# Amin-Nadimy/P-A_multigrids

Hardware: NVIDIA B200
Metric: DG DOF-updates/s per smoother sweep (higher is better)
Workload: dtype f64

## Files before the change

### p-a_multigrids_b200/csrc/pamg_api.cu

```cuda
#include <cuda_runtime.h>
#include <dlfcn.h>

#include <algorithm>
#include <cmath>
#include <cstdio>
#include <cstring>
#include <string>
#include <vector>

#include "pamg_internal.h"
#include "pamg_kernels.cuh"
#include "pamg_unstr.cuh"

using namespace pamg;

namespace {
typedef struct ncclComm* ncclComm_t;
typedef struct { char internal[128]; } ncclUniqueId;
enum { ncclUint8 = 1, ncclInt32 = 2, ncclFloat64 = 8, ncclSum = 0, ncclMax = 2, ncclMin = 3, ncclSuccess = 0 };
struct NcclApi {
  void* lib = nullptr;
  int (*GetUniqueId)(ncclUniqueId*) = nullptr;
  int (*CommInitRank)(ncclComm_t*, int, ncclUniqueId, int) = nullptr;
  int (*CommDestroy)(ncclComm_t) = nullptr;
  int (*GroupStart)() = nullptr;
  int (*GroupEnd)() = nullptr;
  int (*Send)(const void*, size_t, int, int, ncclComm_t, cudaStream_t) = nullptr;
  int (*Recv)(void*, size_t, int, int, ncclComm_t, cudaStream_t) = nullptr;
  int (*AllReduce)(const void*, void*, size_t, int, int, ncclComm_t, cudaStream_t) = nullptr;
  bool load() {
    if (lib) return true;
    lib = dlopen("libnccl.so.2", RTLD_NOW | RTLD_GLOBAL);
    if (!lib) return false;
    GetUniqueId = (decltype(GetUniqueId))dlsym(lib, "ncclGetUniqueId");
    CommInitRank = (decltype(CommInitRank))dlsym(lib, "ncclCommInitRank");
    CommDestroy = (decltype(CommDestroy))dlsym(lib, "ncclCommDestroy");
    GroupStart = (decltype(GroupStart))dlsym(lib, "ncclGroupStart");
    GroupEnd = (decltype(GroupEnd))dlsym(lib, "ncclGroupEnd");
    Send = (decltype(Send))dlsym(lib, "ncclSend");
    Recv = (decltype(Recv))dlsym(lib, "ncclRecv");
    AllReduce = (decltype(AllReduce))dlsym(lib, "ncclAllReduce");
    return GetUniqueId && CommInitRank && CommDestroy && GroupStart && GroupEnd && Send && Recv && AllReduce;
  }
};
NcclApi g_nccl;
}

__attribute__((constructor)) static void pamg_request_eager_loading() { setenv("CUDA_MODULE_LOADING", "EAGER", 0); }

struct pamg_handle;
namespace { void p2p_close(pamg_handle* h); }
enum { AGG_COUNTER = 0, AGG_EPOCH = 8, AGG_FLAGS = 40, AGG_EXPECT = 72, AGG_WORDS = 104 };

struct LevelDev {
  int s = 0, S = 0;
  long long C = 0, nelem = 0, ndof = 0;
  double* T[2] = {nullptr, nullptr};
  int cur = 0;
  bool tnew_alias = true;
  double *told = nullptr, *rhs = nullptr, *res = nullptr;
  double* ovlb[2] = {nullptr, nullptr};
  int ovl_cur = 0;
  bool strips_valid = false;
  bool cut_valid = false;
  bool stage_valid = false;
  ulonglong2* xsend = nullptr;
  double* ovl_old = nullptr;
  double* pc = nullptr;
  double* pc_old = nullptr;
  bool rhs_valid = false;
  double* spare = nullptr;
};

struct pamg_handle {
  pamg_params p;
  int device = 0, nsm = 148;
  cudaStream_t stream = nullptr;
  cudaEvent_t ev[16] = {};
  long long launches = 0;
  std::string err;
  HaloPlan plan;
  int U = 0;
  double* xg = nullptr;
  int32_t *strip_of = nullptr, *dst_strip = nullptr, *rev = nullptr, *hmap = nullptr, *nsrc = nullptr, *cut_lf = nullptr;
  std::vector<int32_t> bc_kind_h; std::vector<double> bc_val_h;
  int32_t* bc_kind = nullptr; double* bc_val = nullptr;
  double* strip_arena = nullptr; size_t strip_arena_bytes = 0;
  bool l2_persist = true;
  std::vector<LevelDev> lev;
  double* partial = nullptr; int npartial = 0; int last_partials = 0;
  double* out3 = nullptr;
  double* out3_host = nullptr;
  double* scratch = nullptr; size_t scratch_bytes = 0;
  int kernel_mode = 4;
  int halo_mode = 2;
  long long debug_gap_ns = 0;
  struct KernelCfg { int win2[2] = {0, 0}, win2x = 0, win[2] = {0, 0}, tma[2] = {0, 0}, gs2 = 0, gs2x = 0, gs = 0, halo = 0; bool done = false; } kc;
  bool capturing = false;
  bool use_graph = true;
  struct VcGraph { long long key; std::vector<cudaGraphExec_t> exec; std::vector<long long> launches; };
  std::vector<VcGraph> vc_graphs;
  bool graph_nccl = true;
  bool gs_tma = true;
  bool win_producer = true;
  bool gs_fused = true;
  bool vc_norm_fuse = true;
  bool profiling = false;
  std::vector<cudaEvent_t> pev;
  int pev_used = 0;
  ncclComm_t comm = nullptr; int nranks = 1, rank = 0;
  pamg_handle* agg = nullptr;
  int agg_level = 0;
  int level_offset = 0;
  bool shared_stream = false;
  std::vector<int32_t> part_first;
  int U_global = 0;
  std::vector<pamg_handle*> parts;
  bool is_root = false;
  bool in_group = false;
  unsigned long long* agg_words = nullptr;
  UnstrDev un;
  int un_use_dir = 0;
  long long un_host_syncs = 0;
  cudaStream_t up_stream = nullptr, down_stream = nullptr;
  cudaEvent_t ev_up = nullptr, ev_comp = nullptr, ev_down[2] = {nullptr, nullptr};
  unsigned pipe_calls = 0;
  const double* last_out = nullptr;
  bool p2p_enabled = true, p2p_ready = false, p2p_failed = false;
  unsigned long long* p2p_sync = nullptr;
  unsigned long long* p2p_err_host = nullptr;
  unsigned long long* p2p_err_dev = nullptr;
  uint4* p2p_stage = nullptr;
  long long p2p_strips = 0;
  bool xchg_in_kernel = true;
  struct P2PPeer { int slot_at_peer = -1, strip_begin_at_peer = 0; long long recv_strips_at_peer = 0; uint4* stage = nullptr; };
  std::vector<P2PPeer> p2p_peers;
  std::vector<void*> p2p_opened;
  unsigned long long p2p_timeout_ns = 60000000000ull;
};

namespace {

int fail(pamg_handle* h, int code, const std::string& msg) {
  if (h) h->err = msg;
  return code;
}
 #define CK_(hh, call)                                                                            \
  do {                                                                                           \
    cudaError_t e_ = (call);                                                                     \
    if (e_ != cudaSuccess)                                                                       \
      return fail(hh, PAMG_ERR_CUDA, std::string(#call) + ": " + cudaGetErrorString(e_));        \
  } while (0)
#define CK(call)                                                                                 \
  do {                                                                                           \
    cudaError_t e_ = (call);                                                                     \
    if (e_ != cudaSuccess)                                                                       \
      return fail(h, PAMG_ERR_CUDA, std::string(#call) + ": " + cudaGetErrorString(e_));         \
  } while (0)

inline int grid_for(const pamg_handle* h, long long n) {
  long long need = (n + TPB - 1) / TPB;
  long long cap = (long long)h->nsm * 8;
  return (int)std::max(1ll, std::min(need, cap));
}

bool valid_level(const pamg_handle* h, int level) { return h && level >= 1 && level <= (int)h->lev.size(); }

double* tnew_ptr(LevelDev& L) { return L.tnew_alias ? L.T[L.cur] : L.T[L.cur ^ 1]; }

int materialise_tnew(pamg_handle* h, LevelDev& L) {
  if (!L.tnew_alias) return PAMG_OK;
  CK(cudaMemcpyAsync(L.T[L.cur ^ 1], L.T[L.cur], L.ndof * sizeof(double), cudaMemcpyDeviceToDevice, h->stream));
  L.tnew_alias = false;
  return PAMG_OK;
}

double* field_ptr(pamg_handle* h, int field, int level, bool for_write, int* rc) {
  *rc = PAMG_OK;
  LevelDev& L = h->lev[level - 1];
  switch (field) {
    case PAMG_TNEW:
      if (for_write) { *rc = materialise_tnew(h, L); L.strips_valid = false; L.cut_valid = false; L.stage_valid = false; return L.T[L.cur ^ 1]; }
      return tnew_ptr(L);
    case PAMG_TNONLIN:
      if (for_write) { *rc = materialise_tnew(h, L); L.strips_valid = false; L.cut_valid = false; L.stage_valid = false; }
      return L.T[L.cur];
    case PAMG_TOLD: if (for_write) L.rhs_valid = false; return L.told;
    case PAMG_RHS: if (for_write) L.rhs_valid = true; return L.rhs;
    case PAMG_RES: return L.res;
  }
  *rc = PAMG_ERR_ARG;
  return nullptr;
}

bool parent_coefficients(const pamg_params& p, const double* Xall, const int32_t* neig, const int32_t* bc_kind,
                         int g , int s, double* pc, double th, bool with_mass = true) {
  bool supported = true;
  const double* X = Xall + (size_t)g * 6;
  const double x1 = X[0], y1 = X[1], x2 = X[2], y2 = X[3], x3 = X[4], y3 = X[5];
  const double A = x1 - x3, B = y1 - y3, Cc = x2 - x3, D = y2 - y3;
  const double detj = A * D - B * Cc;
  const double area = 0.5 * std::fabs(detj);
  const double g1[2] = {D / detj, -Cc / detj}, g2[2] = {-B / detj, A / detj};
  const double g3[2] = {-(g1[0] + g2[0]), -(g1[1] + g2[1])};
  const double* G[3] = {g1, g2, g3};
  const double two_s = std::ldexp(1.0, s), four_s = std::ldexp(1.0, 2 * s);
  pc[PC_CM] = with_mass ? area / (12.0 * four_s * p.dt) : 0.0;
  auto dot = [](const double* a, const double* b) { return a[0] * b[0] + a[1] * b[1]; };
  const double kth = th * p.k;
  pc[PC_K11] = kth * area * dot(g1, g1); pc[PC_K12] = kth * area * dot(g1, g2); pc[PC_K13] = kth * area * dot(g1, g3);
  pc[PC_K22] = kth * area * dot(g2, g2); pc[PC_K23] = kth * area * dot(g2, g3); pc[PC_K33] = kth * area * dot(g3, g3);
  const double uu[2] = {th * p.u_x, th * p.u_y};
  for (int i = 0; i < 3; ++i) pc[PC_ADV + i] = area * dot(G[i], uu) / (3.0 * two_s);
  const double cx = (x1 + x2 + x3) / 3.0, cy = (y1 + y2 + y3) / 3.0;
  const int fa[3] = {0, 2, 1}, fb[3] = {2, 1, 0}, mface[3] = {0, 2, 1};
  const double V1[2] = {A, B}, V2[2] = {Cc, D};
  const double ci[3][2] = {{1.0 / 3, -2.0 / 3}, {-2.0 / 3, 1.0 / 3}, {1.0 / 3, 1.0 / 3}};
  for (int f = 0; f < 3; ++f) {
    const double ax = X[2 * fa[f]], ay = X[2 * fa[f] + 1], bx = X[2 * fb[f]], by = X[2 * fb[f] + 1];
    const double ex = bx - ax, ey = by - ay, L = std::sqrt(ex * ex + ey * ey);
    double nx = ey / L, ny = -ex / L;
    const double mx = 0.5 * (ax + bx), my = 0.5 * (ay + by);
    if (nx * (mx - cx) + ny * (my - cy) < 0) { nx = -nx; ny = -ny; }
    const double lhalf = 0.5 * L;
    pc[PC_FL + f] = (uu[0] * nx + uu[1] * ny) * lhalf / (3.0 * two_s);
    const double dix = ci[f][0] * V1[0] + ci[f][1] * V2[0], diy = ci[f][0] * V1[1] + ci[f][1] * V2[1];
    const double dcI = std::sqrt(dix * dix + diy * diy);
    pc[PC_PENI + f] = kth * lhalf / (3.0 * dcI);
    const int q = neig[(size_t)g * 3 + mface[f]];
    double dcX;
    if (q != 0) {
      const double* Y = Xall + (size_t)(q - 1) * 6;
      const double qx = (Y[0] + Y[2] + Y[4]) / 3.0, qy = (Y[1] + Y[3] + Y[5]) / 3.0;
      dcX = std::sqrt((cx - qx) * (cx - qx) + (cy - qy) * (cy - qy));
    } else {
      dcX = std::sqrt((cx - mx) * (cx - mx) + (cy - my) * (cy - my));
    }
    pc[PC_PENX + f] = kth * lhalf / (3.0 * dcX);
    if (q == 0 && bc_kind && bc_kind[(size_t)g * 3 + mface[f]] == 2) {
      pc[PC_PENX + f] = 0.0;
      if (p.face_terms && pc[PC_FL + f] < 0.0) supported = false;
    }
  }
  const double f2 = p.face_terms ? 2.0 : 0.0;
  pc[PC_W + 0] = p.omega / (4.0 * pc[PC_CM] + pc[PC_K11] + f2 * (pc[PC_PENI + 0] + pc[PC_PENI + 2]));
  pc[PC_W + 1] = p.omega / (4.0 * pc[PC_CM] + pc[PC_K22] + f2 * (pc[PC_PENI + 1] + pc[PC_PENI + 2]));
  pc[PC_W + 2] = p.omega / (4.0 * pc[PC_CM] + pc[PC_K33] + f2 * (pc[PC_PENI + 0] + pc[PC_PENI + 1]));
  pc[22] = 0.0; pc[23] = 0.0;
  for (int o = 0; o < 2; ++o) {
    const double sg = o == 0 ? 1.0 : -1.0;
    double* F = pc + PC_FOLD + 16 * o;
    double A[3][3];
    const double K[3][3] = {{pc[PC_K11], pc[PC_K12], pc[PC_K13]}, {pc[PC_K12], pc[PC_K22], pc[PC_K23]},
                            {pc[PC_K13], pc[PC_K23], pc[PC_K33]}};
    for (int i = 0; i < 3; ++i)
      for (int j = 0; j < 3; ++j)
        A[i][j] = pc[PC_CM] * ((i == j ? 1.0 : 0.0) + 1.0) - sg * pc[PC_ADV + i] + K[i][j];
    const int fa2[3] = {0, 2, 1}, fb2[3] = {2, 1, 0};
    double c[3];
    for (int f = 0; f < 3; ++f) {
      const double pen = p.face_terms ? pc[PC_PENI + f] : 0.0;
      const double fl = p.face_terms ? sg * pc[PC_FL + f] : 0.0;
      const bool in = fl < 0.0;
      const double own = pen + (in ? 0.0 : fl);
      c[f] = -pen + (in ? fl : 0.0);
      const int ia = fa2[f], ib = fb2[f];
      A[ia][ia] += 2.0 * own; A[ia][ib] += own; A[ib][ia] += own; A[ib][ib] += 2.0 * own;
    }
    F[0] = A[0][0]; F[1] = A[0][1]; F[2] = A[0][2]; F[3] = A[1][0]; F[4] = A[1][1]; F[5] = A[1][2];
    F[6] = A[2][0]; F[7] = A[2][1]; F[8] = A[2][2]; F[9] = c[0]; F[10] = c[1]; F[11] = c[2];
    F[12] = pc[PC_W + 0]; F[13] = pc[PC_W + 1]; F[14] = pc[PC_W + 2]; F[15] = 0.0;
  }
  for (int f = 0; f < 3; ++f) pc[PC_DPEN + f] = p.face_terms ? pc[PC_PENX + f] - pc[PC_PENI + f] : 0.0;
  pc[PC_DPEN + 3] = 0.0;
  for (int mask = 0; mask < 8; ++mask) {
    double pen[3];
    for (int f = 0; f < 3; ++f) pen[f] = p.face_terms ? ((mask >> f) & 1 ? pc[PC_PENX + f] : pc[PC_PENI + f]) : 0.0;
    pc[PC_WB + mask * 3 + 0] = p.omega / (4.0 * pc[PC_CM] + pc[PC_K11] + 2.0 * (pen[0] + pen[2]));
    pc[PC_WB + mask * 3 + 1] = p.omega / (4.0 * pc[PC_CM] + pc[PC_K22] + 2.0 * (pen[1] + pen[2]));
    pc[PC_WB + mask * 3 + 2] = p.omega / (4.0 * pc[PC_CM] + pc[PC_K33] + 2.0 * (pen[0] + pen[1]));
  }
  for (int i = PC_WB + 24; i < NPC; ++i) pc[i] = 0.0;
  if (!with_mass) {
    for (int i = 0; i < 3; ++i) { pc[PC_W + i] = 0.0; pc[PC_FOLD + 12 + i] = 0.0; pc[PC_FOLD + 16 + 12 + i] = 0.0; }
    for (int i = 0; i < 24; ++i) pc[PC_WB + i] = 0.0;
  }
  return supported;
}

int launch_halo(pamg_handle* h, int level, int what = 0);
int p2p_upload_args(pamg_handle* h);

void p2p_close(pamg_handle* h) {
  for (void* p : h->p2p_opened) cudaIpcCloseMemHandle(p);
  h->p2p_opened.clear();
  if (h->p2p_sync) { cudaFree(h->p2p_sync); h->p2p_sync = nullptr; }
  if (h->p2p_stage) { cudaFree(h->p2p_stage); h->p2p_stage = nullptr; }
  if (h->p2p_err_host) { cudaFreeHost(h->p2p_err_host); h->p2p_err_host = nullptr; h->p2p_err_dev = nullptr; }
  h->p2p_ready = false; h->p2p_failed = false;
  for (auto& pp : h->p2p_peers) pp.stage = nullptr;
}

int p2p_check(pamg_handle* h) {
  if (h->p2p_err_host && *(volatile unsigned long long*)h->p2p_err_host)
    return fail(h, PAMG_ERR_CUDA, "halo exchange timed out waiting for a peer GPU");
  return PAMG_OK;
}

long long stage_offset(long long strips, const std::vector<LevelDev>& lev, int il) {
  long long off = 0;
  for (int l = 0; l < il; ++l) off += (long long)P2P_SLOTS * strips * 3 * lev[l].S;
  return off;
}

int p2p_alloc_local(pamg_handle* h) {
  long long strips = 0;
  for (const auto& pr : h->plan.peers) strips = std::max(strips, (long long)pr.strip_begin + pr.nfaces);
  h->p2p_strips = strips;
  const size_t nlev = h->lev.size();
  const size_t stage_bytes = (size_t)std::max(1ll, stage_offset(h->p2p_strips, h->lev, (int)nlev)) * sizeof(uint4);
  CK(cudaMalloc(&h->p2p_sync, nlev * P2P_WORDS * sizeof(unsigned long long)));
  CK(cudaMemset(h->p2p_sync, 0, nlev * P2P_WORDS * sizeof(unsigned long long)));
  CK(cudaMalloc(&h->p2p_stage, stage_bytes));
  CK(cudaMemset(h->p2p_stage, 0, stage_bytes));
  CK(cudaHostAlloc(&h->p2p_err_host, sizeof(unsigned long long), cudaHostAllocMapped | cudaHostAllocPortable));
  *h->p2p_err_host = 0;
  CK(cudaHostGetDevicePointer((void**)&h->p2p_err_dev, h->p2p_err_host, 0));
  return PAMG_OK;
}

int p2p_setup(pamg_handle* h) {
  const int R = h->nranks;
  int ok = 1;
  if ((int)h->plan.peers.size() > P2P_MAXP) ok = 0;
  for (const auto& pp : h->p2p_peers) if (pp.slot_at_peer < 0) ok = 0;
  if (p2p_alloc_local(h) != PAMG_OK) { ok = 0; (void)cudaGetLastError(); }
  struct Card { cudaIpcMemHandle_t handle; };
  Card mine;
  std::memset(&mine, 0, sizeof(mine));
  if (ok && cudaIpcGetMemHandle(&mine.handle, h->p2p_stage) != cudaSuccess) { ok = 0; (void)cudaGetLastError(); }
  const size_t hb = sizeof(Card);
  std::vector<Card> all(R);
  unsigned char* d_buf = nullptr;
  const bool have_buf = cudaMalloc(&d_buf, hb * (R + 1) + sizeof(int)) == cudaSuccess;
  int rc = PAMG_OK;
  if (!have_buf) {
    return fail(h, PAMG_ERR_CUDA, "cudaMalloc failed in the halo-exchange set-up");
  }
  unsigned char* d_mine = d_buf; unsigned char* d_all = d_buf + hb; int* d_ok = (int*)(d_buf + hb * (R + 1));
  if (cudaMemcpy(d_mine, &mine, hb, cudaMemcpyHostToDevice) != cudaSuccess) ok = 0;
  g_nccl.GroupStart();
  for (int r = 0; r < R; ++r) {
    g_nccl.Send(d_mine, hb, ncclUint8, r, h->comm, h->stream);
    g_nccl.Recv(d_all + hb * r, hb, ncclUint8, r, h->comm, h->stream);
  }
  if (g_nccl.GroupEnd() != ncclSuccess) rc = fail(h, PAMG_ERR_CUDA, "handle exchange failed");
  if (!rc && cudaStreamSynchronize(h->stream) != cudaSuccess) ok = 0;
  if (!rc && cudaMemcpy(all.data(), d_all, hb * R, cudaMemcpyDeviceToHost) != cudaSuccess) ok = 0;
  if (!rc && ok) {
    for (size_t i = 0; i < h->plan.peers.size(); ++i) {
      void* ptr = nullptr;
      if (cudaIpcOpenMemHandle(&ptr, all[h->plan.peers[i].part].handle, cudaIpcMemLazyEnablePeerAccess) != cudaSuccess) { ok = 0; (void)cudaGetLastError(); break; }
      h->p2p_opened.push_back(ptr);
      h->p2p_peers[i].stage = (uint4*)ptr;
    }
  }
  if (!rc) {
    if (cudaMemcpy(d_ok, &ok, sizeof(int), cudaMemcpyHostToDevice) != cudaSuccess) ok = 0;
    if (g_nccl.AllReduce(d_ok, d_ok, 1, ncclInt32, ncclMin, h->comm, h->stream) != ncclSuccess) rc = fail(h, PAMG_ERR_CUDA, "ncclAllReduce failed");
    else if (cudaStreamSynchronize(h->stream) != cudaSuccess || cudaMemcpy(&ok, d_ok, sizeof(int), cudaMemcpyDeviceToHost) != cudaSuccess)
      rc = fail(h, PAMG_ERR_CUDA, "halo-exchange set-up: reading the agreement failed");
  }
  cudaFree(d_buf);
  if (rc) return rc;
  if (ok) {
    if ((rc = p2p_upload_args(h))) return rc;
    h->p2p_ready = true;
  } else h->p2p_failed = true;
  return PAMG_OK;
}

int p2p_args(pamg_handle* h, LevelDev& L, double* ovl, P2PArgs& a) {
  const long long S3 = 3ll * L.S;
  const int il = (int)(&L - h->lev.data());
  const int base = h->plan.peers[0].send_begin;
  a.send = ovl + ((size_t)h->plan.nstrips + base) * S3;
  a.strips = ovl; a.stage = h->p2p_stage + stage_offset(h->p2p_strips, h->lev, il); a.stage_words = h->p2p_strips * S3;
  a.sync = h->p2p_sync + (size_t)il * P2P_WORDS; a.err = h->p2p_err_dev; a.npeers = (int)h->plan.peers.size();
  a.timeout_ns = h->p2p_timeout_ns;
  long long so = 0, ro = 0;
  for (int i = 0; i < a.npeers; ++i) {
    const auto& pr = h->plan.peers[i];
    if ((long long)(pr.send_begin - base) * S3 != so) return fail(h, PAMG_ERR_STATE, "send slots are not contiguous per peer");
    a.remote[i] = h->p2p_peers[i].stage + stage_offset(h->p2p_peers[i].recv_strips_at_peer, h->lev, il) +
                  (long long)h->p2p_peers[i].strip_begin_at_peer * S3;
    a.rstride[i] = h->p2p_peers[i].recv_strips_at_peer * S3;
    a.soff[i] = so; a.roff[i] = ro; a.rbeg[i] = (long long)pr.strip_begin * S3;
    so += pr.nfaces * S3; ro += pr.nfaces * S3;
  }
  a.soff[a.npeers] = so; a.roff[a.npeers] = ro;
  a.send_base = base;
  return PAMG_OK;
}

int p2p_upload_args(pamg_handle* h) {
  if (h->plan.peers.empty()) return PAMG_OK;
  std::vector<ulonglong2> t((size_t)h->U * 3);
  for (size_t l = 0; l < h->lev.size(); ++l) {
    P2PArgs v;
    std::memset(&v, 0, sizeof(v));
    int rc = p2p_args(h, h->lev[l], h->lev[l].ovlb[0], v);
    if (rc) return rc;
    const long long S3 = 3ll * h->lev[l].S;
    for (int lf = 0; lf < h->U * 3; ++lf) {
      const int d = h->plan.dst_strip[lf];
      t[lf] = make_ulonglong2(0ull, 0ull);
      if (d < h->plan.nstrips) continue;
      const long long q0 = (long long)(d - h->plan.nstrips - v.send_base) * S3;
      int p = 0;
      while (q0 >= v.soff[p + 1]) ++p;
      t[lf] = make_ulonglong2((unsigned long long)(v.remote[p] + (q0 - v.soff[p])), (unsigned long long)v.rstride[p]);
    }
    if (!h->lev[l].xsend) CK(cudaMalloc(&h->lev[l].xsend, t.size() * sizeof(ulonglong2)));
    CK(cudaMemcpy(h->lev[l].xsend, t.data(), t.size() * sizeof(ulonglong2), cudaMemcpyHostToDevice));
  }
  return PAMG_OK;
}

int exchange_halo_nccl(pamg_handle* h, LevelDev& L, double* ovl) {
  if (!h->comm) return fail(h, PAMG_ERR_STATE, "partitioned mesh but pamg_comm_init was not called");
  const size_t S3 = (size_t)3 * L.S;
  g_nccl.GroupStart();
  for (const auto& pr : h->plan.peers) {
    const size_t n = (size_t)pr.nfaces * S3;
    g_nccl.Send(ovl + ((size_t)h->plan.nstrips + pr.send_begin) * S3, n, ncclFloat64, pr.part, h->comm, h->stream);
    g_nccl.Recv(ovl + (size_t)pr.strip_begin * S3, n, ncclFloat64, pr.part, h->comm, h->stream);
  }
  if (g_nccl.GroupEnd() != ncclSuccess) return fail(h, PAMG_ERR_CUDA, "ncclGroupEnd failed in halo exchange");
  return PAMG_OK;
}

int launch_halo(pamg_handle* h, int level, int what) {
  LevelDev& L = h->lev[level - 1];
  HaloArgs a;
  a.tnew = tnew_ptr(L); a.told = L.told; a.ovl = L.ovlb[L.ovl_cur]; a.ovl_old = L.ovl_old; a.xg = h->xg;
  a.dst_strip = h->dst_strip; a.rev = h->rev; a.strip_of = h->strip_of;
  a.bc_scale = (h->p.coarse_bc_zero && level + h->level_offset > 1) ? 0.0 : 1.0;
  a.U = h->U; a.s = L.s; a.with_old = (what == 0) ? 1 : 0; a.what = what; a.nstrips = h->plan.nstrips;
  a.cut_lf = h->cut_lf; a.ncut = (int)h->plan.cut_lf.size();
  a.bc_kind = h->bc_kind; a.bc_val = h->bc_val;
  const bool cut = what != 1 && !h->plan.peers.empty();
  if ((what == 2 || what == 4) && !cut) { L.cut_valid = true; return PAMG_OK; }
  if (what == 4 && !(h->p2p_ready && L.stage_valid)) return fail(h, PAMG_ERR_STATE, "nothing staged to unpack");
  const long long n = (what == 2 ? (long long)a.ncut : what == 4 ? (long long)a.ncut * 3 : (long long)h->U * 3) * L.S;
  a.x.npeers = 0;
  if (cut && h->comm && h->p2p_enabled && !h->p2p_ready && !h->p2p_failed && !h->capturing && h->level_offset == 0) {
    int rc = p2p_setup(h);
    if (rc) return rc;
  }
  const bool fused_x = cut && h->p2p_ready;
  if (what == 0 && cut) {
    HaloArgs b = a;
    b.tnew = L.told; b.ovl = L.ovl_old; b.with_old = 0; b.what = 2;
    if (fused_x) { int rc = p2p_args(h, L, L.ovl_old, b.x); if (rc) return rc; }
    const long long n2 = (long long)b.ncut * L.S;
    int g2 = grid_for(h, n2);
    if (fused_x) g2 = std::min(g2, h->nsm * std::min(std::max(h->kc.halo, 1), 4));
    k_halo<<<g2, TPB, 0, h->stream>>>(b);
    h->launches++;
    CK(cudaGetLastError());
    if (!fused_x) { int rc = exchange_halo_nccl(h, L, L.ovl_old); if (rc) return rc; }
  }
  if (fused_x) { int rc = p2p_args(h, L, L.ovlb[L.ovl_cur], a.x); if (rc) return rc; }
  int hgrid = grid_for(h, n);
  if (fused_x) hgrid = std::min(hgrid, h->nsm * std::min(std::max(h->kc.halo, 1), 4));
  k_halo<<<hgrid, TPB, 0, h->stream>>>(a);
  h->launches++;
  CK(cudaGetLastError());
  if (what == 1) return PAMG_OK;
  if (what == 4) { L.cut_valid = true; return PAMG_OK; }
  if (cut && !fused_x) { int rc = exchange_halo_nccl(h, L, L.ovlb[L.ovl_cur]); if (rc) return rc; }
  L.cut_valid = true;
  if (fused_x) L.stage_valid = true;
  if (what != 2) L.strips_valid = true;
  return PAMG_OK;
}

int ensure_strips(pamg_handle* h, int level, bool all = true) {
  LevelDev& L = h->lev[level - 1];
  if (!h->p.face_terms) return PAMG_OK;
  if ((all || h->halo_mode == 0) && !L.strips_valid) return launch_halo(h, level, 3);
  if (L.cut_valid) return PAMG_OK;
  return launch_halo(h, level, (L.stage_valid && h->p2p_ready) ? 4 : 2);
}

bool xchg_kernel(const pamg_handle* h, const LevelDev& L) {
  return h->xchg_in_kernel && h->p2p_ready && L.xsend && !h->plan.peers.empty() && h->p.face_terms &&
         h->kernel_mode == 4 && h->win_producer && L.s >= 6 && L.s <= 8;
}

int add_old_time_terms(pamg_handle* h);

int launch_build_rhs(pamg_handle* h) {
  LevelDev& L = h->lev[0];
  RhsArgs a;
  a.told = L.told; a.rhs = L.rhs; a.pc = L.pc; a.xg = h->xg; a.dt = h->p.dt; a.source_coef = h->p.source_coef;
  a.nelem = L.nelem; a.s = L.s; a.literal_source = h->p.literal_source;
  k_build_rhs<<<grid_for(h, L.nelem), TPB, 0, h->stream>>>(a);
  h->launches++;
  CK(cudaGetLastError());
  if (L.pc_old) { int rc = add_old_time_terms(h); if (rc) return rc; }
  L.rhs_valid = true;
  return PAMG_OK;
}

template <typename K>
int configure_one(pamg_handle* h, K kern, int threads, size_t smem, int& resident) {
  CK(cudaFuncSetAttribute(kern, cudaFuncAttributeMaxDynamicSharedMemorySize, (int)smem));
  CK(cudaOccupancyMaxActiveBlocksPerMultiprocessor(&resident, kern, threads, smem));
  if (resident < 1) resident = 1;
  return PAMG_OK;
}
template <bool FACE>
int configure_face(pamg_handle* h) {
  int rc, dummy = 0;
  const int f = FACE ? 1 : 0;
  if ((rc = configure_one(h, k_element_win2<MODE_JACOBI, FACE>, WIN2_THREADS, WIN_SMEM_BYTES, h->kc.win2[f]))) return rc;
  if ((rc = configure_one(h, k_element_win2<MODE_RESID, FACE>, WIN2_THREADS, WIN_SMEM_BYTES, dummy))) return rc;
  if ((rc = configure_one(h, k_element_win2<MODE_RICH, FACE>, WIN2_THREADS, WIN_SMEM_BYTES, dummy))) return rc;
  if (FACE) {
    if ((rc = configure_one(h, k_element_win2<MODE_JACOBI, FACE, true>, WIN2_THREADS, WIN_SMEM_BYTES, h->kc.win2x))) return rc;
    if ((rc = configure_one(h, k_element_win2<MODE_JACOBI, FACE, false, true>, WIN2_THREADS, WIN_SMEM_BYTES, dummy))) return rc;
    if ((rc = configure_one(h, k_element_win2<MODE_JACOBI, FACE, true, true>, WIN2_THREADS, WIN_SMEM_BYTES, dummy))) return rc;
    if ((rc = configure_one(h, k_element_win2<MODE_RICH, FACE, true>, WIN2_THREADS, WIN_SMEM_BYTES, dummy))) return rc;
  }
  if ((rc = configure_one(h, k_element_win<MODE_JACOBI, FACE>, TPB, WIN_SMEM_BYTES, h->kc.win[f]))) return rc;
  if ((rc = configure_one(h, k_element_win<MODE_RESID, FACE>, TPB, WIN_SMEM_BYTES, dummy))) return rc;
  if ((rc = configure_one(h, k_element_win<MODE_RICH, FACE>, TPB, WIN_SMEM_BYTES, dummy))) return rc;
  if ((rc = configure_one(h, k_element_win<MODE_GS, FACE>, TPB, WIN_SMEM_BYTES, dummy))) return rc;
  if ((rc = configure_one(h, k_element_tma<MODE_JACOBI, FACE>, TPB, TMA_SMEM_BYTES, h->kc.tma[f]))) return rc;
  if ((rc = configure_one(h, k_element_tma<MODE_RESID, FACE>, TPB, TMA_SMEM_BYTES, dummy))) return rc;
  if ((rc = configure_one(h, k_element_tma<MODE_RICH, FACE>, TPB, TMA_SMEM_BYTES, dummy))) return rc;
  if ((rc = configure_one(h, k_element_tma<MODE_GS, FACE>, TPB, TMA_SMEM_BYTES, dummy))) return rc;
  return PAMG_OK;
}
int configure_kernels(pamg_handle* h) {
  if (h->kc.done) return PAMG_OK;
  int rc;
  if ((rc = configure_face<true>(h))) return rc;
  if ((rc = configure_face<false>(h))) return rc;
  if ((rc = configure_one(h, k_gs_win2<false>, WIN2_THREADS, GSW_SMEM_BYTES, h->kc.gs2))) return rc;
  if ((rc = configure_one(h, k_gs_win2<true>, WIN2_THREADS, GSW_SMEM_BYTES, h->kc.gs2x))) return rc;
  if ((rc = configure_one(h, k_gs_win, TPB, GSW_SMEM_BYTES, h->kc.gs))) return rc;
  CK(cudaOccupancyMaxActiveBlocksPerMultiprocessor(&h->kc.halo, k_halo, TPB, 0));
  if (h->kc.halo < 1) h->kc.halo = 1;
  cudaFuncAttributes fa;
  CK(cudaFuncGetAttributes(&fa, k_halo));
  CK(cudaFuncGetAttributes(&fa, k_gs_small));
  CK(cudaFuncGetAttributes(&fa, k_build_rhs));
  CK(cudaFuncGetAttributes(&fa, k_restrict));
  CK(cudaFuncGetAttributes(&fa, k_prolong_literal));
  CK(cudaFuncGetAttributes(&fa, k_prolong_p1));
  CK(cudaFuncGetAttributes(&fa, k_reduce_partials));
  CK(cudaFuncGetAttributes(&fa, k_fill));
  CK(cudaFuncGetAttributes(&fa, k_push));
  CK(cudaFuncGetAttributes(&fa, k_wait_flags));
  CK(cudaFuncGetAttributes(&fa, k_spin));
  CK(cudaFuncGetAttributes(&fa, k_output_fields));
  CK(cudaFuncGetAttributes(&fa, k_element_direct2<MODE_JACOBI, true>));
  CK(cudaFuncGetAttributes(&fa, k_element_direct2<MODE_JACOBI, false>));
  CK(cudaFuncGetAttributes(&fa, k_element_direct2<MODE_RESID, true>));
  CK(cudaFuncGetAttributes(&fa, k_element_direct2<MODE_RESID, false>));
  CK(cudaFuncGetAttributes(&fa, k_element_direct2<MODE_RICH, true>));
  CK(cudaFuncGetAttributes(&fa, k_element_direct2<MODE_RICH, false>));
  CK(cudaFuncGetAttributes(&fa, k_element_direct2<MODE_GS, true>));
  CK(cudaFuncGetAttributes(&fa, k_element_direct2<MODE_GS, false>));
  h->kc.done = true;
  return PAMG_OK;
}

bool producer_kernel(const pamg_handle* h, const LevelDev& L, bool gs) {
  if (!(h->kernel_mode == 4 && h->win_producer && L.s >= 6 && L.s <= 8)) return false;
  return !gs || (h->gs_fused && h->p.face_terms);
}

struct ElemOverride { const double* ovl; const double* pc; double rsign; };

template <int MODE>
int launch_element(pamg_handle* h, LevelDev& L, const double* Tin, double* Tout, int colour, int grid, bool use_strips,
                   bool write_next = false, bool xchg = false, bool norm = false, const ElemOverride* ov = nullptr) {
  ElemArgs a;
  a.xsend = L.xsend; a.xsync = h->p2p_sync ? h->p2p_sync + (size_t)(&L - h->lev.data()) * P2P_WORDS : nullptr;
  if (MODE == MODE_RESID) xchg = false;
  a.Tin = Tin; a.Tout = Tout; a.rhs = L.rhs; a.ovl = L.ovlb[L.ovl_cur]; a.pc = L.pc; a.strip_of = h->strip_of; a.hmap = h->hmap;
  a.nsrc = (use_strips || Tin == Tout) ? nullptr : h->nsrc;
  a.ovl_next = write_next ? L.ovlb[L.ovl_cur ^ 1] : nullptr; a.dst_strip = h->dst_strip; a.rev = h->rev; a.nstrips = h->plan.nstrips;
  a.partial = h->partial; a.omega = h->p.omega; a.rsign = (double)h->p.residual_sign; a.nelem = L.nelem; a.s = L.s;
  a.colour = colour; a.partial_off = 0;
  if (ov) { a.ovl = ov->ovl; a.pc = ov->pc; a.rsign = ov->rsign; }
  const int f = h->p.face_terms ? 1 : 0;
  const bool prof = !ov && h->profiling && h->pev_used + 2 <= (int)h->pev.size();
  if (prof) CK(cudaEventRecord(h->pev[h->pev_used], h->stream));
  if (MODE != MODE_GS && h->kernel_mode == 4 && h->win_producer && L.s >= 6 && L.s <= 8) {
    auto kern = xchg ? k_element_win2<MODE == MODE_RESID ? MODE_JACOBI : MODE, true, true>
                     : h->p.face_terms ? k_element_win2<MODE, true> : k_element_win2<MODE, false>;
    if (norm) kern = xchg ? k_element_win2<MODE == MODE_JACOBI ? MODE_JACOBI : MODE, true, true, MODE == MODE_JACOBI>
                          : k_element_win2<MODE == MODE_JACOBI ? MODE_JACOBI : MODE, true, false, MODE == MODE_JACOBI>;
    const int tgrid = (int)std::max(1ll, std::min(L.nelem / TPB, (long long)h->nsm * (xchg ? h->kc.win2x : h->kc.win2[f])));
    kern<<<tgrid, WIN2_THREADS, WIN_SMEM_BYTES, h->stream>>>(a);
    if (MODE == MODE_RESID || norm) h->last_partials = tgrid;
  } else if ((MODE != MODE_GS || h->gs_tma) && h->kernel_mode == 4 && L.C >= TPB && L.s <= 8) {
    auto kern = h->p.face_terms ? k_element_win<MODE, true> : k_element_win<MODE, false>;
    const int tgrid = (int)std::max(1ll, std::min(L.nelem / TPB, (long long)h->nsm * h->kc.win[f]));
    kern<<<tgrid, TPB, WIN_SMEM_BYTES, h->stream>>>(a);
    if (MODE == MODE_RESID) h->last_partials = tgrid;
  } else if ((MODE != MODE_GS || h->gs_tma) && (h->kernel_mode == 1 || h->kernel_mode == 4) && L.C >= TPB) {
    auto kern = h->p.face_terms ? k_element_tma<MODE, true> : k_element_tma<MODE, false>;
    const int tgrid = (int)std::max(1ll, std::min((L.nelem + TPB - 1) / TPB, (long long)h->nsm * h->kc.tma[f]));
    kern<<<tgrid, TPB, TMA_SMEM_BYTES, h->stream>>>(a);
    if (MODE == MODE_RESID) h->last_partials = tgrid;
  } else {
    if (MODE == MODE_RESID) h->last_partials = grid;
    if (h->p.face_terms) k_element_direct2<MODE, true><<<grid, TPB, 0, h->stream>>>(a);
    else k_element_direct2<MODE, false><<<grid, TPB, 0, h->stream>>>(a);
  }
  if (prof) { CK(cudaEventRecord(h->pev[h->pev_used + 1], h->stream)); h->pev_used += 2; }
  h->launches++;
  CK(cudaGetLastError());
  return PAMG_OK;
}

int exchange_told_cut(pamg_handle* h) {
  LevelDev& L = h->lev[0];
  if (h->plan.peers.empty()) return PAMG_OK;
  HaloArgs b;
  b.tnew = L.told; b.told = L.told; b.ovl = L.ovl_old; b.ovl_old = L.ovl_old; b.xg = h->xg;
  b.dst_strip = h->dst_strip; b.rev = h->rev; b.strip_of = h->strip_of;
  b.bc_scale = 1.0; b.U = h->U; b.s = L.s; b.with_old = 0; b.what = 2; b.nstrips = h->plan.nstrips;
  b.cut_lf = h->cut_lf; b.ncut = (int)h->plan.cut_lf.size();
  b.bc_kind = h->bc_kind; b.bc_val = h->bc_val;
  b.x.npeers = 0;
  if (h->comm && h->p2p_enabled && !h->p2p_ready && !h->p2p_failed && !h->capturing && h->level_offset == 0) {
    int rc = p2p_setup(h);
    if (rc) return rc;
  }
  const bool fused_x = h->p2p_ready;
  if (fused_x) { int rc = p2p_args(h, L, L.ovl_old, b.x); if (rc) return rc; }
  int g2 = grid_for(h, (long long)b.ncut * L.S);
  if (fused_x) g2 = std::min(g2, h->nsm * std::min(std::max(h->kc.halo, 1), 4));
  k_halo<<<g2, TPB, 0, h->stream>>>(b);
  h->launches++;
  CK(cudaGetLastError());
  if (!fused_x) { int rc = exchange_halo_nccl(h, L, L.ovl_old); if (rc) return rc; }
  if (fused_x) L.stage_valid = false;
  return PAMG_OK;
}

int add_old_time_terms(pamg_handle* h) {
  LevelDev& L = h->lev[0];
  int rc;
  if (h->p.face_terms && (rc = exchange_told_cut(h))) return rc;
  const int grid = grid_for(h, L.nelem);
  if (2 * grid > h->npartial) return fail(h, PAMG_ERR_STATE, "partial buffer too small");
  const ElemOverride ov = {L.ovl_old, L.pc_old, -1.0};
  if ((rc = launch_element<MODE_RESID>(h, L, L.told, L.res, 0, grid, false, false, false, false, &ov))) return rc;
  CK(cudaMemcpyAsync(L.rhs, L.res, (size_t)L.ndof * sizeof(double), cudaMemcpyDeviceToDevice, h->stream));
  return PAMG_OK;
}

bool gs_small_ok(const pamg_handle* h, const LevelDev& L) {
  return h->gs_fused && h->kernel_mode == 4 && h->p.face_terms && L.C <= TPB;
}
bool gs_fused_ok(const pamg_handle* h, const LevelDev& L) {
  if (gs_small_ok(h, L)) return true;
  return h->gs_fused && h->kernel_mode == 4 && h->p.face_terms && L.C >= TPB && L.s <= 8;
}

int launch_gs_fused(pamg_handle* h, LevelDev& L, const double* Tin, double* Tout, bool use_strips, bool write_next, bool xchg) {
  ElemArgs a;
  a.xsend = L.xsend; a.xsync = h->p2p_sync ? h->p2p_sync + (size_t)(&L - h->lev.data()) * P2P_WORDS : nullptr;
  a.Tin = Tin; a.Tout = Tout; a.rhs = L.rhs; a.ovl = L.ovlb[L.ovl_cur]; a.pc = L.pc; a.strip_of = h->strip_of; a.hmap = h->hmap;
  a.nsrc = use_strips ? nullptr : h->nsrc;
  a.ovl_next = write_next ? L.ovlb[L.ovl_cur ^ 1] : nullptr; a.dst_strip = h->dst_strip; a.rev = h->rev; a.nstrips = h->plan.nstrips;
  a.partial = h->partial; a.omega = h->p.omega; a.rsign = (double)h->p.residual_sign; a.nelem = L.nelem; a.s = L.s;
  a.colour = 1; a.partial_off = 0;
  if (gs_small_ok(h, L)) {
    const long long ppc = TPB / L.C, nparents = L.nelem / L.C;
    const int sgrid = (int)std::max(1ll, std::min((nparents + ppc - 1) / ppc, (long long)h->nsm * 8));
    k_gs_small<<<sgrid, TPB, 0, h->stream>>>(a);
    h->launches++;
    CK(cudaGetLastError());
    return PAMG_OK;
  }
  const bool producer = h->win_producer && L.s >= 6;
  const int resident = producer ? (xchg ? h->kc.gs2x : h->kc.gs2) : h->kc.gs;
  const bool prof = h->profiling && h->pev_used + 2 <= (int)h->pev.size();
  if (prof) CK(cudaEventRecord(h->pev[h->pev_used], h->stream));
  const int tgrid = (int)std::max(1ll, std::min(L.nelem / TPB, (long long)h->nsm * resident));
  if (producer && xchg) k_gs_win2<true><<<tgrid, WIN2_THREADS, GSW_SMEM_BYTES, h->stream>>>(a);
  else if (producer) k_gs_win2<false><<<tgrid, WIN2_THREADS, GSW_SMEM_BYTES, h->stream>>>(a);
  else k_gs_win<<<tgrid, TPB, GSW_SMEM_BYTES, h->stream>>>(a);
  if (prof) { CK(cudaEventRecord(h->pev[h->pev_used + 1], h->stream)); h->pev_used += 2; }
  h->launches++;
  CK(cudaGetLastError());
  return PAMG_OK;
}

bool norm_fusable(const pamg_handle* h, const LevelDev& L) {
  return h->p.face_terms && h->kernel_mode == 4 && h->win_producer && L.s >= 6 && L.s <= 8;
}

int do_smooth(pamg_handle* h, int level, int solver, int nsweeps, bool norm_first = false) {
  LevelDev& L = h->lev[level - 1];
  if (level == 1 && !L.rhs_valid) { int rc = launch_build_rhs(h); if (rc) return rc; }
  const int grid = grid_for(h, L.nelem);
  if (solver < 1 || solver > 4) return fail(h, PAMG_ERR_ARG, "solver must be 1 (Jacobi), 2 (Richardson) or 3 (Gauss-Seidel)");
  for (int sw = 0; sw < nsweeps; ++sw) {
    L.tnew_alias = true;
    if (h->debug_gap_ns > 0) { k_spin<<<1, 32, 0, h->stream>>>(h->debug_gap_ns); }
    const bool gs = solver == 3 || solver == 4;
    const bool in_place = gs && !gs_fused_ok(h, L);
    const bool fusedk = h->halo_mode == 2 && h->p.face_terms && !in_place && producer_kernel(h, L, gs);
    const bool use_strips = in_place || fusedk || h->halo_mode == 0;
    const bool xs = fusedk && xchg_kernel(h, L) && (!gs || (h->win_producer && L.s >= 6));
    int rc = ensure_strips(h, level, use_strips);
    if (rc) return rc;
    if (solver == 1 || solver == 2) {
      rc = (solver == 1) ? launch_element<MODE_JACOBI>(h, L, L.T[L.cur], L.T[L.cur ^ 1], 0, grid, use_strips, fusedk, xs,
                                                       norm_first && sw == 0)
                         : launch_element<MODE_RICH>(h, L, L.T[L.cur], L.T[L.cur ^ 1], 0, grid, use_strips, fusedk, xs);
      if (rc) return rc;
      L.cur ^= 1;
      L.tnew_alias = false;
    } else if (!in_place) {
      rc = launch_gs_fused(h, L, L.T[L.cur], L.T[L.cur ^ 1], use_strips, fusedk, xs);
      if (rc) return rc;
      L.cur ^= 1;
      L.tnew_alias = false;
    } else {
      if (sw == nsweeps - 1 && h->p.keep_tnew_gs) { rc = materialise_tnew(h, L); if (rc) return rc; }
      rc = launch_element<MODE_GS>(h, L, L.T[L.cur], L.T[L.cur], 0, grid, true);
      if (rc) return rc;
      rc = launch_element<MODE_GS>(h, L, L.T[L.cur], L.T[L.cur], 1, grid, true);
      if (rc) return rc;
    }
    if (fusedk) {
      L.ovl_cur ^= 1;
      L.strips_valid = true; L.cut_valid = h->plan.peers.empty();
      L.stage_valid = xs;
    } else {
      L.strips_valid = false; L.cut_valid = false; L.stage_valid = false;
    }
  }
  return PAMG_OK;
}

int queue_norms(pamg_handle* h) {
  k_reduce_partials<<<1, 1024, 0, h->stream>>>(h->partial, h->last_partials, h->out3);
  h->launches++;
  CK(cudaGetLastError());
  if (h->comm && h->nranks > 1) {
    g_nccl.GroupStart();
    g_nccl.AllReduce(h->out3, h->out3, 1, ncclFloat64, ncclSum, h->comm, h->stream);
    g_nccl.AllReduce(h->out3 + 1, h->out3 + 1, 2, ncclFloat64, ncclMax, h->comm, h->stream);
    if (g_nccl.GroupEnd() != ncclSuccess) return fail(h, PAMG_ERR_CUDA, "ncclAllReduce failed");
  }
  CK(cudaMemcpyAsync(h->out3_host, h->out3, 3 * sizeof(double), cudaMemcpyDeviceToHost, h->stream));
  return PAMG_OK;
}

int do_residual(pamg_handle* h, int level, double* l2, double* linf, double* smax, bool queue_only = false) {
  LevelDev& L = h->lev[level - 1];
  if (level == 1 && !L.rhs_valid) { int rc = launch_build_rhs(h); if (rc) return rc; }
  const int grid = grid_for(h, L.nelem);
  if (2 * grid > h->npartial) return fail(h, PAMG_ERR_STATE, "partial buffer too small");
  const bool use_strips = L.strips_valid || h->halo_mode == 0;
  int rc = ensure_strips(h, level, use_strips);
  if (rc) return rc;
  rc = launch_element<MODE_RESID>(h, L, tnew_ptr(L), L.res, 0, grid, use_strips);
  if (rc) return rc;
  if (l2 || linf || smax) {
    if ((rc = queue_norms(h))) return rc;
    if (queue_only || h->capturing) return PAMG_OK;
    CK(cudaStreamSynchronize(h->stream));
    if ((rc = p2p_check(h))) return rc;
    if (l2) *l2 = std::sqrt(h->out3_host[0]);
    if (linf) *linf = h->out3_host[1];
    if (smax) *smax = h->out3_host[2];
  }
  return PAMG_OK;
}

int do_restrict(pamg_handle* h, int fine_level) {
  if (fine_level >= (int)h->lev.size()) return PAMG_OK;
  LevelDev& F = h->lev[fine_level - 1];
  LevelDev& Cc = h->lev[fine_level];
  XferArgs a;
  a.src = F.res; a.dst = Cc.rhs; a.ncoarse = Cc.nelem; a.sc = Cc.s; a.mode = h->p.transfer;
  k_restrict<<<grid_for(h, Cc.nelem), TPB, 0, h->stream>>>(a);
  h->launches++;
  CK(cudaGetLastError());
  Cc.rhs_valid = true;
  return PAMG_OK;
}

int do_prolong(pamg_handle* h, int fine_level, bool keep_tnew = true) {
  if (fine_level >= (int)h->lev.size()) return fail(h, PAMG_ERR_ARG, "no coarser level to prolong from");
  LevelDev& F = h->lev[fine_level - 1];
  LevelDev& Cc = h->lev[fine_level];
  XferArgs a;
  a.ncoarse = Cc.nelem; a.sc = Cc.s; a.mode = h->p.transfer;
  if (h->p.transfer == 0) {
    int rc = materialise_tnew(h, F);
    if (rc) return rc;
    a.src = tnew_ptr(Cc); a.dst = F.T[F.cur ^ 1];
    k_prolong_literal<<<grid_for(h, Cc.nelem), TPB, 0, h->stream>>>(a);
  } else {
    if (keep_tnew) {
      int rc = materialise_tnew(h, F);
      if (rc) return rc;
    } else {
      F.tnew_alias = true;
    }
    a.src = Cc.T[Cc.cur]; a.dst = F.T[F.cur];
    F.strips_valid = false; F.cut_valid = false; F.stage_valid = false;
    k_prolong_p1<<<grid_for(h, F.nelem), TPB, 0, h->stream>>>(a);
  }
  h->launches++;
  CK(cudaGetLastError());
  return PAMG_OK;
}

int do_fill(pamg_handle* h, double* p, long long n, double v) {
  if (v == 0.0) { CK(cudaMemsetAsync(p, 0, n * sizeof(double), h->stream)); return PAMG_OK; }
  k_fill<<<grid_for(h, n), TPB, 0, h->stream>>>(p, n, v);
  h->launches++;
  CK(cudaGetLastError());
  return PAMG_OK;
}

typedef std::vector<pamg_handle*> Group;
Group group_of(pamg_handle* h) { return h->parts.empty() ? Group{h} : h->parts; }
int gfail(pamg_handle* owner, pamg_handle* q, int rc) { if (owner != q) owner->err = q->err; return rc; }
#define GALL(G, owner, q, expr)                                            \
  do {                                                                     \
    for (pamg_handle* q : G) {                                             \
      if (q->in_group) cudaSetDevice(q->device);                           \
      int rc_ = (expr);                                                    \
      if (rc_) return gfail(owner, q, rc_);                                \
    }                                                                      \
  } while (0)

int vcycle_rec(const Group& G, pamg_handle* owner, int level, int solver, int nu1, int nu2, int ncoarse, int skip_pre = 0);

int launch_push(pamg_handle* q, const double* src, double* dst, long long n, int channel, unsigned long long* peer_flag) {
  PushArgs a;
  a.src = src; a.dst = dst; a.n = n; a.counter = q->agg_words + AGG_COUNTER; a.epoch = q->agg_words + AGG_EPOCH + channel;
  a.flag = peer_flag;
  const int grid = (int)std::max(1ll, std::min((n + TPB - 1) / TPB, (long long)q->nsm * 2));
  k_push<<<grid, TPB, 0, q->stream>>>(a);
  q->launches++;
  CK_(q, cudaGetLastError());
  return PAMG_OK;
}

int launch_wait(pamg_handle* q, unsigned senders) {
  WaitArgs a;
  a.flags = q->agg_words + AGG_FLAGS; a.expect = q->agg_words + AGG_EXPECT; a.err = q->p2p_err_dev;
  a.timeout_ns = q->p2p_timeout_ns; a.senders = senders;
  k_wait_flags<<<1, 32, 0, q->stream>>>(a);
  q->launches++;
  CK_(q, cudaGetLastError());
  return PAMG_OK;
}

int agg_coarse_solve(const Group& G, pamg_handle* owner, int solver, int nu1, int nu2, int ncoarse) {
  pamg_handle* h0 = G[0];
  const int lvl = h0->agg_level;
  const size_t per_parent = (size_t)3 * h0->lev[lvl - 1].C;
  if (G.size() == 1) {
    pamg_handle* h = h0;
    LevelDev& Lc = h->lev[lvl - 1];
    if (!h->comm) return fail(h, PAMG_ERR_STATE, "agglomeration needs pamg_comm_init");
    g_nccl.GroupStart();
    if (h->rank == 0) {
      LevelDev& A = h->agg->lev[0];
      for (int p = 1; p < h->nranks; ++p)
        g_nccl.Recv(A.rhs + per_parent * h->part_first[p], per_parent * (h->part_first[p + 1] - h->part_first[p]), ncclFloat64, p,
                    h->comm, h->stream);
    } else {
      g_nccl.Send(Lc.rhs, per_parent * h->U, ncclFloat64, 0, h->comm, h->stream);
    }
    if (g_nccl.GroupEnd() != ncclSuccess) return fail(h, PAMG_ERR_CUDA, "ncclGroupEnd failed in coarse gather");
    if (h->rank == 0) {
      pamg_handle* g = h->agg;
      LevelDev& A = g->lev[0];
      CK(cudaMemcpyAsync(A.rhs, Lc.rhs, per_parent * h->U * sizeof(double), cudaMemcpyDeviceToDevice, h->stream));
      CK(cudaMemsetAsync(A.T[A.cur], 0, A.ndof * sizeof(double), h->stream));
      A.tnew_alias = true; A.strips_valid = false; A.cut_valid = false; A.stage_valid = false; A.rhs_valid = true;
      const long long l0 = g->launches;
      int rc = vcycle_rec(Group{g}, g, 1, solver, nu1, nu2, ncoarse);
      h->launches += g->launches - l0;
      if (rc) return fail(h, rc, g->err);
      CK(cudaMemcpyAsync(Lc.T[Lc.cur], A.T[A.cur], per_parent * h->U * sizeof(double), cudaMemcpyDeviceToDevice, h->stream));
    }
    g_nccl.GroupStart();
    if (h->rank == 0) {
      LevelDev& A = h->agg->lev[0];
      for (int p = 1; p < h->nranks; ++p)
        g_nccl.Send(A.T[A.cur] + per_parent * h->part_first[p], per_parent * (h->part_first[p + 1] - h->part_first[p]), ncclFloat64,
                    p, h->comm, h->stream);
    } else {
      g_nccl.Recv(Lc.T[Lc.cur], per_parent * h->U, ncclFloat64, 0, h->comm, h->stream);
    }
    if (g_nccl.GroupEnd() != ncclSuccess) return fail(h, PAMG_ERR_CUDA, "ncclGroupEnd failed in coarse scatter");
    Lc.tnew_alias = true; Lc.strips_valid = false; Lc.cut_valid = false; Lc.stage_valid = false;
    return PAMG_OK;
  }
  pamg_handle* g = h0->agg;
  LevelDev& A = g->lev[0];
  unsigned all = 0;
  for (size_t p = 1; p < G.size(); ++p) {
    pamg_handle* q = G[p];
    cudaSetDevice(q->device);
    LevelDev& Lc = q->lev[lvl - 1];
    int rc = launch_push(q, Lc.rhs, A.rhs + per_parent * q->part_first[p], (long long)(per_parent * q->U), 0,
                         h0->agg_words + AGG_FLAGS + p);
    if (rc) return gfail(owner, q, rc);
    all |= 1u << p;
  }
  {
    pamg_handle* h = h0;
    cudaSetDevice(h->device);
    LevelDev& Lc = h->lev[lvl - 1];
    CK(cudaMemcpyAsync(A.rhs, Lc.rhs, per_parent * h->U * sizeof(double), cudaMemcpyDeviceToDevice, h->stream));
    CK(cudaMemsetAsync(A.T[A.cur], 0, A.ndof * sizeof(double), h->stream));
    int rc = launch_wait(h, all);
    if (rc) return gfail(owner, h, rc);
    A.tnew_alias = true; A.strips_valid = false; A.cut_valid = false; A.stage_valid = false; A.rhs_valid = true;
    const long long l0 = g->launches;
    rc = vcycle_rec(Group{g}, g, 1, solver, nu1, nu2, ncoarse);
    h->launches += g->launches - l0;
    if (rc) { h->err = g->err; return gfail(owner, h, rc); }
    CK(cudaMemcpyAsync(Lc.T[Lc.cur], A.T[A.cur], per_parent * h->U * sizeof(double), cudaMemcpyDeviceToDevice, h->stream));
    Lc.tnew_alias = true; Lc.strips_valid = false; Lc.cut_valid = false; Lc.stage_valid = false;
    for (size_t p = 1; p < G.size(); ++p) {
      pamg_handle* q = G[p];
      LevelDev& Lq = q->lev[lvl - 1];
      rc = launch_push(h, A.T[A.cur] + per_parent * q->part_first[p], Lq.T[Lq.cur], (long long)(per_parent * q->U), (int)p,
                       q->agg_words + AGG_FLAGS + 0);
      if (rc) return gfail(owner, h, rc);
    }
  }
  for (size_t p = 1; p < G.size(); ++p) {
    pamg_handle* q = G[p];
    cudaSetDevice(q->device);
    int rc = launch_wait(q, 1u);
    if (rc) return gfail(owner, q, rc);
    LevelDev& Lq = q->lev[lvl - 1];
    Lq.tnew_alias = true; Lq.strips_valid = false; Lq.cut_valid = false; Lq.stage_valid = false;
  }
  return PAMG_OK;
}

int normalise_parity(pamg_handle* h, LevelDev& L, int cur0) {
  if (L.cur == cur0) return PAMG_OK;
  CK(cudaMemcpyAsync(L.T[L.cur ^ 1], L.T[L.cur], L.ndof * sizeof(double), cudaMemcpyDeviceToDevice, h->stream));
  L.cur ^= 1;
  L.tnew_alias = true;
  return PAMG_OK;
}

int vcycle_rec(const Group& G, pamg_handle* owner, int level, int solver, int nu1, int nu2, int ncoarse, int skip_pre) {
  const int Lmax = (int)G[0]->lev.size();
  std::vector<int> cur0(G.size());
  for (size_t i = 0; i < G.size(); ++i) cur0[i] = G[i]->lev[level - 1].cur;
  auto restore = [&]() -> int {
    for (size_t i = 0; i < G.size(); ++i) {
      if (G[i]->in_group) cudaSetDevice(G[i]->device);
      int rc = normalise_parity(G[i], G[i]->lev[level - 1], cur0[i]);
      if (rc) return gfail(owner, G[i], rc);
    }
    return PAMG_OK;
  };
  if (level == Lmax) {
    GALL(G, owner, q, do_smooth(q, level, solver, ncoarse));
    return restore();
  }
  GALL(G, owner, q, do_smooth(q, level, solver, nu1 - skip_pre));
  for (pamg_handle* q : G) q->lev[level - 1].tnew_alias = true;
  GALL(G, owner, q, do_residual(q, level, nullptr, nullptr, nullptr));
  GALL(G, owner, q, do_restrict(q, level));
  for (pamg_handle* q : G) {
    if (q->in_group) cudaSetDevice(q->device);
    LevelDev& Cc = q->lev[level];
    int rc = do_fill(q, Cc.T[Cc.cur], Cc.ndof, 0.0);
    if (rc) return gfail(owner, q, rc);
    Cc.tnew_alias = true;
    Cc.strips_valid = false; Cc.cut_valid = false; Cc.stage_valid = false;
  }
  int rc;
  if (G[0]->agg_level && level + 1 == G[0]->agg_level) {
    if ((rc = agg_coarse_solve(G, owner, solver, nu1, nu2, ncoarse))) return rc;
  } else {
    if ((rc = vcycle_rec(G, owner, level + 1, solver, nu1, nu2, ncoarse))) return rc;
  }
  GALL(G, owner, q, do_prolong(q, level, false));
  GALL(G, owner, q, do_smooth(q, level, solver, nu2));
  return skip_pre ? PAMG_OK : restore();
}

int vcycle_body(const Group& G, pamg_handle* owner, int solver, int nu1, int nu2, int ncoarse, bool fuse = false, bool first = true) {
  int rc;
  if ((rc = vcycle_rec(G, owner, 1, solver, nu1, nu2, ncoarse, (fuse && !first) ? 1 : 0))) return rc;
  for (pamg_handle* q : G) q->lev[0].tnew_alias = true;
  if (fuse) {
    GALL(G, owner, q, do_smooth(q, 1, solver, 1, true));
    GALL(G, owner, q, queue_norms(q));
    return PAMG_OK;
  }
  double dummy;
  GALL(G, owner, q, do_residual(q, 1, &dummy, nullptr, nullptr, true));
  return PAMG_OK;
}

int undo_norm_sweep(pamg_handle* h) {
  LevelDev& L = h->lev[0];
  const bool fusedk = h->halo_mode == 2 && h->p.face_terms && producer_kernel(h, L, false);
  L.cur ^= 1;
  L.tnew_alias = true;
  if (fusedk) { L.ovl_cur ^= 1; L.strips_valid = true; L.cut_valid = true; }
  else { L.strips_valid = false; L.cut_valid = false; }
  L.stage_valid = false;
  return PAMG_OK;
}

int group_norms(const Group& G, pamg_handle* owner, double* l2, double* linf, double* smax) {
  double s0 = 0.0, s1 = 0.0, s2 = 0.0;
  for (pamg_handle* q : G) {
    if (q->in_group) cudaSetDevice(q->device);
    CK_(q, cudaStreamSynchronize(q->stream));
    int rc = p2p_check(q);
    if (rc) return gfail(owner, q, rc);
    s0 += q->out3_host[0]; s1 = std::max(s1, q->out3_host[1]); s2 = std::max(s2, q->out3_host[2]);
  }
  for (pamg_handle* q : G) if (q != owner && !q->err.empty()) { owner->err = q->err; }
  if (l2) *l2 = std::sqrt(s0);
  if (linf) *linf = s1;
  if (smax) *smax = s2;
  return PAMG_OK;
}

void free_levels(pamg_handle* h) {
  for (auto& g : h->vc_graphs) for (auto e : g.exec) cudaGraphExecDestroy(e);
  h->vc_graphs.clear();
  for (auto& L : h->lev) {
    cudaFree(L.T[0]); cudaFree(L.T[1]); cudaFree(L.spare); cudaFree(L.told); cudaFree(L.rhs); cudaFree(L.res);
    cudaFree(L.ovl_old); cudaFree(L.pc); cudaFree(L.pc_old); cudaFree(L.xsend);
  }
  h->lev.clear();
  cudaFree(h->strip_arena); h->strip_arena = nullptr; h->strip_arena_bytes = 0;
  cudaFree(h->xg); cudaFree(h->strip_of); cudaFree(h->dst_strip); cudaFree(h->rev); cudaFree(h->hmap);
  cudaFree(h->nsrc); cudaFree(h->cut_lf); cudaFree(h->bc_kind); cudaFree(h->bc_val);
  cudaFree(h->partial);
  h->xg = nullptr; h->strip_of = h->dst_strip = h->rev = h->hmap = h->nsrc = h->cut_lf = h->bc_kind = nullptr;
  h->bc_val = nullptr; h->partial = nullptr;
}

}

#define FANOUT(h, q, expr)                                                              \
  if ((h) && !(h)->parts.empty()) {                                                     \
    for (pamg_handle* q : (h)->parts) { int rc_ = (expr); if (rc_) return gfail((h), q, rc_); } \
    return PAMG_OK;                                                                     \
  }
#define ON_PART0(h) if ((h) && !(h)->parts.empty()) (h) = (h)->parts[0]

extern "C" {

const char* pamg_version(void) { return "pamg-b200 0.1 (sm_100a)"; }

int pamg_device_count(int* n) {
  if (!n) return PAMG_ERR_ARG;
  int c = 0;
  cudaError_t e = cudaGetDeviceCount(&c);
  if (e != cudaSuccess || c < 1) { *n = 0; return PAMG_ERR_CUDA; }
  *n = c;
  return PAMG_OK;
}

void pamg_default_params(pamg_params* p, int literal_head) {
  if (!p) return;
  std::memset(p, 0, sizeof(*p));
  p->n_split = 1; p->multi_levels = 1; p->n_smooth = 4; p->n_multigrid = 2; p->n_coarse_smooth = 15; p->solver = 3;
  p->theta = 1.0; p->k = 1.0; p->omega = 0.8; p->u_x = 0.0; p->u_y = 0.0;
  if (literal_head) {
    p->dt = 1.25e-5; p->face_terms = 0; p->literal_source = 1; p->transfer = 0; p->residual_sign = 1;
    p->halo_rule = 0; p->coarse_bc_zero = 0; p->source_coef = -2.0; p->keep_tnew_gs = 1;
  } else {
    p->dt = 1e-3; p->face_terms = 1; p->literal_source = 0; p->transfer = 1; p->residual_sign = -1;
    p->halo_rule = 1; p->coarse_bc_zero = 1; p->source_coef = 2.0; p->keep_tnew_gs = 0;
  }
}

int pamg_create(const pamg_params* p, int device, pamg_handle** out) {
  if (!p || !out) return PAMG_ERR_ARG;
  *out = nullptr;
  if (p->n_split < 1 || p->n_split > 13 || p->multi_levels < 1 || p->multi_levels > p->n_split) return PAMG_ERR_ARG;
  if (!(p->theta >= 0.0 && p->theta <= 1.0)) return PAMG_ERR_ARG;
  if (!(p->dt > 0.0)) return PAMG_ERR_ARG;
  int ndev = 0;
  if (cudaGetDeviceCount(&ndev) != cudaSuccess || ndev < 1) return PAMG_ERR_CUDA;
  if (device < 0 || device >= ndev) return PAMG_ERR_ARG;
  pamg_handle* h = new pamg_handle();
  h->p = *p; h->device = device;
  {
    const char* e = getenv("PAMG_KERNEL");
    if (e && !strcmp(e, "tma1d")) h->kernel_mode = 1;
    else if (e && !strcmp(e, "direct2")) h->kernel_mode = 3;
    else if (e && !strcmp(e, "win")) h->kernel_mode = 4;
    const char* wp = getenv("PAMG_WIN");
    if (wp && !strcmp(wp, "producer")) h->win_producer = true;
    if (wp && !strcmp(wp, "barrier")) h->win_producer = false;
    const char* pp = getenv("PAMG_P2P");
    if (pp && pp[0] == '0') h->p2p_enabled = false;
    const char* pt = getenv("PAMG_P2P_TIMEOUT_S");
    if (pt && atof(pt) > 0.0) h->p2p_timeout_ns = (unsigned long long)(atof(pt) * 1e9);
    const char* dg = getenv("PAMG_DEBUG_GAP_NS");
    if (dg) h->debug_gap_ns = atoll(dg);
    const char* lp = getenv("PAMG_L2_PERSIST");
    if (lp && lp[0] == '0') h->l2_persist = false;
    const char* vn = getenv("PAMG_VC_NORM");
    if (vn && vn[0] == '0') h->vc_norm_fuse = false;
    const char* xk = getenv("PAMG_XCHG");
    if (xk && !strcmp(xk, "halo")) h->xchg_in_kernel = false;
    const char* hl = getenv("PAMG_HALO");
    if (hl && !strcmp(hl, "strips")) h->halo_mode = 0;
    if (hl && !strcmp(hl, "direct")) h->halo_mode = 1;
    if (hl && !strcmp(hl, "fused")) h->halo_mode = 2;
    const char* gr = getenv("PAMG_GRAPH");
    if (gr && gr[0] == '0') h->use_graph = false;
    const char* gn = getenv("PAMG_GRAPH_NCCL");
    if (gn && gn[0] == '0') h->graph_nccl = false;
    const char* g = getenv("PAMG_GS");
    if (g && !strcmp(g, "direct")) { h->gs_tma = false; h->gs_fused = false; }
    if (g && !strcmp(g, "twopass")) h->gs_fused = false;
  }
  if (cudaSetDevice(device) != cudaSuccess) { delete h; return PAMG_ERR_CUDA; }
  cudaDeviceProp prop;
  if (cudaGetDeviceProperties(&prop, device) == cudaSuccess) h->nsm = prop.multiProcessorCount;
  if (cudaStreamCreateWithFlags(&h->stream, cudaStreamNonBlocking) != cudaSuccess) { delete h; return PAMG_ERR_CUDA; }
  bool ok = true;
  for (auto& e : h->ev) ok = ok && cudaEventCreate(&e) == cudaSuccess;
  ok = ok && cudaMalloc(&h->out3, 3 * sizeof(double)) == cudaSuccess;
  ok = ok && cudaMallocHost(&h->out3_host, 3 * sizeof(double)) == cudaSuccess;
  ok = ok && configure_kernels(h) == PAMG_OK;
  if (!ok) { pamg_destroy(h); return PAMG_ERR_CUDA; }
  *out = h;
  return PAMG_OK;
}

namespace {
int group_p2p_setup(pamg_handle* root) {
  const Group& G = root->parts;
  for (pamg_handle* a : G)
    for (pamg_handle* b : G) {
      if (a->device == b->device) continue;
      int can = 0;
      CK_(root, cudaDeviceCanAccessPeer(&can, a->device, b->device));
      if (!can) return fail(root, PAMG_ERR_UNSUPPORTED, "the GPUs of the group cannot access each other's memory (no NVLink / PCIe peer access)");
      CK_(root, cudaSetDevice(a->device));
      cudaError_t e = cudaDeviceEnablePeerAccess(b->device, 0);
      if (e != cudaSuccess && e != cudaErrorPeerAccessAlreadyEnabled) return fail(root, PAMG_ERR_CUDA, std::string("cudaDeviceEnablePeerAccess: ") + cudaGetErrorString(e));
      (void)cudaGetLastError();
    }
  for (pamg_handle* q : G) {
    CK_(root, cudaSetDevice(q->device));
    if ((int)q->plan.peers.size() > P2P_MAXP) return fail(root, PAMG_ERR_UNSUPPORTED, "too many neighbour parts");
    int rc = p2p_alloc_local(q);
    if (rc) return gfail(root, q, rc);
    CK_(root, cudaMalloc(&q->agg_words, AGG_WORDS * sizeof(unsigned long long)));
    CK_(root, cudaMemset(q->agg_words, 0, AGG_WORDS * sizeof(unsigned long long)));
  }
  for (pamg_handle* q : G) {
    for (size_t i = 0; i < q->plan.peers.size(); ++i) {
      if (q->p2p_peers[i].slot_at_peer < 0) return fail(root, PAMG_ERR_STATE, "inconsistent halo plans between parts");
      q->p2p_peers[i].stage = G[q->plan.peers[i].part]->p2p_stage;
    }
  }
  for (pamg_handle* q : G) {
    CK_(root, cudaSetDevice(q->device));
    int rc = p2p_upload_args(q);
    if (rc) return gfail(root, q, rc);
    q->p2p_ready = true;
  }
  return PAMG_OK;
}
}

int pamg_create_multi(const pamg_params* p, int ngpus, const int* devices, pamg_handle** out) {
  if (!p || !out || ngpus < 1 || ngpus > 16) return PAMG_ERR_ARG;
  *out = nullptr;
  pamg_handle* root = new pamg_handle();
  root->p = *p; root->is_root = true;
  for (int i = 0; i < ngpus; ++i) {
    pamg_handle* q = nullptr;
    int rc = pamg_create(p, devices ? devices[i] : i, &q);
    if (rc) { pamg_destroy(root); return rc; }
    q->in_group = true; q->nranks = ngpus; q->rank = i;
    root->parts.push_back(q);
  }
  root->device = root->parts[0]->device; root->nsm = root->parts[0]->nsm; root->use_graph = root->parts[0]->use_graph;
  *out = root;
  return PAMG_OK;
}

void pamg_destroy(pamg_handle* h) {
  if (!h) return;
  if (h->is_root) {
    for (pamg_handle* q : h->parts) { cudaSetDevice(q->device); if (q->stream) cudaStreamSynchronize(q->stream); }
    for (auto& g : h->vc_graphs) for (auto e : g.exec) cudaGraphExecDestroy(e);
    h->vc_graphs.clear();
    for (pamg_handle* q : h->parts) pamg_destroy(q);
    delete h;
    return;
  }
  cudaSetDevice(h->device);
  if (h->stream) cudaStreamSynchronize(h->stream);
  for (auto& g : h->vc_graphs) for (auto e : g.exec) cudaGraphExecDestroy(e);
  h->vc_graphs.clear();
  if (h->stream) cudaStreamSynchronize(h->stream);
  if (h->agg) { pamg_destroy(h->agg); h->agg = nullptr; }
  if (h->comm) g_nccl.CommDestroy(h->comm);
  p2p_close(h);
  if (h->agg_words) { cudaFree(h->agg_words); h->agg_words = nullptr; }
  free_levels(h);
  unstr_free(h->un);
  cudaFree(h->out3); cudaFreeHost(h->out3_host); cudaFree(h->scratch);
  for (auto& e : h->ev) if (e) cudaEventDestroy(e);
  for (auto& e : h->pev) if (e) cudaEventDestroy(e);
  if (h->up_stream) { cudaStreamSynchronize(h->up_stream); cudaStreamSynchronize(h->down_stream); cudaStreamDestroy(h->up_stream); cudaStreamDestroy(h->down_stream); cudaEventDestroy(h->ev_up); cudaEventDestroy(h->ev_comp); cudaEventDestroy(h->ev_down[0]); cudaEventDestroy(h->ev_down[1]); }
  if (h->stream && !h->shared_stream) cudaStreamDestroy(h->stream);
  delete h;
}

const char* pamg_last_error(const pamg_handle* h) { return h ? h->err.c_str() : "null handle"; }

int pamg_set_parents_partition(pamg_handle* h, int U_global, const double* X, const int32_t* neig,
                               const int32_t* fneig, const int32_t* dir, int nparts, const int32_t* part_first,
                               int my_part) {
  if (!h) return PAMG_ERR_ARG;
  if (h->is_root) return fail(h, PAMG_ERR_ARG, "a multi-GPU handle partitions the mesh itself: call pamg_set_parents");
  CK(cudaSetDevice(h->device));
  int rc = build_halo_plan(U_global, X, neig, fneig, dir, h->p.halo_rule, nparts, part_first, my_part, h->plan);
  if (rc) return fail(h, rc, "inconsistent parent arrays (X / Neig / fNeig)");
  free_levels(h);
  if (h->agg) { pamg_destroy(h->agg); h->agg = nullptr; }
  h->agg_level = 0;
  p2p_close(h);
  h->p2p_peers.assign(h->plan.peers.size(), pamg_handle::P2PPeer());
  for (size_t i = 0; i < h->plan.peers.size(); ++i) {
    HaloPlan theirs;
    if (build_halo_plan(U_global, X, neig, fneig, dir, h->p.halo_rule, nparts, part_first, h->plan.peers[i].part, theirs)) continue;
    for (size_t j = 0; j < theirs.peers.size(); ++j)
      h->p2p_peers[i].recv_strips_at_peer = std::max(h->p2p_peers[i].recv_strips_at_peer, (long long)theirs.peers[j].strip_begin + theirs.peers[j].nfaces);
    for (size_t j = 0; j < theirs.peers.size(); ++j)
      if (theirs.peers[j].part == my_part && theirs.peers[j].nfaces == h->plan.peers[i].nfaces) {
        h->p2p_peers[i].slot_at_peer = (int)j;
        h->p2p_peers[i].strip_begin_at_peer = theirs.peers[j].strip_begin;
      }
  }
  const int U = h->plan.U_local, first = h->plan.first;
  if (U < 1) return fail(h, PAMG_ERR_ARG, "empty partition");
  h->U = U; h->U_global = U_global;
  h->part_first.assign(nparts + 1, 0);
  if (part_first) for (int i = 0; i <= nparts; ++i) h->part_first[i] = part_first[i]; else h->part_first[1] = U_global;
  std::vector<double> xg((size_t)U * 6);
  for (int u = 0; u < U; ++u) {
    const double* P = X + (size_t)(first + u) * 6;
    double* o = &xg[(size_t)u * 6];
    o[0] = P[4]; o[1] = P[5]; o[2] = P[0] - P[4]; o[3] = P[1] - P[5]; o[4] = P[2] - P[4]; o[5] = P[3] - P[5];
  }
  CK(cudaMalloc(&h->xg, xg.size() * sizeof(double)));
  CK(cudaMemcpy(h->xg, xg.data(), xg.size() * sizeof(double), cudaMemcpyHostToDevice));
  const size_t n3 = (size_t)U * 3 * sizeof(int32_t);
  CK(cudaMalloc(&h->strip_of, n3)); CK(cudaMalloc(&h->dst_strip, n3)); CK(cudaMalloc(&h->rev, n3)); CK(cudaMalloc(&h->hmap, n3));
  CK(cudaMemcpy(h->strip_of, h->plan.strip_of.data(), n3, cudaMemcpyHostToDevice));
  CK(cudaMemcpy(h->dst_strip, h->plan.dst_strip.data(), n3, cudaMemcpyHostToDevice));
  CK(cudaMemcpy(h->rev, h->plan.rev.data(), n3, cudaMemcpyHostToDevice));
  CK(cudaMemcpy(h->hmap, h->plan.hmap.data(), n3, cudaMemcpyHostToDevice));
  CK(cudaMalloc(&h->nsrc, n3));
  CK(cudaMemcpy(h->nsrc, h->plan.nsrc.data(), n3, cudaMemcpyHostToDevice));
  if (!h->plan.cut_lf.empty()) {
    CK(cudaMalloc(&h->cut_lf, h->plan.cut_lf.size() * sizeof(int32_t)));
    CK(cudaMemcpy(h->cut_lf, h->plan.cut_lf.data(), h->plan.cut_lf.size() * sizeof(int32_t), cudaMemcpyHostToDevice));
  }
  const int32_t* bc_glob = nullptr;
  if (!h->bc_kind_h.empty()) {
    if ((int)h->bc_kind_h.size() != U_global * 3) return fail(h, PAMG_ERR_ARG, "pamg_set_boundary_data was given a different number of parents");
    bc_glob = h->bc_kind_h.data();
    CK(cudaMalloc(&h->bc_kind, n3)); CK(cudaMalloc(&h->bc_val, (size_t)U * 3 * sizeof(double)));
    CK(cudaMemcpy(h->bc_kind, h->bc_kind_h.data() + (size_t)first * 3, n3, cudaMemcpyHostToDevice));
    CK(cudaMemcpy(h->bc_val, h->bc_val_h.data() + (size_t)first * 3, (size_t)U * 3 * sizeof(double), cudaMemcpyHostToDevice));
  }
  h->lev.resize(h->p.multi_levels);
  {
    size_t tot = 0;
    for (int il = 0; il < h->p.multi_levels; ++il) {
      const size_t S = (size_t)1 << (h->p.n_split - il);
      tot += 2 * (((size_t)(h->plan.nstrips + h->plan.nsend) * 3 * S * sizeof(double) + 255) / 256 * 256);
    }
    CK(cudaMalloc(&h->strip_arena, tot));
    CK(cudaMemsetAsync(h->strip_arena, 0, tot, h->stream));
    h->strip_arena_bytes = tot;
    if (h->l2_persist && !h->shared_stream) {
      cudaDeviceProp prop;
      if (cudaGetDeviceProperties(&prop, h->device) == cudaSuccess && prop.persistingL2CacheMaxSize > 0) {
        const size_t want = std::min((size_t)prop.persistingL2CacheMaxSize, std::max(tot, (size_t)1 << 20));
        cudaDeviceSetLimit(cudaLimitPersistingL2CacheSize, want);
        cudaStreamAttrValue av;
        std::memset(&av, 0, sizeof(av));
        av.accessPolicyWindow.base_ptr = h->strip_arena;
        av.accessPolicyWindow.num_bytes = std::min(tot, (size_t)prop.accessPolicyMaxWindowSize);
        av.accessPolicyWindow.hitRatio = (float)std::min(1.0, (double)want / (double)std::max(tot, (size_t)1));
        av.accessPolicyWindow.hitProp = cudaAccessPropertyPersisting;
        av.accessPolicyWindow.missProp = cudaAccessPropertyStreaming;
        cudaStreamSetAttribute(h->stream, cudaStreamAttributeAccessPolicyWindow, &av);
        (void)cudaGetLastError();
      }
    }
  }
  size_t arena_off = 0;
  std::vector<double> pc((size_t)U * NPC);
  for (int il = 0; il < h->p.multi_levels; ++il) {
    LevelDev& L = h->lev[il];
    L.s = h->p.n_split - il; L.S = 1 << L.s; L.C = 1ll << (2 * L.s);
    L.nelem = L.C * U; L.ndof = 3 * L.nelem;
    const size_t fb = (size_t)L.ndof * sizeof(double);
    CK(cudaMalloc(&L.T[0], fb)); CK(cudaMalloc(&L.T[1], fb)); CK(cudaMalloc(&L.told, fb));
    CK(cudaMalloc(&L.rhs, fb)); CK(cudaMalloc(&L.res, fb));
    CK(cudaMemsetAsync(L.T[0], 0, fb, h->stream)); CK(cudaMemsetAsync(L.T[1], 0, fb, h->stream));
    CK(cudaMemsetAsync(L.told, 0, fb, h->stream)); CK(cudaMemsetAsync(L.rhs, 0, fb, h->stream));
    CK(cudaMemsetAsync(L.res, 0, fb, h->stream));
    const size_t ob = (size_t)(h->plan.nstrips + h->plan.nsend) * 3 * L.S * sizeof(double);
    const size_t obp = (ob + 255) / 256 * 256;
    L.ovlb[0] = reinterpret_cast<double*>(reinterpret_cast<char*>(h->strip_arena) + arena_off);
    L.ovlb[1] = reinterpret_cast<double*>(reinterpret_cast<char*>(h->strip_arena) + arena_off + obp);
    arena_off += 2 * obp;
    CK(cudaMalloc(&L.ovl_old, ob));
    CK(cudaMemsetAsync(L.ovl_old, 0, ob, h->stream));
    L.ovl_cur = 0; L.strips_valid = false; L.cut_valid = false; L.stage_valid = false;
    for (int u = 0; u < U; ++u)
      if (!parent_coefficients(h->p, X, neig, bc_glob, first + u, L.s, &pc[(size_t)u * NPC], h->p.theta))
        return fail(h, PAMG_ERR_UNSUPPORTED, "open boundary face (kind 2) with inflow: give it Dirichlet data instead");
    CK(cudaMalloc(&L.pc, pc.size() * sizeof(double)));
    CK(cudaMemcpy(L.pc, pc.data(), pc.size() * sizeof(double), cudaMemcpyHostToDevice));
    if (il == 0 && h->p.theta != 1.0 && h->level_offset == 0) {
      for (int u = 0; u < U; ++u)
        if (!parent_coefficients(h->p, X, neig, bc_glob, first + u, L.s, &pc[(size_t)u * NPC], 1.0 - h->p.theta, false))
          return fail(h, PAMG_ERR_UNSUPPORTED, "open boundary face (kind 2) with inflow: give it Dirichlet data instead");
      CK(cudaMalloc(&L.pc_old, pc.size() * sizeof(double)));
      CK(cudaMemcpy(L.pc_old, pc.data(), pc.size() * sizeof(double), cudaMemcpyHostToDevice));
    }
    L.cur = 0; L.tnew_alias = true; L.rhs_valid = (il != 0);
  }
  for (int il = 1; il <= h->p.multi_levels; ++il)
    for (int bsel = 0; bsel < 2; ++bsel) {
      h->lev[il - 1].ovl_cur = bsel;
      int rc2 = launch_halo(h, il, 1);
      if (rc2) return rc2;
    }
  for (auto& Lv : h->lev) Lv.ovl_cur = 0;
  if (h->lev[0].pc_old) {
    LevelDev& L1 = h->lev[0];
    double* keep = L1.ovlb[0];
    L1.ovlb[0] = L1.ovl_old;
    int rc2 = launch_halo(h, 1, 1);
    L1.ovlb[0] = keep;
    if (rc2) return rc2;
  }
  if (nparts > 1 && h->level_offset == 0) {
    const char* e = getenv("PAMG_AGG_ELEMS");
    const long long limit = e ? atoll(e) : (1ll << 17);
    int lvl = 0;
    for (int il = 2; il <= h->p.multi_levels; ++il)
      if (limit > 0 && (long long)U_global * h->lev[il - 1].C <= limit) { lvl = il; break; }
    if (lvl) {
      h->agg_level = lvl;
      if (my_part == 0) {
        pamg_params ap = h->p;
        ap.n_split = h->lev[lvl - 1].s;
        ap.multi_levels = h->p.multi_levels - lvl + 1;
        pamg_handle* g = new pamg_handle();
        g->p = ap; g->device = h->device; g->nsm = h->nsm; g->kernel_mode = h->kernel_mode; g->gs_tma = h->gs_tma; g->gs_fused = h->gs_fused; g->win_producer = h->win_producer;
        g->stream = h->stream; g->shared_stream = true; g->level_offset = lvl - 1; g->halo_mode = h->halo_mode;
        g->bc_kind_h = h->bc_kind_h; g->bc_val_h = h->bc_val_h;
        h->agg = g;
        for (auto& ev : g->ev) CK(cudaEventCreate(&ev));
        CK(cudaMalloc(&g->out3, 3 * sizeof(double)));
        CK(cudaMallocHost(&g->out3_host, 3 * sizeof(double)));
        if (configure_kernels(g)) return fail(h, PAMG_ERR_CUDA, g->err);
        int rc3 = pamg_set_parents_partition(g, U_global, X, neig, fneig, dir, 1, nullptr, 0);
        if (rc3) return fail(h, rc3, std::string("agglomerated coarse problem: ") + g->err);
      }
    }
  }
  h->npartial = h->nsm * 16;
  CK(cudaMalloc(&h->partial, (size_t)h->npartial * 3 * sizeof(double)));
  CK(cudaStreamSynchronize(h->stream));
  return PAMG_OK;
}

int pamg_halo_sources(int U_global, const double* X, const int32_t* neig, const int32_t* fneig, const int32_t* dir,
                      int halo_rule, int nparts, const int32_t* part_first, int my_part, int s, int64_t* src) {
  if (!src || s < 1 || s > 13) return PAMG_ERR_ARG;
  HaloPlan plan;
  int rc = build_halo_plan(U_global, X, neig, fneig, dir, halo_rule, nparts, part_first, my_part, plan);
  if (rc != PAMG_OK) return rc;
  const int S = 1 << s;
  for (int lf = 0; lf < plan.U_local * 3; ++lf) {
    const int d = plan.nsrc[lf];
    for (int p = 0; p < S; ++p) {
      int64_t* o = src + ((size_t)lf * S + p) * 2;
      if (d < 0) { o[0] = o[1] = -1; continue; }
      const size_t base = nbr_child_offset(d, p, s);
      o[0] = (int64_t)(base + (d & 3)); o[1] = (int64_t)(base + ((d >> 2) & 3));
    }
  }
  return PAMG_OK;
}

int pamg_numbering(int what, int s, int64_t first, int64_t count, int32_t* out) {
  if (!out || s < 1 || s > 13 || what < 0 || what > 3 || first < 0 || count < 0) return PAMG_ERR_ARG;
  const int64_t C = (int64_t)1 << (2 * s);
  if (first + count > C) return PAMG_ERR_ARG;
  const int b = 2 << s;
  for (int64_t i = 0; i < count; ++i) {
    const int k = (int)(first + i);
    int32_t* o = out + 4 * i;
    int r = 0, ipos = 0, ele = 0, len = 0;
    if (what == 0) { child_from_ele0(k, s, r, ipos, len); o[0] = r; o[1] = ipos; o[2] = len; o[3] = 0; }
    else if (what == 1) { child_from_flat(k, s, r, ipos, ele, len); o[0] = r; o[1] = ipos; o[2] = ele; o[3] = len; }
    else if (what == 2) { int fin[4]; child_from_ele0(k, s, r, ipos, len); fine_children(s, r, ipos, fin); for (int q = 0; q < 4; ++q) o[q] = fin[q]; }
    else {
      if (k + TPB >= C) { o[0] = o[1] = o[2] = o[3] = 0; continue; }
      child_from_ele0(k, s, r, ipos, len);
      child_advance(s, b, k + TPB, r, ipos);
      o[0] = r; o[1] = ipos; o[2] = b + 1 - 2 * r; o[3] = 0;
    }
  }
  return PAMG_OK;
}

int pamg_parent_table(const pamg_params* p, int U, const double* X, const int32_t* neig, const int32_t* bc_kind, int parent,
                      int s, double theta_weight, int with_mass, double* table) {
  if (!p || !X || !neig || !table || U < 1 || parent < 0 || parent >= U || s < 0 || s > 13 || !(p->dt > 0.0)) return PAMG_ERR_ARG;
  for (int f = 0; f < 3; ++f) { const int q = neig[(size_t)parent * 3 + f]; if (q < 0 || q > U) return PAMG_ERR_ARG; }
  return parent_coefficients(*p, X, neig, bc_kind, parent, s, table, theta_weight, with_mass != 0) ? PAMG_OK : PAMG_ERR_UNSUPPORTED;
}

int pamg_set_boundary_data(pamg_handle* h, int U_global, const int32_t* kind, const double* value) {
  if (!h || U_global < 1 || !kind) return PAMG_ERR_ARG;
  for (size_t i = 0; i < (size_t)U_global * 3; ++i)
    if (kind[i] < 0 || kind[i] > 2) return fail(h, PAMG_ERR_ARG, "boundary kind must be 0 (sin(x+y)), 1 (constant) or 2 (open)");
  h->bc_kind_h.assign(kind, kind + (size_t)U_global * 3);
  if (value) h->bc_val_h.assign(value, value + (size_t)U_global * 3);
  else h->bc_val_h.assign((size_t)U_global * 3, 0.0);
  FANOUT(h, q, pamg_set_boundary_data(q, U_global, kind, value));
  if (!h->lev.empty()) return fail(h, PAMG_ERR_STATE, "pamg_set_boundary_data must precede pamg_set_parents (the coefficient tables depend on it)");
  return PAMG_OK;
}

int pamg_set_parents(pamg_handle* h, int U, const double* X, const int32_t* neig, const int32_t* fneig,
                     const int32_t* dir) {
  if (h && h->is_root) {
    const int n = (int)h->parts.size();
    if (U < n) return fail(h, PAMG_ERR_ARG, "fewer parents than GPUs");
    std::vector<int32_t> pf(n + 1);
    for (int i = 0; i <= n; ++i) pf[i] = (int32_t)((long long)U * i / n);
    for (auto& g : h->vc_graphs) for (auto e : g.exec) cudaGraphExecDestroy(e);
    h->vc_graphs.clear();
    for (int i = 0; i < n; ++i) {
      pamg_handle* q = h->parts[i];
      if (q->agg_words) { cudaSetDevice(q->device); cudaFree(q->agg_words); q->agg_words = nullptr; }
      int rc = pamg_set_parents_partition(q, U, X, neig, fneig, dir, n, pf.data(), i);
      if (rc) return gfail(h, q, rc);
    }
    h->U = U; h->U_global = U;
    return n > 1 ? group_p2p_setup(h) : PAMG_OK;
  }
  return pamg_set_parents_partition(h, U, X, neig, fneig, dir, 1, nullptr, 0);
}

int pamg_ndof(const pamg_handle* h, int level, int64_t* ndof) {
  if (h && h->is_root && ndof) {
    *ndof = 0;
    for (const pamg_handle* q : h->parts) { if (!valid_level(q, level)) return PAMG_ERR_ARG; *ndof += q->lev[level - 1].ndof; }
    return PAMG_OK;
  }
  if (!valid_level(h, level) || !ndof) return PAMG_ERR_ARG;
  *ndof = h->lev[level - 1].ndof;
  return PAMG_OK;
}

int pamg_upload_field(pamg_handle* h, int field, int level, const double* host) {
  if (h && h->is_root && host) {
    size_t off = 0;
    for (pamg_handle* q : h->parts) {
      int rc = pamg_upload_field(q, field, level, host + off);
      if (rc) return gfail(h, q, rc);
      off += (size_t)q->lev[level - 1].ndof;
    }
    return PAMG_OK;
  }
  if (!valid_level(h, level) || !host) return PAMG_ERR_ARG;
  CK(cudaSetDevice(h->device));
  int rc;
  double* d = field_ptr(h, field, level, true, &rc);
  if (rc) return rc;
  CK(cudaMemcpyAsync(d, host, h->lev[level - 1].ndof * sizeof(double), cudaMemcpyHostToDevice, h->stream));
  CK(cudaStreamSynchronize(h->stream));
  return PAMG_OK;
}

int pamg_download_field(pamg_handle* h, int field, int level, double* host) {
  if (h && h->is_root && host) {
    size_t off = 0;
    for (pamg_handle* q : h->parts) {
      int rc = pamg_download_field(q, field, level, host + off);
      if (rc) return gfail(h, q, rc);
      off += (size_t)q->lev[level - 1].ndof;
    }
    return PAMG_OK;
  }
  if (!valid_level(h, level) || !host) return PAMG_ERR_ARG;
  CK(cudaSetDevice(h->device));
  int rc;
  double* d = field_ptr(h, field, level, false, &rc);
  if (rc) return rc;
  CK(cudaMemcpyAsync(host, d, h->lev[level - 1].ndof * sizeof(double), cudaMemcpyDeviceToHost, h->stream));
  CK(cudaStreamSynchronize(h->stream));
  return p2p_check(h);
}

int pamg_fill_field(pamg_handle* h, int field, int level, double value) {
  FANOUT(h, q, pamg_fill_field(q, field, level, value));
  if (!valid_level(h, level)) return PAMG_ERR_ARG;
  CK(cudaSetDevice(h->device));
  int rc;
  double* d = field_ptr(h, field, level, true, &rc);
  if (rc) return rc;
  return do_fill(h, d, h->lev[level - 1].ndof, value);
}

int pamg_copy_field(pamg_handle* h, int level, int dst_field, int src_field) {
  FANOUT(h, q, pamg_copy_field(q, level, dst_field, src_field));
  if (!valid_level(h, level)) return PAMG_ERR_ARG;
  CK(cudaSetDevice(h->device));
  LevelDev& L = h->lev[level - 1];
  if (dst_field == src_field) return PAMG_OK;
  if (dst_field == PAMG_TNEW && src_field == PAMG_TNONLIN) { L.tnew_alias = true; return PAMG_OK; }
  if (dst_field == PAMG_TNONLIN && src_field == PAMG_TNEW) {
    if (!L.tnew_alias) { L.cur ^= 1; L.tnew_alias = true; L.strips_valid = false; L.cut_valid = false; L.stage_valid = false; }
    return PAMG_OK;
  }
  int rc;
  const double* s = field_ptr(h, src_field, level, false, &rc);
  if (rc) return rc;
  double* d = field_ptr(h, dst_field, level, true, &rc);
  if (rc) return rc;
  CK(cudaMemcpyAsync(d, s, L.ndof * sizeof(double), cudaMemcpyDeviceToDevice, h->stream));
  return PAMG_OK;
}

int pamg_download_overlap(pamg_handle* h, int level, int old, double* host) {
  if (h && h->is_root && host) {
    size_t off = 0;
    for (pamg_handle* q : h->parts) {
      int rc = pamg_download_overlap(q, level, old, host + off);
      if (rc) return gfail(h, q, rc);
      off += (size_t)q->U * 9 * q->lev[level - 1].S;
    }
    return PAMG_OK;
  }
  if (!valid_level(h, level) || !host) return PAMG_ERR_ARG;
  CK(cudaSetDevice(h->device));
  LevelDev& L = h->lev[level - 1];
  const size_t S3 = (size_t)3 * L.S;
  std::vector<double> tmp((size_t)h->plan.nstrips * S3);
  CK(cudaMemcpyAsync(tmp.data(), old ? L.ovl_old : L.ovlb[L.ovl_cur], tmp.size() * sizeof(double), cudaMemcpyDeviceToHost, h->stream));
  CK(cudaStreamSynchronize(h->stream));
  for (int lf = 0; lf < h->U * 3; ++lf)
    std::memcpy(host + (size_t)lf * S3, &tmp[(size_t)h->plan.strip_of[lf] * S3], S3 * sizeof(double));
  return PAMG_OK;
}

int pamg_device_ptr(pamg_handle* h, int field, int level, void** dptr) {
  if (h && h->is_root) return fail(h, PAMG_ERR_UNSUPPORTED, "a multi-GPU handle has no single device pointer per field");
  if (!valid_level(h, level) || !dptr) return PAMG_ERR_ARG;
  int rc;
  *dptr = field_ptr(h, field, level, false, &rc);
  return rc;
}

int pamg_update_overlaps(pamg_handle* h, int level) {
  FANOUT(h, q, pamg_update_overlaps(q, level));
  if (!valid_level(h, level)) return PAMG_ERR_ARG;
  CK(cudaSetDevice(h->device));
  return launch_halo(h, level);
}

int pamg_build_rhs(pamg_handle* h) {
  FANOUT(h, q, pamg_build_rhs(q));
  if (!valid_level(h, 1)) return PAMG_ERR_STATE;
  CK(cudaSetDevice(h->device));
  return launch_build_rhs(h);
}

int pamg_smooth(pamg_handle* h, int level, int solver, int nsweeps) {
  if (h && h->is_root) {
    for (int done = 0; done < nsweeps; done += 4)
      for (pamg_handle* q : h->parts) { int rc = pamg_smooth(q, level, solver, std::min(4, nsweeps - done)); if (rc) return gfail(h, q, rc); }
    return PAMG_OK;
  }
  if (!valid_level(h, level) || nsweeps < 0) return PAMG_ERR_ARG;
  CK(cudaSetDevice(h->device));
  return do_smooth(h, level, solver, nsweeps);
}

int pamg_residual(pamg_handle* h, int level, double* l2, double* linf) {
  if (h && h->is_root) {
    const Group& G = h->parts;
    if (!valid_level(G[0], level)) return PAMG_ERR_ARG;
    double dummy;
    GALL(G, h, q, do_residual(q, level, &dummy, nullptr, nullptr, true));
    return group_norms(G, h, l2, linf, nullptr);
  }
  if (!valid_level(h, level)) return PAMG_ERR_ARG;
  CK(cudaSetDevice(h->device));
  return do_residual(h, level, l2, linf, nullptr);
}

int pamg_convergence(pamg_handle* h, int level, double* conv) {
  if (h && h->is_root && conv) {
    const Group& G = h->parts;
    if (!valid_level(G[0], level)) return PAMG_ERR_ARG;
    double dummy;
    GALL(G, h, q, do_residual(q, level, &dummy, nullptr, nullptr, true));
    return group_norms(G, h, nullptr, nullptr, conv);
  }
  if (!valid_level(h, level) || !conv) return PAMG_ERR_ARG;
  CK(cudaSetDevice(h->device));
  double l2, li;
  return do_residual(h, level, &l2, &li, conv);
}

int pamg_restrict(pamg_handle* h, int fine_level) {
  FANOUT(h, q, pamg_restrict(q, fine_level));
  if (!valid_level(h, fine_level)) return PAMG_ERR_ARG;
  CK(cudaSetDevice(h->device));
  return do_restrict(h, fine_level);
}

int pamg_prolong(pamg_handle* h, int fine_level) {
  FANOUT(h, q, pamg_prolong(q, fine_level));
  if (!valid_level(h, fine_level)) return PAMG_ERR_ARG;
  CK(cudaSetDevice(h->device));
  return do_prolong(h, fine_level);
}

int pamg_vcycle_solve(pamg_handle* h, int solver, int nu1, int nu2, int ncoarse, int max_cycles, double tol,
                      int* cycles, double* hist) {
  if (!h || max_cycles < 0) return PAMG_ERR_ARG;
  const Group G = group_of(h);
  if (!valid_level(G[0], 1)) return PAMG_ERR_ARG;
  CK(cudaSetDevice(G[0]->device));
  int rc;
  for (pamg_handle* q : G) { LevelDev& L = q->lev[0]; L.tnew_alias = true; L.strips_valid = false; L.cut_valid = false; L.stage_valid = false; }
  double r0 = 0, r = 0, dummy;
  GALL(G, h, q, do_residual(q, 1, &dummy, nullptr, nullptr, true));
  if ((rc = group_norms(G, h, &r0, nullptr, nullptr))) return rc;
  if (hist) hist[0] = r0;
  if (cycles) *cycles = 0;
  if (r0 == 0.0) return PAMG_OK;
  bool fuse = solver == 1 && nu1 >= 1 && G[0]->vc_norm_fuse;
  for (pamg_handle* q : G) fuse = fuse && norm_fusable(q, q->lev[0]) && q->halo_mode == 2;
  bool swept = false;
  auto finish = [&]() -> int {
    if (!fuse || !swept) return PAMG_OK;
    for (pamg_handle* q : G) { if (q->in_group) cudaSetDevice(q->device); int rc2 = undo_norm_sweep(q); if (rc2) return gfail(h, q, rc2); }
    GALL(G, h, q, do_residual(q, 1, nullptr, nullptr, nullptr));
    return PAMG_OK;
  };
  const long long key0 = (((((long long)solver * 64 + nu1) * 64 + nu2) * 64 + ncoarse) * 2 + (fuse ? 1 : 0));
  bool graph_ok = h->use_graph;
  for (pamg_handle* q : G) graph_ok = graph_ok && !q->profiling && (!q->comm || q->graph_nccl);
  for (int c = 1; c <= max_cycles; ++c) {
    if (c >= 2 && graph_ok) {
      unsigned long long hk = (unsigned long long)key0;
      for (pamg_handle* q : G) for (auto& Lv : q->lev) hk = hk * 1000003ull + (unsigned long long)(Lv.cur * 2 + Lv.ovl_cur + 1);
      const long long key = (long long)hk;
      pamg_handle::VcGraph* vg = nullptr;
      for (auto& g : h->vc_graphs) if (g.key == key) vg = &g;
      if (!vg) {
        if (h->vc_graphs.size() >= 8) { for (auto e : h->vc_graphs.front().exec) cudaGraphExecDestroy(e); h->vc_graphs.erase(h->vc_graphs.begin()); }
        std::vector<long long> l0(G.size());
        size_t begun = 0;
        cudaError_t ce = cudaSuccess;
        for (; begun < G.size(); ++begun) {
          pamg_handle* q = G[begun];
          if (q->in_group) cudaSetDevice(q->device);
          l0[begun] = q->launches;
          ce = cudaStreamBeginCapture(q->stream, G.size() > 1 ? cudaStreamCaptureModeRelaxed : cudaStreamCaptureModeThreadLocal);
          if (ce != cudaSuccess) break;
          q->capturing = true;
// ... 291 lines not shown
  if (val) {
    k_from_planes<double><<<grid, TPB, 0, h->stream>>>(h->un.bsr_val, h->un.xfer, 36, h->un.E, h->un.ld);
    h->launches++;
    CK(cudaGetLastError());
    CK(cudaMemcpyAsync(val, h->un.xfer, E * 36 * sizeof(double), cudaMemcpyDeviceToHost, h->stream));
  }
  if (col) {
    int32_t* tmp = reinterpret_cast<int32_t*>(h->un.xfer);
    CK(cudaStreamSynchronize(h->stream));
    k_from_planes<int32_t><<<grid, TPB, 0, h->stream>>>(h->un.bsr_col, tmp, 4, h->un.E, h->un.ld);
    h->launches++;
    CK(cudaGetLastError());
    CK(cudaMemcpyAsync(col, tmp, E * 4 * sizeof(int32_t), cudaMemcpyDeviceToHost, h->stream));
  }
  CK(cudaStreamSynchronize(h->stream));
  return PAMG_OK;
}

int pamg_implicit_apply(pamg_handle* h, const double* x, double* y) {
  ON_PART0(h);
  if (!h || h->un.E < 1 || !x || !y) return PAMG_ERR_ARG;
  if (!h->un.assembled) return fail(h, PAMG_ERR_STATE, "pamg_implicit_assemble has not been called");
  CK(cudaSetDevice(h->device));
  const size_t nb = (size_t)h->un.E * 3 * sizeof(double);
  double* W = h->un.work;
  CK(cudaMemcpyAsync(W, x, nb, cudaMemcpyHostToDevice, h->stream));
  const int grid = stream_grid(k_bsr_spmv, h->un.occ_spmv, h->un.E, h->nsm);
  k_bsr_spmv<<<grid, TPB, 0, h->stream>>>(h->un.bsr_val, h->un.bsr_col, W, nullptr, W + (size_t)h->un.E * 3, h->un.E, h->un.ld, 0);
  h->launches++;
  CK(cudaGetLastError());
  CK(cudaMemcpyAsync(y, W + (size_t)h->un.E * 3, nb, cudaMemcpyDeviceToHost, h->stream));
  CK(cudaStreamSynchronize(h->stream));
  return PAMG_OK;
}

int pamg_implicit_set_stab(pamg_handle* h, int with_stab) {
  ON_PART0(h);
  if (!h || h->un.E < 1) return PAMG_ERR_ARG;
  if (!h->un.assembled) return fail(h, PAMG_ERR_STATE, "pamg_implicit_assemble has not been called");
  CK(cudaSetDevice(h->device));
  if (h->un.with_stab && !with_stab)
    return pamg_implicit_assemble_diffusion(h, h->un.dt, h->un.ux, h->un.uy, h->un.kdiff, -1);
  if (with_stab && !h->un.with_stab) {
    const size_t bytes = h->un.ld * 9 * sizeof(double);
    if (!h->un.diag0) CK(cudaMalloc(&h->un.diag0, bytes));
    CK(cudaMemcpyAsync(h->un.diag0, h->un.bsr_val, bytes, cudaMemcpyDeviceToDevice, h->stream));
  }
  h->un.with_stab = with_stab != 0;
  return PAMG_OK;
}

int pamg_unstr_stab(pamg_handle* h, const double* told, double dt, double u_x, double u_y, double* diff_coe, double* stab) {
  ON_PART0(h);
  if (!h || h->un.E < 1 || !told || !(dt > 0.0) || (!diff_coe && !stab)) return PAMG_ERR_ARG;
  CK(cudaSetDevice(h->device));
  const size_t E = (size_t)h->un.E;
  double *d_old = nullptr, *d_out = nullptr;
  CK(cudaMalloc(&d_old, E * 3 * sizeof(double)));
  if (cudaMalloc(&d_out, E * 12 * sizeof(double)) != cudaSuccess) { cudaFree(d_old); return fail(h, PAMG_ERR_CUDA, "cudaMalloc"); }
  cudaMemcpyAsync(d_old, told, E * 3 * sizeof(double), cudaMemcpyHostToDevice, h->stream);
  StabArgs sa;
  sa.X = h->un.X; sa.tnew = h->un.T[h->un.cur]; sa.told = d_old; sa.diff_coe = d_out + E * 9; sa.stab = d_out; sa.diag0 = nullptr;
  sa.val = nullptr; sa.dinv = nullptr; sa.dt = dt; sa.ux = u_x; sa.uy = u_y; sa.ld = h->un.ld; sa.E = h->un.E; sa.mode = 0;
  const int grid = std::max(1, std::min((h->un.E + TPB - 1) / TPB, h->nsm * 8));
  k_unstr_stab<<<grid, TPB, 0, h->stream>>>(sa);
  h->launches++;
  cudaError_t e1 = cudaGetLastError();
  if (stab) cudaMemcpyAsync(stab, d_out, E * 9 * sizeof(double), cudaMemcpyDeviceToHost, h->stream);
  if (diff_coe) cudaMemcpyAsync(diff_coe, d_out + E * 9, E * 3 * sizeof(double), cudaMemcpyDeviceToHost, h->stream);
  cudaError_t e2 = cudaStreamSynchronize(h->stream);
  cudaFree(d_old); cudaFree(d_out);
  if (e1 != cudaSuccess || e2 != cudaSuccess) return fail(h, PAMG_ERR_CUDA, cudaGetErrorString(e1 != cudaSuccess ? e1 : e2));
  return PAMG_OK;
}

int pamg_implicit_step(pamg_handle* h, int ntime, int nits, double tol, int max_iters, int* iters_total, double* relres) {
  ON_PART0(h);
  if (!h || h->un.E < 1 || ntime < 0 || nits < 1 || !(tol > 0.0) || max_iters < 1) return PAMG_ERR_ARG;
  if (!h->un.assembled) return fail(h, PAMG_ERR_STATE, "pamg_implicit_assemble has not been called");
  CK(cudaSetDevice(h->device));
  std::string e;
  long long nl = 0;
  int rc = implicit_step(h->un, ntime, nits, tol, max_iters, iters_total, relres, h->nsm, h->stream, nl, e, &h->un_host_syncs);
  h->launches += nl;
  if (rc) return fail(h, rc, e);
  return PAMG_OK;
}

int pamg_implicit_spmv_time(pamg_handle* h, int reps, float* ms) {
  ON_PART0(h);
  if (!h || h->un.E < 1 || reps < 1 || !ms) return PAMG_ERR_ARG;
  if (!h->un.assembled) return fail(h, PAMG_ERR_STATE, "pamg_implicit_assemble has not been called");
  CK(cudaSetDevice(h->device));
  double* W = h->un.work;
  const size_t n = (size_t)h->un.E * 3;
  const int grid = stream_grid(k_bsr_spmv, h->un.occ_spmv, h->un.E, h->nsm);
  CK(cudaMemcpyAsync(W, h->un.T[h->un.cur], n * sizeof(double), cudaMemcpyDeviceToDevice, h->stream));
  k_bsr_spmv<<<grid, TPB, 0, h->stream>>>(h->un.bsr_val, h->un.bsr_col, W, nullptr, W + n, h->un.E, h->un.ld, 0);
  CK(cudaEventRecord(h->ev[14], h->stream));
  for (int i = 0; i < reps; ++i) k_bsr_spmv<<<grid, TPB, 0, h->stream>>>(h->un.bsr_val, h->un.bsr_col, W, nullptr, W + n, h->un.E, h->un.ld, 0);
  CK(cudaEventRecord(h->ev[15], h->stream));
  h->launches += reps + 1;
  CK(cudaGetLastError());
  CK(cudaEventSynchronize(h->ev[15]));
  CK(cudaEventElapsedTime(ms, h->ev[14], h->ev[15]));
  *ms /= (float)reps;
  return PAMG_OK;
}

int pamg_implicit_host_syncs(pamg_handle* h, int64_t* n) {
  ON_PART0(h);
  if (!h || !n) return PAMG_ERR_ARG;
  *n = h->un_host_syncs;
  return PAMG_OK;
}

int pamg_trans_rec(pamg_handle* h, double CFL, int no_ele_row, int no_ele_col, double x_length, double y_length, double u_x,
                   double u_y, double time, int nits, int njac_its, int direct_solver, int volume_term, double* x_all,
                   double* tnew, int* ntime) {
  ON_PART0(h);
  if (!h || !tnew || no_ele_row < 1 || no_ele_col < 1 || !(CFL > 0.0) || !(x_length > 0.0) || !(y_length > 0.0) || time < 0.0 ||
      nits < 1 || njac_its < 0)
    return PAMG_ERR_ARG;
  CK(cudaSetDevice(h->device));
  std::string e;
  long long nl = 0;
  int rc = rect_run(CFL, no_ele_row, no_ele_col, x_length, y_length, u_x, u_y, time, nits, njac_its, direct_solver, volume_term,
                    x_all, tnew, ntime, h->nsm, h->stream, nl, e);
  h->launches += nl;
  if (rc) return fail(h, rc, e);
  return PAMG_OK;
}

int pamg_apply_local_minv(pamg_handle* h, int n, int batch, const double* M, const double* rhs, double* x,
                          double* Minv, int32_t* status) {
  ON_PART0(h);
  if (!h || batch < 1 || !M || !(n == 3 || n == 4 || n == 6)) return PAMG_ERR_ARG;
  if (!rhs != !x) return PAMG_ERR_ARG;
  CK(cudaSetDevice(h->device));
  std::string e;
  long long nl = 0;
  int rc = local_minv(n, batch, M, rhs, x, Minv, status, h->nsm, h->stream, nl, e);
  h->launches += nl;
  if (rc) return fail(h, rc, e);
  return PAMG_OK;
}

namespace {
int output_fields(pamg_handle* h, double* x_all, double* analytical, double* error) {
  LevelDev& L = h->lev[0];
  const size_t n = (size_t)L.nelem;
  double* d = nullptr;
  CK(cudaMalloc(&d, n * 12 * sizeof(double)));
  OutArgs a;
  a.xg = h->xg; a.T = tnew_ptr(L); a.x_all = x_all ? d : nullptr; a.analytical = analytical ? d + n * 6 : nullptr;
  a.error = error ? d + n * 9 : nullptr; a.nelem = L.nelem; a.s = L.s;
  k_output_fields<<<grid_for(h, L.nelem), TPB, 0, h->stream>>>(a);
  h->launches++;
  cudaError_t e = cudaGetLastError();
  if (x_all) cudaMemcpyAsync(x_all, d, n * 6 * sizeof(double), cudaMemcpyDeviceToHost, h->stream);
  if (analytical) cudaMemcpyAsync(analytical, d + n * 6, n * 3 * sizeof(double), cudaMemcpyDeviceToHost, h->stream);
  if (error) cudaMemcpyAsync(error, d + n * 9, n * 3 * sizeof(double), cudaMemcpyDeviceToHost, h->stream);
  cudaError_t e2 = cudaStreamSynchronize(h->stream);
  cudaFree(d);
  if (e != cudaSuccess || e2 != cudaSuccess) return fail(h, PAMG_ERR_CUDA, cudaGetErrorString(e != cudaSuccess ? e : e2));
  return PAMG_OK;
}
}

int pamg_output_fields(pamg_handle* h, double* x_all, double* analytical, double* error) {
  if (h && h->is_root) {
    size_t off = 0;
    for (pamg_handle* q : h->parts) {
      int rc = pamg_output_fields(q, x_all ? x_all + off * 6 : nullptr, analytical ? analytical + off * 3 : nullptr,
                                  error ? error + off * 3 : nullptr);
      if (rc) return gfail(h, q, rc);
      off += (size_t)q->lev[0].nelem;
    }
    return PAMG_OK;
  }
  if (!h || h->lev.empty() || (!x_all && !analytical && !error)) return PAMG_ERR_ARG;
  CK(cudaSetDevice(h->device));
  return output_fields(h, x_all, analytical, error);
}

int pamg_write_vtu(pamg_handle* h, const char* path, const char* solve_for, int binary) {
  if (!h || !path || !solve_for) return PAMG_ERR_ARG;
  int64_t nd = 0;
  int rc = pamg_ndof(h, 1, &nd);
  if (rc) return rc;
  const size_t n = (size_t)nd / 3;
  std::vector<double> X(n * 6), T(n * 3), An(n * 3), Er(n * 3);
  if ((rc = pamg_output_fields(h, X.data(), An.data(), Er.data()))) return rc;
  if ((rc = pamg_download_field(h, PAMG_TNEW, 1, T.data()))) return rc;
  FILE* f = fopen(path, binary ? "wb" : "w");
  if (!f) return fail(h, PAMG_ERR_IO, std::string("cannot open ") + path);
  const unsigned long long npts = 3ull * n;
  fprintf(f, "<VTKFile type=\"UnstructuredGrid\" version=\"0.1\" byte_order=\"LittleEndian\"%s>\n", binary ? " header_type=\"UInt64\"" : "");
  fprintf(f, "  <UnstructuredGrid>\n    <Piece NumberOfPoints=\"%llu\" NumberOfCells=\"%llu\">\n", npts, (unsigned long long)n);
  fprintf(f, "      <PointData Scalars=\"scalars\">\n");
  if (!binary) {
    const double* arr[3] = {T.data(), Er.data(), An.data()};
    const char* names[3] = {solve_for, "error", "analytical"};
    for (int k = 0; k < 3; ++k) {
      fprintf(f, "        <DataArray type=\"Float32\" Name=\"%s\" Format=\"ascii\">\n", names[k]);
      for (size_t i = 0; i < n * 3; ++i) fprintf(f, k == 0 ? "          %12.10f  \n" : "          %10.7f  \n", arr[k][i]);
      fprintf(f, "        </DataArray>\n");
    }
    fprintf(f, "      </PointData>\n      <Points>\n        <DataArray type=\"Float32\" NumberOfComponents=\"3\" Format=\"ascii\">\n");
    for (size_t i = 0; i < n * 3; ++i) fprintf(f, "          %.3f %.3f %.3f   \n", X[2 * i], X[2 * i + 1], 0.0);
    fprintf(f, "        </DataArray>\n      </Points>\n      <Cells>\n        <DataArray type=\"Int32\" Name=\"connectivity\" Format=\"ascii\">\n");
    for (size_t e = 0; e < n; ++e) fprintf(f, "          %zu %zu %zu\n", 3 * e, 3 * e + 1, 3 * e + 2);
    fprintf(f, "        </DataArray>\n        <DataArray type=\"Int32\" Name=\"offsets\" Format=\"ascii\">\n          ");
    for (size_t e = 1; e <= n; ++e) fprintf(f, e == 1 ? "%zu" : "  %zu", 3 * e);
    fprintf(f, "\n        </DataArray>\n        <DataArray type=\"Int32\" Name=\"types\" Format=\"ascii\">\n          ");
    for (size_t e = 0; e < n; ++e) fprintf(f, e == 0 ? "5" : " 5");
    fprintf(f, "\n        </DataArray>\n      </Cells>\n    </Piece>\n  </UnstructuredGrid>\n</VTKFile>\n");
  } else {
    unsigned long long off = 0;
    const char* names[3] = {solve_for, "error", "analytical"};
    for (int k = 0; k < 3; ++k) {
      fprintf(f, "        <DataArray type=\"Float64\" Name=\"%s\" format=\"appended\" offset=\"%llu\"/>\n", names[k], off);
      off += 8 + npts * 8;
    }
    fprintf(f, "      </PointData>\n      <Points>\n        <DataArray type=\"Float64\" NumberOfComponents=\"3\" format=\"appended\" offset=\"%llu\"/>\n      </Points>\n", off);
    off += 8 + npts * 24;
    fprintf(f, "      <Cells>\n        <DataArray type=\"Int64\" Name=\"connectivity\" format=\"appended\" offset=\"%llu\"/>\n", off);
    off += 8 + npts * 8;
    fprintf(f, "        <DataArray type=\"Int64\" Name=\"offsets\" format=\"appended\" offset=\"%llu\"/>\n", off);
    off += 8 + n * 8;
    fprintf(f, "        <DataArray type=\"UInt8\" Name=\"types\" format=\"appended\" offset=\"%llu\"/>\n", off);
    fprintf(f, "      </Cells>\n    </Piece>\n  </UnstructuredGrid>\n  <AppendedData encoding=\"raw\">\n   _");
    auto block = [&](const void* p, unsigned long long bytes) { fwrite(&bytes, 8, 1, f); fwrite(p, 1, bytes, f); };
    block(T.data(), npts * 8); block(Er.data(), npts * 8); block(An.data(), npts * 8);
    std::vector<double> P3(npts * 3);
    for (size_t i = 0; i < npts; ++i) { P3[3 * i] = X[2 * i]; P3[3 * i + 1] = X[2 * i + 1]; P3[3 * i + 2] = 0.0; }
    block(P3.data(), npts * 24);
    std::vector<long long> conn(npts), offs(n);
    for (size_t i = 0; i < npts; ++i) conn[i] = (long long)i;
    for (size_t e = 0; e < n; ++e) offs[e] = 3ll * (long long)(e + 1);
    block(conn.data(), npts * 8); block(offs.data(), n * 8);
    std::vector<unsigned char> types(n, 5);
    block(types.data(), n);
    fprintf(f, "\n  </AppendedData>\n</VTKFile>\n");
  }
  if (fclose(f) != 0) return fail(h, PAMG_ERR_IO, std::string("write failed: ") + path);
  return PAMG_OK;
}

int pamg_sync(pamg_handle* h) {
  if (!h) return PAMG_ERR_ARG;
  FANOUT(h, q, pamg_sync(q));
  CK(cudaSetDevice(h->device));
  CK(cudaStreamSynchronize(h->stream));
  if (h->up_stream) { CK(cudaStreamSynchronize(h->up_stream)); CK(cudaStreamSynchronize(h->down_stream)); h->pipe_calls = 0; h->last_out = nullptr; }
  return p2p_check(h);
}

int pamg_event_record(pamg_handle* h, int slot) {
  if (!h || slot < 0 || slot >= 16) return PAMG_ERR_ARG;
  FANOUT(h, q, pamg_event_record(q, slot));
  CK(cudaSetDevice(h->device));
  CK(cudaEventRecord(h->ev[slot], h->stream));
  return PAMG_OK;
}

int pamg_event_elapsed_ms(pamg_handle* h, int a, int b, float* ms) {
  if (!h || !ms || a < 0 || a >= 16 || b < 0 || b >= 16) return PAMG_ERR_ARG;
  if (h->is_root) {
    *ms = 0.f;
    for (pamg_handle* q : h->parts) { float m = 0.f; int rc = pamg_event_elapsed_ms(q, a, b, &m); if (rc) return gfail(h, q, rc); *ms = std::max(*ms, m); }
    return PAMG_OK;
  }
  CK(cudaSetDevice(h->device));
  CK(cudaEventSynchronize(h->ev[b]));
  CK(cudaEventElapsedTime(ms, h->ev[a], h->ev[b]));
  return PAMG_OK;
}

int pamg_launch_count(const pamg_handle* h, int64_t* n) {
  if (!h || !n) return PAMG_ERR_ARG;
  *n = h->launches;
  for (const pamg_handle* q : h->parts) *n += q->launches;
  return PAMG_OK;
}

int pamg_profile(pamg_handle* h, int on) {
  if (!h) return PAMG_ERR_ARG;
  FANOUT(h, q, pamg_profile(q, on));
  CK(cudaSetDevice(h->device));
  if (on && h->pev.empty()) {
    h->pev.resize(2048);
    for (auto& e : h->pev) CK(cudaEventCreate(&e));
  }
  h->profiling = on != 0;
  h->pev_used = 0;
  return PAMG_OK;
}

int pamg_profile_read(pamg_handle* h, double* total_ms, int* launches) {
  if (!h || !total_ms || !launches) return PAMG_ERR_ARG;
  if (h->is_root) {
    *total_ms = 0.0; *launches = 0;
    for (pamg_handle* q : h->parts) { double t = 0; int l = 0; int rc = pamg_profile_read(q, &t, &l); if (rc) return gfail(h, q, rc); *total_ms += t; *launches += l; }
    return PAMG_OK;
  }
// ... 35 lines not shown
```

### p-a_multigrids_b200/csrc/pamg_kernels.cuh

```cuda
#pragma once
#include <cstdint>

namespace pamg {

constexpr int NPC = 88;
constexpr int PC_FOLD = 24;
constexpr int PC_DPEN = 56;
constexpr int PC_WB = 60;
enum { PC_CM = 0, PC_K11 = 1, PC_K12, PC_K13, PC_K22, PC_K23, PC_K33, PC_ADV = 7, PC_FL = 10, PC_PENI = 13, PC_W = 16, PC_PENX = 19 };

constexpr int TPB = 256;

enum { MODE_JACOBI = 0, MODE_RESID = 1, MODE_GS = 2, MODE_RICH = 3 };

constexpr int P2P_SLOTS = 4;
constexpr int P2P_MAXP = 16;
enum { P2P_EPOCH = 0, P2P_COUNT = 1, P2P_WORDS = 8 };
struct P2PArgs {
  const double* send;
  int send_base;
  double* strips;
  uint4* remote[P2P_MAXP];
  long long rstride[P2P_MAXP];
  long long soff[P2P_MAXP + 1];
  long long rbeg[P2P_MAXP];
  long long roff[P2P_MAXP + 1];
  uint4* stage;
  long long stage_words;
  unsigned long long* sync;
  unsigned long long* err;
  int npeers;
  unsigned long long timeout_ns;
};

__device__ __forceinline__ unsigned long long p2p_now() {
  unsigned long long t;
  asm volatile("mov.u64 %0, %%globaltimer;" : "=l"(t));
  return t;
}

__device__ __forceinline__ void p2p_put(const P2PArgs& a, unsigned e, int p, long long idx, double val) {
  const unsigned long long v = (unsigned long long)__double_as_longlong(val);
  asm volatile("st.volatile.global.v4.u32 [%0], {%1, %2, %3, %4};" ::"l"(a.remote[p] + (long long)(e & (P2P_SLOTS - 1)) * a.rstride[p] + idx), "r"((unsigned)v), "r"(e),
               "r"((unsigned)(v >> 32)), "r"(e) : "memory");
}


struct ElemArgs {
  const double* Tin;
  double* Tout;
  const double* rhs;
  const double* ovl;
  const double* pc;
  const int32_t* strip_of;
  const int32_t* hmap;
  const int32_t* nsrc;
  double* ovl_next;
  const int32_t* dst_strip;
  const int32_t* rev;
  int nstrips;
  const ulonglong2* xsend;
  unsigned long long* xsync;
  double* partial;
  double omega;
  double rsign;
  long long nelem;
  int s;
  int colour;
  int partial_off;
};

__host__ __device__ __forceinline__ void child_from_flat(int t, int s, int& r, int& ipos, int& ele, int& len) {
  const int b = 2 << s;
  const int S = 1 << s;
  const int p = t >> (s + 1);
  const int q = t & (b - 1);
  const int lenA = b - 1 - 2 * p;
  if (q < lenA) { r = p + 1; ipos = q + 1; len = lenA; }
  else { r = S - p; ipos = q - lenA + 1; len = 2 * p + 1; }
  ele = 1 + (r - 1) * (b + 1 - r) + ipos - 1;
}

struct FaceIn { double n1a, n1b, n2a, n2b, n3a, n3b, pen1, pen2, pen3; };

template <int MODE, bool FACE>
__device__ __forceinline__ void elem_apply(const double* __restrict__ pc, bool up, double T1, double T2, double T3,
                                           const FaceIn& fi, double b1, double b2, double b3, double omega,
                                           double rsign, double& o1, double& o2, double& o3) {
  const double sg = up ? 1.0 : -1.0;
  const double cm = __ldg(pc + PC_CM);
  const double sumT = T1 + T2 + T3;
  const double k11 = __ldg(pc + PC_K11), k12 = __ldg(pc + PC_K12), k13 = __ldg(pc + PC_K13);
  const double k22 = __ldg(pc + PC_K22), k23 = __ldg(pc + PC_K23), k33 = __ldg(pc + PC_K33);
  const double adv = sg * sumT;
  const double mass1 = cm * (T1 + sumT), mass2 = cm * (T2 + sumT), mass3 = cm * (T3 + sumT);
  const double st1 = __ldg(pc + PC_ADV + 0) * adv, st2 = __ldg(pc + PC_ADV + 1) * adv, st3 = __ldg(pc + PC_ADV + 2) * adv;
  double ax1 = mass1 - st1 + (k11 * T1 + k12 * T2 + k13 * T3);
  double ax2 = mass2 - st2 + (k12 * T1 + k22 * T2 + k23 * T3);
  double ax3 = mass3 - st3 + (k13 * T1 + k23 * T2 + k33 * T3);
  double d1 = 4.0 * cm + k11, d2 = 4.0 * cm + k22, d3 = 4.0 * cm + k33;
  double fx1 = 0.0, fx2 = 0.0, fx3 = 0.0;
  if (FACE) {
    {
      const double da = T1 - fi.n1a, db = T3 - fi.n1b;
      ax1 += fi.pen1 * (2.0 * da + db); ax3 += fi.pen1 * (da + 2.0 * db);
      d1 += 2.0 * fi.pen1; d3 += 2.0 * fi.pen1;
    }
    {
      const double da = T3 - fi.n2a, db = T2 - fi.n2b;
      ax3 += fi.pen2 * (2.0 * da + db); ax2 += fi.pen2 * (da + 2.0 * db);
      d3 += 2.0 * fi.pen2; d2 += 2.0 * fi.pen2;
    }
    {
      const double da = T2 - fi.n3a, db = T1 - fi.n3b;
      ax2 += fi.pen3 * (2.0 * da + db); ax1 += fi.pen3 * (da + 2.0 * db);
      d2 += 2.0 * fi.pen3; d1 += 2.0 * fi.pen3;
    }
    {
      const double fl = sg * __ldg(pc + PC_FL + 0);
      const bool in = fl < 0.0;
      const double wa = in ? fi.n1a : T1, wb = in ? fi.n1b : T3;
      fx1 += fl * (2.0 * wa + wb); fx3 += fl * (wa + 2.0 * wb);
    }
    {
      const double fl = sg * __ldg(pc + PC_FL + 1);
      const bool in = fl < 0.0;
      const double wa = in ? fi.n2a : T3, wb = in ? fi.n2b : T2;
      fx3 += fl * (2.0 * wa + wb); fx2 += fl * (wa + 2.0 * wb);
    }
    {
      const double fl = sg * __ldg(pc + PC_FL + 2);
      const bool in = fl < 0.0;
      const double wa = in ? fi.n3a : T2, wb = in ? fi.n3b : T1;
      fx2 += fl * (2.0 * wa + wb); fx1 += fl * (wa + 2.0 * wb);
    }
    ax1 += fx1; ax2 += fx2; ax3 += fx3;
  }
  if (MODE == MODE_RESID) {
    o1 = rsign * (ax1 - b1); o2 = rsign * (ax2 - b2); o3 = rsign * (ax3 - b3);
  } else if (MODE == MODE_RICH) {
    o1 = T1 + omega * (b1 - (mass1 - st1 + fx1));
    o2 = T2 + omega * (b2 - (mass2 - st2 + fx2));
    o3 = T3 + omega * (b3 - (mass3 - st3 + fx3));
  } else {
    o1 = T1 + omega / d1 * (b1 - ax1);
    o2 = T2 + omega / d2 * (b2 - ax2);
    o3 = T3 + omega / d3 * (b3 - ax3);
  }
}

__host__ __device__ __forceinline__ size_t nbr_child_offset(int d, int p, int s) {
  const int S = 1 << s, b = 2 << s;
  const int m = (d & 16) ? (S - 1 - p) : p;
  const int ns = (d >> 5) & 3;
  const int e0 = (ns == 0) ? 2 * m : (m * (b - m) + (ns == 1 ? b - 2 - 2 * m : 0));
  return ((((size_t)(d >> 7)) << (2 * s)) + (size_t)e0) * 3;
}
__device__ __forceinline__ void nbr_pair(const double* __restrict__ T, int d, int p, int s, double& va, double& vb) {
  const size_t o = nbr_child_offset(d, p, s);
  va = __ldg(T + o + (d & 3)); vb = __ldg(T + o + ((d >> 2) & 3));
}

__device__ __forceinline__ void ext_pair(const ElemArgs& a, int d, int strip, int hm, int p, int S, double& va, double& vb) {
  if (d >= 0) { nbr_pair(a.Tin, d, p, a.s, va, vb); return; }
  const double* e = a.ovl + ((size_t)strip * S + p) * 3;
  va = __ldg(e + (hm & 3)); vb = __ldg(e + (hm >> 2));
}

__device__ __forceinline__ void halo_pair(const ElemArgs& a, int u, int mf, int slot0, int S, double& va, double& vb) {
  const int d = a.nsrc ? __ldg(a.nsrc + u * 3 + mf) : -1;
  ext_pair(a, d, __ldg(a.strip_of + u * 3 + mf), __ldg(a.hmap + u * 3 + mf), slot0, S, va, vb);
}

__device__ __forceinline__ void p2p_advance(unsigned long long* sync, unsigned long long e64) {
  if (atomicAdd(sync + P2P_COUNT, 1ull) == (unsigned long long)gridDim.x - 1) {
    sync[P2P_COUNT] = 0;
    *(volatile unsigned long long*)(sync + P2P_EPOCH) = e64 + 1;
  }
}

__device__ __forceinline__ void block_partial(double acc_sum, double acc_abs, double acc_max, double* partial) {
  for (int o = 16; o > 0; o >>= 1) {
    acc_sum += __shfl_xor_sync(0xffffffffu, acc_sum, o);
    acc_abs = fmax(acc_abs, __shfl_xor_sync(0xffffffffu, acc_abs, o));
    acc_max = fmax(acc_max, __shfl_xor_sync(0xffffffffu, acc_max, o));
  }
  __shared__ double sh[3][TPB / 32];
  const int w = threadIdx.x >> 5, l = threadIdx.x & 31;
  if (l == 0) { sh[0][w] = acc_sum; sh[1][w] = acc_abs; sh[2][w] = acc_max; }
  __syncthreads();
  if (threadIdx.x == 0) {
    double s0 = 0, s1 = 0, s2 = 0;
    for (int i = 0; i < TPB / 32; ++i) { s0 += sh[0][i]; s1 = fmax(s1, sh[1][i]); s2 = fmax(s2, sh[2][i]); }
    partial[(size_t)blockIdx.x * 3 + 0] = s0;
    partial[(size_t)blockIdx.x * 3 + 1] = s1;
    partial[(size_t)blockIdx.x * 3 + 2] = s2;
  }
}

__device__ __forceinline__ uint32_t smem_u32(const void* p) { return (uint32_t)__cvta_generic_to_shared(p); }
__device__ __forceinline__ void mbar_init(uint64_t* bar, int count) {
  asm volatile("mbarrier.init.shared::cta.b64 [%0], %1;" ::"r"(smem_u32(bar)), "r"(count) : "memory");
}
__device__ __forceinline__ void mbar_expect_tx(uint64_t* bar, uint32_t bytes) {
  asm volatile("mbarrier.arrive.expect_tx.shared::cta.b64 _, [%0], %1;" ::"r"(smem_u32(bar)), "r"(bytes) : "memory");
}
__device__ __forceinline__ void mbar_wait(uint64_t* bar, uint32_t parity) {
  asm volatile(
      "{\n"
      ".reg .pred p;\n"
      "LAB_WAIT_%=:\n"
      "mbarrier.try_wait.parity.shared::cta.b64 p, [%0], %1;\n"
      "@p bra LAB_DONE_%=;\n"
      "bra LAB_WAIT_%=;\n"
      "LAB_DONE_%=:\n"
      "}\n" ::"r"(smem_u32(bar)), "r"(parity) : "memory");
}
__device__ __forceinline__ void tma_load_1d(void* smem_dst, const void* gsrc, uint32_t bytes, uint64_t* bar) {
  asm volatile("cp.async.bulk.shared::cluster.global.mbarrier::complete_tx::bytes [%0], [%1], %2, [%3];" ::"r"(
                   smem_u32(smem_dst)), "l"(gsrc), "r"(bytes), "r"(smem_u32(bar)) : "memory");
}
__device__ __forceinline__ void tma_store_1d(void* gdst, const void* smem_src, uint32_t bytes) {
  asm volatile("cp.async.bulk.global.shared::cta.bulk_group [%0], [%1], %2;" ::"l"(gdst), "r"(smem_u32(smem_src)),
               "r"(bytes) : "memory");
}
__device__ __forceinline__ void tma_store_commit() { asm volatile("cp.async.bulk.commit_group;" ::: "memory"); }
__device__ __forceinline__ void tma_store_wait_read() { asm volatile("cp.async.bulk.wait_group.read 0;" ::: "memory"); }
__device__ __forceinline__ void tma_store_wait_all() { asm volatile("cp.async.bulk.wait_group 0;" ::: "memory"); }
__device__ __forceinline__ void fence_async_smem() { asm volatile("fence.proxy.async.shared::cta;" ::: "memory"); }

__host__ __device__ __forceinline__ void child_from_ele0(int k, int s, int& r, int& ipos, int& len) {
  const int b = 2 << s, S = 1 << s;
  int m = (int)(((float)b - sqrtf((float)(b * b - 4 * k))) * 0.5f);
  m = max(0, min(m, S - 1));
  m -= (m * (b - m) > k);
  m += (m + 1 < S) && ((m + 1) * (b - m - 1) <= k);
  m -= (m * (b - m) > k);
  r = m + 1;
  ipos = k - m * (b - m) + 1;
  len = b + 1 - 2 * r;
}

__host__ __device__ __forceinline__ void child_advance(int s, int b, int k_next, int& r, int& ipos) {
  if (k_next < TPB) { int len; child_from_ele0(k_next, s, r, ipos, len); return; }
  ipos += TPB;
  int len = b + 1 - 2 * r;
  while (ipos > len) { ipos -= len; len -= 2; ++r; }
}

constexpr int TMA_T_DOUBLES = 3 * TPB + 8;
constexpr int NSTAGE = 3;
constexpr size_t TMA_SMEM_BYTES = sizeof(double) * (NSTAGE * (TMA_T_DOUBLES + 3 * TPB) + 2 * 3 * TPB) + 16 * NSTAGE + 64;

struct ParentRegs {
  double cm, k11, k12, k13, k22, k23, k33, adv1, adv2, adv3, fl1, fl2, fl3, pi1, pi2, pi3;
  double w1, w2, w3;
  double px1, px2, px3;
};
static_assert(sizeof(ParentRegs) == 22 * sizeof(double), "ParentRegs must mirror the pc table");
__device__ __forceinline__ void load_parent(const double* __restrict__ pc, ParentRegs& P) {
  double* d = reinterpret_cast<double*>(&P);
#pragma unroll
  for (int i = 0; i < 22; ++i) d[i] = __ldg(pc + i);
}

struct Folded { double a11, a12, a13, a21, a22, a23, a31, a32, a33, c1, c2, c3, w1, w2, w3, pad; };
static_assert(sizeof(Folded) == 16 * sizeof(double), "Folded layout");

template <int MODE, bool WITH_R = false>
__device__ __forceinline__ void elem_apply_folded(const Folded& F, const double* ext, int mask, double T1, double T2,
                                                  double T3, const FaceIn& fi, double b1, double b2, double b3,
                                                  double rsign, double& o1, double& o2, double& o3, double* rr = nullptr) {
  double ax1 = F.a11 * T1 + F.a12 * T2 + F.a13 * T3;
  double ax2 = F.a21 * T1 + F.a22 * T2 + F.a23 * T3;
  double ax3 = F.a31 * T1 + F.a32 * T2 + F.a33 * T3;
  ax1 += F.c1 * (2.0 * fi.n1a + fi.n1b); ax3 += F.c1 * (fi.n1a + 2.0 * fi.n1b);
  ax3 += F.c2 * (2.0 * fi.n2a + fi.n2b); ax2 += F.c2 * (fi.n2a + 2.0 * fi.n2b);
  ax2 += F.c3 * (2.0 * fi.n3a + fi.n3b); ax1 += F.c3 * (fi.n3a + 2.0 * fi.n3b);
  double w1 = F.w1, w2 = F.w2, w3 = F.w3;
  if (mask) {
    if (mask & 1) { const double dp = ext[0], da = T1 - fi.n1a, db = T3 - fi.n1b; ax1 += dp * (2.0 * da + db); ax3 += dp * (da + 2.0 * db); }
    if (mask & 2) { const double dp = ext[1], da = T3 - fi.n2a, db = T2 - fi.n2b; ax3 += dp * (2.0 * da + db); ax2 += dp * (da + 2.0 * db); }
    if (mask & 4) { const double dp = ext[2], da = T2 - fi.n3a, db = T1 - fi.n3b; ax2 += dp * (2.0 * da + db); ax1 += dp * (da + 2.0 * db); }
    const double* wb = ext + 4 + mask * 3;
    w1 = wb[0]; w2 = wb[1]; w3 = wb[2];
  }
  if (WITH_R) { rr[0] = rsign * (ax1 - b1); rr[1] = rsign * (ax2 - b2); rr[2] = rsign * (ax3 - b3); }
  if (MODE == MODE_RESID) {
    o1 = rsign * (ax1 - b1); o2 = rsign * (ax2 - b2); o3 = rsign * (ax3 - b3);
  } else {
    o1 = T1 + w1 * (b1 - ax1); o2 = T2 + w2 * (b2 - ax2); o3 = T3 + w3 * (b3 - ax3);
  }
}

template <int MODE, bool FACE>
__device__ __forceinline__ void elem_apply_regs(const ParentRegs& P, bool up, bool interior, double T1, double T2,
                                                double T3, const FaceIn& fi, double b1, double b2, double b3,
                                                double omega, double rsign, double& o1, double& o2, double& o3) {
  const double sg = up ? 1.0 : -1.0;
  const double sumT = T1 + T2 + T3;
  const double adv = sg * sumT;
  const double mass1 = P.cm * (T1 + sumT), mass2 = P.cm * (T2 + sumT), mass3 = P.cm * (T3 + sumT);
  const double st1 = P.adv1 * adv, st2 = P.adv2 * adv, st3 = P.adv3 * adv;
  double ax1 = mass1 - st1 + (P.k11 * T1 + P.k12 * T2 + P.k13 * T3);
  double ax2 = mass2 - st2 + (P.k12 * T1 + P.k22 * T2 + P.k23 * T3);
  double ax3 = mass3 - st3 + (P.k13 * T1 + P.k23 * T2 + P.k33 * T3);
  double fx1 = 0.0, fx2 = 0.0, fx3 = 0.0;
  if (FACE) {
    {
      const double da = T1 - fi.n1a, db = T3 - fi.n1b;
      ax1 += fi.pen1 * (2.0 * da + db); ax3 += fi.pen1 * (da + 2.0 * db);
    }
    {
      const double da = T3 - fi.n2a, db = T2 - fi.n2b;
      ax3 += fi.pen2 * (2.0 * da + db); ax2 += fi.pen2 * (da + 2.0 * db);
    }
    {
      const double da = T2 - fi.n3a, db = T1 - fi.n3b;
      ax2 += fi.pen3 * (2.0 * da + db); ax1 += fi.pen3 * (da + 2.0 * db);
// ... 239 lines not shown
        const int mf = (p.ipos == 1) ? 2 : 1;
        const int strip = same ? sIdx[mf] : __ldg(a.strip_of + u * 3 + mf), hm = same ? sIdx[4 + mf] : __ldg(a.hmap + u * 3 + mf);
        const int d = same ? sIdx[8 + mf] : (a.nsrc ? __ldg(a.nsrc + u * 3 + mf) : -1);
        ext_pair(a, d, strip, hm, p.r - 1, S, p.h2a, p.h2b);
      }
    }
  };
  Prep cur, nxt;
  prepare(tbeg, cur);
  for (long long tile = tbeg; tile < tend; ++tile) {
    const int it = (int)(tile - tbeg);
    const long long g0 = tile * TPB;
    if (tid == 0) {
      if (tile + 5 < thi) issueT(tile + 5);
      if (tile + 2 < tend) { tma_store_wait_read1(); issueB(tile + 2); }
    }
    {
      const int u_tile = (int)(g0 >> twos);
      if (u_tile != u_loaded) {
        __syncthreads();
        if (tid < NPC) sPC[tid] = __ldg(a.pc + (size_t)u_tile * NPC + tid);
        else if (tid < NPC + 3) sIdx[tid - NPC] = __ldg(a.strip_of + u_tile * 3 + (tid - NPC));
        else if (tid < NPC + 6) sIdx[4 + tid - NPC - 3] = __ldg(a.hmap + u_tile * 3 + (tid - NPC - 3));
        else if (tid < NPC + 9) sIdx[8 + tid - NPC - 6] = a.nsrc ? __ldg(a.nsrc + u_tile * 3 + (tid - NPC - 6)) : -1;
        __syncthreads();
        u_loaded = u_tile;
      }
    }
    prepare(tile + 1, nxt);
    if (it == 0) {
      for (long long tw = tlo; tw <= min(tile + 2, thi - 1); ++tw) mbar_wait(&barT[tw & (WIN_NT - 1)], (uint32_t)(((tw - tlo) >> 3) & 1));
    } else if (tile + 2 < thi) {
      mbar_wait(&barT[(tile + 2) & (WIN_NT - 1)], (uint32_t)(((tile + 2 - tlo) >> 3) & 1));
    }
    mbar_wait(&barB[it & (WIN_NB - 1)], (uint32_t)((it / WIN_NB) & 1));
    double* bb = sB + (it & (WIN_NB - 1)) * 3 * TPB + tid * 3;
    {
      const int cw = (int)(g0 & (WIN_CH - 1)) + tid;
      const double* t = sT + cw * 3;
      const double T1 = t[0], T2 = t[1], T3 = t[2];
      const bool up = cur.ipos & 1;
      double o1, o2, o3;
      if (MODE == MODE_GS && (int)up != a.colour) {
        o1 = T1; o2 = T2; o3 = T3;
      } else {
        FaceIn fi;
        int bmask = 0;
        bool interior = true;
        const ParentRegs& P = *reinterpret_cast<const ParentRegs*>(sPC);
        if (FACE) {
          fi.pen1 = P.pi1; fi.pen2 = P.pi2; fi.pen3 = P.pi3;
          const int dv = up ? (2 * cur.r - b - 2) : (b - 2 * cur.r);
          const double* tv = sT + ((cw + dv) & (WIN_CH - 1)) * 3;
          fi.n1a = tv[2]; fi.n1b = tv[0];
          const double* tl = sT + ((cw - 1) & (WIN_CH - 1)) * 3;
          const double* tr = sT + ((cw + 1) & (WIN_CH - 1)) * 3;
          const double* t2 = up ? tl : tr;
          const double* t3 = up ? tr : tl;
          fi.n2a = t2[1]; fi.n2b = t2[2];
          fi.n3a = t3[0]; fi.n3b = t3[1];
          if (up && (cur.r == 1 || cur.ipos == 1 || cur.ipos == cur.len)) {
            interior = false;
            if (cur.r == 1) { fi.n1a = cur.h1a; fi.n1b = cur.h1b; fi.pen1 = P.px1; bmask |= 1; }
            if (cur.ipos == 1) { fi.n2a = cur.h2a; fi.n2b = cur.h2b; fi.pen2 = P.px2; bmask |= 2; }
            if (cur.ipos == cur.len) {
              if (cur.len == 1) halo_pair(a, (int)(g0 >> twos), 1, cur.r - 1, S, fi.n3a, fi.n3b);
              else { fi.n3a = cur.h2a; fi.n3b = cur.h2b; }
              fi.pen3 = P.px3; bmask |= 4;
            }
          }
        }
        if (FACE && MODE != MODE_RICH) {
          const Folded& F = *reinterpret_cast<const Folded*>(sPC + PC_FOLD + (up ? 0 : 16));
          elem_apply_folded<MODE>(F, sPC + PC_DPEN, bmask, T1, T2, T3, fi, bb[0], bb[1], bb[2], a.rsign, o1, o2, o3);
        } else {
          elem_apply_regs<MODE, FACE>(P, up, interior, T1, T2, T3, fi, bb[0], bb[1], bb[2], a.omega, a.rsign, o1, o2, o3);
        }
      }
      bb[0] = o1; bb[1] = o2; bb[2] = o3;
      if (MODE == MODE_RESID) {
        acc_sum += o1 * o1 + o2 * o2 + o3 * o3;
        acc_abs = fmax(acc_abs, fmax(fabs(o1), fmax(fabs(o2), fabs(o3))));
        acc_max = fmax(acc_max, fmax(o1, fmax(o2, o3)));
      }
    }
    fence_async_smem();
    __syncthreads();
    if (tid == 0) {
      tma_store_1d(a.Tout + g0 * 3, sB + (it & (WIN_NB - 1)) * 3 * TPB, TILE_BYTES);
      tma_store_commit();
    }
    cur = nxt;
  }
  if (tid == 0) tma_store_wait_all();
  if (MODE == MODE_RESID) block_partial(acc_sum, acc_abs, acc_max, a.partial + (size_t)3 * a.partial_off);
}

struct StripDst { int d0, d1, d2, rv; uint4 *r0, *r1, *r2; };
__device__ __forceinline__ StripDst strip_dst_load(const ElemArgs& a, int u, int lane, unsigned long long xe = 0) {
  int d = 0, rv = 0;
  unsigned long long r = 0;
  if (lane < 3) {
    d = __ldg(a.dst_strip + u * 3 + lane); rv = __ldg(a.rev + u * 3 + lane) << lane;
    if (xe != 0) {
      const ulonglong2 t = __ldg(a.xsend + u * 3 + lane);
      if (t.x) r = t.x + (xe & (P2P_SLOTS - 1)) * t.y * sizeof(uint4);
    }
  }
  StripDst o;
  o.d0 = __shfl_sync(0xffffffffu, d, 0); o.d1 = __shfl_sync(0xffffffffu, d, 1); o.d2 = __shfl_sync(0xffffffffu, d, 2);
  o.rv = __shfl_sync(0xffffffffu, rv, 0) | __shfl_sync(0xffffffffu, rv, 1) | __shfl_sync(0xffffffffu, rv, 2);
  o.r0 = (uint4*)__shfl_sync(0xffffffffu, r, 0); o.r1 = (uint4*)__shfl_sync(0xffffffffu, r, 1); o.r2 = (uint4*)__shfl_sync(0xffffffffu, r, 2);
  return o;
}

__device__ __forceinline__ void strips_from_tile(const ElemArgs& a, const double* __restrict__ tile, const StripDst& sd, int k0,
                                                 int s, int& m0, int lane, unsigned long long xe = 0) {
  const int S = 1 << s, b = 2 << s;
  const int kend = k0 + TPB;
  auto put = [&](int dst, uint4* rbase, int rvf, int pos, int k) {
    const int slot = rvf ? (S - 1 - pos) : pos;
    const double* t = tile + (k - k0) * 3;
    if (rbase != nullptr) {
      const unsigned e = (unsigned)xe;
#pragma unroll
      for (int i = 0; i < 3; ++i) {
        const unsigned long long v = (unsigned long long)__double_as_longlong(t[i]);
        asm volatile("st.volatile.global.v4.u32 [%0], {%1, %2, %3, %4};" ::"l"(rbase + slot * 3 + i), "r"((unsigned)v), "r"(e), "r"((unsigned)(v >> 32)), "r"(e) : "memory");
      }
      return;
    }
    double* e = a.ovl_next + ((size_t)dst * S + slot) * 3;
    e[0] = t[0]; e[1] = t[1]; e[2] = t[2];
  };
  if (sd.d0 >= 0 && k0 < b - 1) {
    const int e1 = min(kend, b - 1);
    for (int k = k0 + 2 * lane; k < e1; k += 64) put(sd.d0, sd.r0, sd.rv & 1, k >> 1, k);
  }
  while ((m0 + 1) * (b - m0 - 1) <= k0) ++m0;
  if (sd.d1 >= 0 || sd.d2 >= 0) {
    for (int m = m0 + lane; m < S; m += 32) {
      const int first = m * (b - m);
      if (first >= kend) break;
      const int last = (m + 1) * (b - m - 1) - 1;
      if (sd.d2 >= 0 && first >= k0) put(sd.d2, sd.r2, sd.rv & 4, m, first);
      if (sd.d1 >= 0 && last < kend) put(sd.d1, sd.r1, sd.rv & 2, m, last);
    }
  }
}

constexpr int WIN2_THREADS = TPB + 32;
__device__ __forceinline__ void named_arrive(int id, int count) { asm volatile("bar.arrive %0, %1;" ::"r"(id), "r"(count) : "memory"); }
__device__ __forceinline__ void named_sync(int id, int count) { asm volatile("bar.sync %0, %1;" ::"r"(id), "r"(count) : "memory"); }

template <int MODE, bool FACE, bool XCHG = false, bool NORM = false>
__global__ void __launch_bounds__(WIN2_THREADS, 3) k_element_win2(ElemArgs a) {
  extern __shared__ __align__(128) unsigned char dsm[];
  double* sT = reinterpret_cast<double*>(dsm);
  double* sB = sT + 3 * WIN_CH;
  uint64_t* barT = reinterpret_cast<uint64_t*>(sB + 3 * TPB * WIN_NB);
  uint64_t* barB = barT + WIN_NT;
  __shared__ __align__(16) double sPC2[2][NPC];
  __shared__ int sIdx2[2][12];
  __shared__ double shp[3][TPB / 32];
  const int s = a.s, twos = 2 * s, b = 2 << s, S = 1 << s;
  const long long Cmask = (1ll << twos) - 1;
  const int tid = threadIdx.x;
  constexpr uint32_t TILE_BYTES = 3 * TPB * sizeof(double);
  double acc_sum = 0.0, acc_abs = 0.0, acc_max = 0.0;
  if (tid == 0) {
    for (int i = 0; i < WIN_NT + WIN_NB; ++i) mbar_init(&barT[i], 1);
    asm volatile("fence.mbarrier_init.release.cluster;" ::: "memory");
  }
  __syncthreads();
  const long long ntiles = a.nelem / TPB;
  const long long per = (ntiles + gridDim.x - 1) / gridDim.x;
  const long long tbeg = (long long)blockIdx.x * per, tend = min(ntiles, tbeg + per);
  const long long tlo = max(0ll, tbeg - 2), thi = min(ntiles, tend + 2);

  if (tid >= TPB) {
    const int lane = tid - TPB;
    int u_loaded = -1;
    unsigned long long e64 = 0;
    if (XCHG) e64 = *(volatile unsigned long long*)(a.xsync + P2P_EPOCH);
    auto issueT = [&](long long tile) {
      const int sl = (int)(tile & (WIN_NT - 1));
      mbar_expect_tx(&barT[sl], TILE_BYTES);
      tma_load_1d(sT + sl * 3 * TPB, a.Tin + tile * 3 * TPB, TILE_BYTES, &barT[sl]);
    };
    auto issueB = [&](long long tile) {
      const int u = (int)((tile * TPB) >> twos);
      if (u != u_loaded) {
        for (int i = lane; i < NPC; i += 32) sPC2[u & 1][i] = __ldg(a.pc + (size_t)u * NPC + i);
        if (lane < 3) {
          sIdx2[u & 1][lane] = __ldg(a.strip_of + u * 3 + lane); sIdx2[u & 1][4 + lane] = __ldg(a.hmap + u * 3 + lane);
          sIdx2[u & 1][8 + lane] = a.nsrc ? __ldg(a.nsrc + u * 3 + lane) : -1;
        }
        u_loaded = u;
        __syncwarp();
      }
      if (lane == 0) {
        const int sl = (int)((tile - tbeg) & (WIN_NB - 1));
        mbar_expect_tx(&barB[sl], TILE_BYTES);
        tma_load_1d(sB + sl * 3 * TPB, a.rhs + tile * 3 * TPB, TILE_BYTES, &barB[sl]);
      }
    };
    if (tbeg < tend) {
      if (lane == 0) for (long long t = tlo; t < min(thi, tbeg + 6); ++t) issueT(t);
      for (long long t = tbeg; t < min(tend, tbeg + 3); ++t) issueB(t);
    }
    int m0 = 0, u_m0 = -1;
    StripDst sd = {-1, -1, -1, 0, nullptr, nullptr, nullptr};
    for (long long p = tbeg; p < tend; ++p) {
      const int it = (int)(p - tbeg);
      named_sync(1 + (it & 3), WIN2_THREADS);
      if (lane == 0) {
        tma_store_1d(a.Tout + p * 3 * TPB, sB + (it & (WIN_NB - 1)) * 3 * TPB, TILE_BYTES);
        tma_store_commit();
        if (p + 6 < thi) issueT(p + 6);
        if (p + 3 < tend) tma_store_wait_read1();
      }
      __syncwarp();
      if (p + 3 < tend) issueB(p + 3);
      if (MODE != MODE_RESID && a.ovl_next) {
        const int u = (int)((p * TPB) >> twos);
        if (u != u_m0) { m0 = 0; u_m0 = u; sd = strip_dst_load(a, u, lane, XCHG ? e64 + 1 : 0); }
        strips_from_tile(a, sB + (it & (WIN_NB - 1)) * 3 * TPB, sd, (int)((p * TPB) & Cmask), s, m0, lane, XCHG ? e64 + 1 : 0);
      }
    }
    if (XCHG && MODE != MODE_RESID && lane == 0) p2p_advance(a.xsync, e64);
    if (lane == 0) tma_store_wait_all();
  } else {
    const int tbegi = (int)tbeg, tendi = (int)tend, tloi = (int)tlo, thii = (int)thi;
    const int pshift = twos - 8;
    const unsigned kmask = (unsigned)Cmask;
    struct Prep { int r, ipos, len; double h1a, h1b, h2a, h2b; };
    auto prepare = [&](int tile, int u_cur, bool first, Prep& p) {
      p.h1a = 0.0; p.h1b = 0.0; p.h2a = 0.0; p.h2b = 0.0;
      if (tile >= tendi) return;
      const int kk = (int)((((unsigned)tile << 8) + (unsigned)tid) & kmask);
      if (first) child_from_ele0(kk, s, p.r, p.ipos, p.len);
      else child_advance(s, b, kk, p.r, p.ipos);
      p.len = b + 1 - 2 * p.r;
      if (!FACE || !(p.ipos & 1)) return;
      const bool f1 = p.r == 1, side = p.ipos == 1 || p.ipos == p.len;
      if (f1 | side) {
        const int u = tile >> pshift;
        const bool same = u == u_cur;
        const int* ix = sIdx2[u & 1];
        if (f1) {
          const int strip = same ? ix[0] : __ldg(a.strip_of + u * 3), hm = same ? ix[4] : __ldg(a.hmap + u * 3);
          const int d = same ? ix[8] : (a.nsrc ? __ldg(a.nsrc + u * 3) : -1);
          ext_pair(a, d, strip, hm, p.ipos >> 1, S, p.h1a, p.h1b);
        }
        if (side) {
          const int mf = (p.ipos == 1) ? 2 : 1;
          const int strip = same ? ix[mf] : __ldg(a.strip_of + u * 3 + mf), hm = same ? ix[4 + mf] : __ldg(a.hmap + u * 3 + mf);
          const int d = same ? ix[8 + mf] : (a.nsrc ? __ldg(a.nsrc + u * 3 + mf) : -1);
          ext_pair(a, d, strip, hm, p.r - 1, S, p.h2a, p.h2b);
        }
      }
    };
    Prep cur, nxt;
    cur.r = 2; cur.ipos = 2; cur.len = 3;
    prepare(tbegi, -1, true, cur);
    for (int tile = tbegi; tile < tendi; ++tile) {
      const int it = tile - tbegi;
      const int u_tile = tile >> pshift;
      if (it == 0) {
        for (int tw = tloi; tw <= min(tile + 2, thii - 1); ++tw) mbar_wait(&barT[tw & (WIN_NT - 1)], (uint32_t)(((tw - tloi) >> 3) & 1));
      } else if (tile + 2 < thii) {
        mbar_wait(&barT[(tile + 2) & (WIN_NT - 1)], (uint32_t)(((tile + 2 - tloi) >> 3) & 1));
      }
      mbar_wait(&barB[it & (WIN_NB - 1)], (uint32_t)((it / WIN_NB) & 1));
      nxt.r = cur.r; nxt.ipos = cur.ipos;
      prepare(tile + 1, u_tile, false, nxt);
      const double* sPC = sPC2[u_tile & 1];
      double* bb = sB + (it & (WIN_NB - 1)) * (3 * TPB) + tid * 3;
      {
        const int cw = ((tile & (WIN_NT - 1)) << 8) + tid;
        const double* t = sT + cw * 3;
        const double T1 = t[0], T2 = t[1], T3 = t[2];
        const bool up = cur.ipos & 1;
        double o1, o2, o3;
        FaceIn fi;
        int bmask = 0;
        bool interior = true;
        const ParentRegs& P = *reinterpret_cast<const ParentRegs*>(sPC);
        if (FACE) {
          fi.pen1 = P.pi1; fi.pen2 = P.pi2; fi.pen3 = P.pi3;
          const int dv = up ? (2 * cur.r - b - 2) : (b - 2 * cur.r);
          const double* tv = sT + ((cw + dv) & (WIN_CH - 1)) * 3;
          fi.n1a = tv[2]; fi.n1b = tv[0];
          const double* tl = sT + ((cw - 1) & (WIN_CH - 1)) * 3;
          const double* tr = sT + ((cw + 1) & (WIN_CH - 1)) * 3;
          const double* t2 = up ? tl : tr;
          const double* t3 = up ? tr : tl;
          fi.n2a = t2[1]; fi.n2b = t2[2];
          fi.n3a = t3[0]; fi.n3b = t3[1];
          if (up && (cur.r == 1 || cur.ipos == 1 || cur.ipos == cur.len)) {
            interior = false;
            if (cur.r == 1) { fi.n1a = cur.h1a; fi.n1b = cur.h1b; fi.pen1 = P.px1; bmask |= 1; }
            if (cur.ipos == 1) { fi.n2a = cur.h2a; fi.n2b = cur.h2b; fi.pen2 = P.px2; bmask |= 2; }
            if (cur.ipos == cur.len) {
              if (cur.len == 1) halo_pair(a, u_tile, 1, cur.r - 1, S, fi.n3a, fi.n3b);
              else { fi.n3a = cur.h2a; fi.n3b = cur.h2b; }
              fi.pen3 = P.px3; bmask |= 4;
            }
          }
        }
        if (FACE && MODE != MODE_RICH) {
          const Folded& F = *reinterpret_cast<const Folded*>(sPC + PC_FOLD + (up ? 0 : 16));
          if (NORM) {
            double rr[3];
            elem_apply_folded<MODE, true>(F, sPC + PC_DPEN, bmask, T1, T2, T3, fi, bb[0], bb[1], bb[2], a.rsign, o1, o2, o3, rr);
            acc_sum += rr[0] * rr[0] + rr[1] * rr[1] + rr[2] * rr[2];
            acc_abs = fmax(acc_abs, fmax(fabs(rr[0]), fmax(fabs(rr[1]), fabs(rr[2]))));
            acc_max = fmax(acc_max, fmax(rr[0], fmax(rr[1], rr[2])));
          } else {
            elem_apply_folded<MODE>(F, sPC + PC_DPEN, bmask, T1, T2, T3, fi, bb[0], bb[1], bb[2], a.rsign, o1, o2, o3);
          }
        } else {
          elem_apply_regs<MODE, FACE>(P, up, interior, T1, T2, T3, fi, bb[0], bb[1], bb[2], a.omega, a.rsign, o1, o2, o3);
        }
        bb[0] = o1; bb[1] = o2; bb[2] = o3;
        if (MODE == MODE_RESID) {
          acc_sum += o1 * o1 + o2 * o2 + o3 * o3;
          acc_abs = fmax(acc_abs, fmax(fabs(o1), fmax(fabs(o2), fabs(o3))));
          acc_max = fmax(acc_max, fmax(o1, fmax(o2, o3)));
        }
      }
      fence_async_smem();
      named_arrive(1 + (it & 3), WIN2_THREADS);
      cur = nxt;
    }
  }
  if (MODE == MODE_RESID || NORM) {
    if (tid < TPB) {
      for (int o = 16; o > 0; o >>= 1) {
        acc_sum += __shfl_xor_sync(0xffffffffu, acc_sum, o);
        acc_abs = fmax(acc_abs, __shfl_xor_sync(0xffffffffu, acc_abs, o));
        acc_max = fmax(acc_max, __shfl_xor_sync(0xffffffffu, acc_max, o));
      }
      if ((tid & 31) == 0) { shp[0][tid >> 5] = acc_sum; shp[1][tid >> 5] = acc_abs; shp[2][tid >> 5] = acc_max; }
    }
    __syncthreads();
    if (tid == 0) {
      double s0 = 0, s1 = 0, s2 = 0;
      for (int i = 0; i < TPB / 32; ++i) { s0 += shp[0][i]; s1 = fmax(s1, shp[1][i]); s2 = fmax(s2, shp[2][i]); }
      double* partial = a.partial + (size_t)3 * a.partial_off;
      partial[(size_t)blockIdx.x * 3 + 0] = s0; partial[(size_t)blockIdx.x * 3 + 1] = s1; partial[(size_t)blockIdx.x * 3 + 2] = s2;
    }
  }
}

constexpr size_t GSW_SMEM_BYTES = WIN_SMEM_BYTES;
__device__ __forceinline__ void tma_store_wait_read2() { asm volatile("cp.async.bulk.wait_group.read 2;" ::: "memory"); }

__global__ void __launch_bounds__(TPB, 3) k_gs_win(ElemArgs a) {
  extern __shared__ __align__(128) unsigned char dsm[];
  double* sT = reinterpret_cast<double*>(dsm);
  double* sB = sT + 3 * WIN_CH;
  uint64_t* barT = reinterpret_cast<uint64_t*>(sB + 3 * TPB * WIN_NB);
  uint64_t* barB = barT + WIN_NT;
  __shared__ __align__(16) double sPC[NPC];
  __shared__ __align__(16) double sPD[16];
  __shared__ int sIdx[12];
  const int s = a.s, twos = 2 * s, b = 2 << s, S = 1 << s;
  const long long Cmask = (1ll << twos) - 1;
  const int tid = threadIdx.x;
  constexpr uint32_t TILE_BYTES = 3 * TPB * sizeof(double);
  if (tid == 0) {
    for (int i = 0; i < WIN_NT + WIN_NB; ++i) mbar_init(&barT[i], 1);
    asm volatile("fence.mbarrier_init.release.cluster;" ::: "memory");
  }
  __syncthreads();
  const long long ntiles = a.nelem / TPB;
  const long long per = (ntiles + gridDim.x - 1) / gridDim.x;
  const long long tbeg = (long long)blockIdx.x * per, tend = min(ntiles, tbeg + per);
  if (tbeg >= tend) return;
  const long long dlo = max(0ll, tbeg - 2), dhi = min(ntiles - 1, tend);
  const long long tlo = max(0ll, dlo - 1), thi = min(ntiles, dhi + 3);
  const long long t0 = dlo - 2;

  auto issueT = [&](long long tile) {
    const int sl = (int)(tile & (WIN_NT - 1));
    mbar_expect_tx(&barT[sl], TILE_BYTES);
    tma_load_1d(sT + sl * 3 * TPB, a.Tin + tile * 3 * TPB, TILE_BYTES, &barT[sl]);
  };
  auto issueB = [&](long long tile) {
    const int sl = (int)((tile - dlo) & (WIN_NB - 1));
    mbar_expect_tx(&barB[sl], TILE_BYTES);
    tma_load_1d(sB + sl * 3 * TPB, a.rhs + tile * 3 * TPB, TILE_BYTES, &barB[sl]);
  };
  auto waitT = [&](long long tile) { mbar_wait(&barT[tile & (WIN_NT - 1)], (uint32_t)(((tile - tlo) >> 3) & 1)); };
  auto waitB = [&](long long tile) { mbar_wait(&barB[(tile - dlo) & (WIN_NB - 1)], (uint32_t)(((tile - dlo) >> 2) & 1)); };
  if (tid == 0) {
    for (long long t = tlo; t < min(thi, t0 + 6); ++t) issueT(t);
    for (long long t = dlo; t <= min(dhi, dlo + 3); ++t) issueB(t);
  }

  int u_up = -1, u_dn = -1;
  struct Prep { int r, ipos, len; double h1a, h1b, h2a, h2b; };
  auto prepare = [&](long long tile, Prep& p) {
    p.r = 2; p.ipos = 2; p.len = 3; p.h1a = 0.0; p.h1b = 0.0; p.h2a = 0.0; p.h2b = 0.0;
    if (tile < tbeg || tile >= tend) return;
    const long long g = tile * TPB + tid;
    child_from_ele0((int)(g & Cmask), s, p.r, p.ipos, p.len);
    if (!(p.ipos & 1)) return;
    const bool f1 = p.r == 1, side = p.ipos == 1 || p.ipos == p.len;
    if (f1 | side) {
      const int u = (int)(g >> twos);
      const bool same = u == u_up;
      if (f1) {
        const int strip = same ? sIdx[0] : __ldg(a.strip_of + u * 3), hm = same ? sIdx[4] : __ldg(a.hmap + u * 3);
        const int d = same ? sIdx[8] : (a.nsrc ? __ldg(a.nsrc + u * 3) : -1);
        ext_pair(a, d, strip, hm, p.ipos >> 1, S, p.h1a, p.h1b);
      }
      if (side) {
        const int mf = (p.ipos == 1) ? 2 : 1;
        const int strip = same ? sIdx[mf] : __ldg(a.strip_of + u * 3 + mf), hm = same ? sIdx[4 + mf] : __ldg(a.hmap + u * 3 + mf);
        const int d = same ? sIdx[8 + mf] : (a.nsrc ? __ldg(a.nsrc + u * 3 + mf) : -1);
        ext_pair(a, d, strip, hm, p.r - 1, S, p.h2a, p.h2b);
      }
    }
  };
  Prep cur, nxt;
  prepare(t0, cur);
  for (long long tile = t0; tile < tend; ++tile) {
    const long long td = tile + 2;
    const bool doD = td >= dlo && td <= dhi, doU = tile >= tbeg;
    if (tid == 0 && tile > t0) {
      if (tile + 5 < thi) { tma_store_wait_read2(); issueT(tile + 5); }
      if (td + 1 >= dlo + 4 && td + 1 <= dhi) issueB(td + 1);
    }
    {
      const int ud = doD ? (int)((td * TPB) >> twos) : u_dn;
      const int uu = doU ? (int)((tile * TPB) >> twos) : u_up;
      if (ud != u_dn || uu != u_up) {
        __syncthreads();
        if (uu != u_up) {
          if (tid < NPC) sPC[tid] = __ldg(a.pc + (size_t)uu * NPC + tid);
          else if (tid < NPC + 3) sIdx[tid - NPC] = __ldg(a.strip_of + uu * 3 + (tid - NPC));
          else if (tid < NPC + 6) sIdx[4 + tid - NPC - 3] = __ldg(a.hmap + uu * 3 + (tid - NPC - 3));
          else if (tid < NPC + 9) sIdx[8 + tid - NPC - 6] = a.nsrc ? __ldg(a.nsrc + uu * 3 + (tid - NPC - 6)) : -1;
        }
        if (ud != u_dn && tid >= 128 && tid < 144) sPD[tid - 128] = __ldg(a.pc + (size_t)ud * NPC + PC_FOLD + 16 + (tid - 128));
        __syncthreads();
        u_dn = ud; u_up = uu;
      }
    }
    prepare(tile + 1, nxt);
    if (tile == t0) {
      for (long long tw = tlo; tw < min(thi, tile + 5); ++tw) waitT(tw);
    } else if (tile + 4 < thi) {
      waitT(tile + 4);
    }
    if (doD) {
      waitB(td);
      const long long g = td * TPB + tid;
      int r, ipos, len;
      child_from_ele0((int)(g & Cmask), s, r, ipos, len);
      if (!(ipos & 1)) {
        const int cw = (int)((td * TPB) & (WIN_CH - 1)) + tid;
        double* t = sT + cw * 3;
        const double T1 = t[0], T2 = t[1], T3 = t[2];
        FaceIn fi;
        const double* tv = sT + ((cw + b - 2 * r) & (WIN_CH - 1)) * 3;
        fi.n1a = tv[2]; fi.n1b = tv[0];
        const double* tr = sT + ((cw + 1) & (WIN_CH - 1)) * 3;
        const double* tl = sT + ((cw - 1) & (WIN_CH - 1)) * 3;
        fi.n2a = tr[1]; fi.n2b = tr[2];
        fi.n3a = tl[0]; fi.n3b = tl[1];
        const double* bb = sB + ((td - dlo) & (WIN_NB - 1)) * 3 * TPB + tid * 3;
        const Folded& F = *reinterpret_cast<const Folded*>(sPD);
        double o1, o2, o3;
        elem_apply_folded<MODE_GS>(F, sPD, 0, T1, T2, T3, fi, bb[0], bb[1], bb[2], a.rsign, o1, o2, o3);
        t[0] = o1; t[1] = o2; t[2] = o3;
      }
    }
    if (doU) {
      if (cur.ipos & 1) {
        const int cw = (int)((tile * TPB) & (WIN_CH - 1)) + tid;
        double* t = sT + cw * 3;
        const double T1 = t[0], T2 = t[1], T3 = t[2];
        FaceIn fi;
        int bmask = 0;
        const double* tv = sT + ((cw + 2 * cur.r - b - 2) & (WIN_CH - 1)) * 3;
        fi.n1a = tv[2]; fi.n1b = tv[0];
        const double* tl = sT + ((cw - 1) & (WIN_CH - 1)) * 3;
        const double* tr = sT + ((cw + 1) & (WIN_CH - 1)) * 3;
        fi.n2a = tl[1]; fi.n2b = tl[2];
        fi.n3a = tr[0]; fi.n3b = tr[1];
        if (cur.r == 1 || cur.ipos == 1 || cur.ipos == cur.len) {
          if (cur.r == 1) { fi.n1a = cur.h1a; fi.n1b = cur.h1b; bmask |= 1; }
          if (cur.ipos == 1) { fi.n2a = cur.h2a; fi.n2b = cur.h2b; bmask |= 2; }
          if (cur.ipos == cur.len) {
            if (cur.len == 1) halo_pair(a, (int)((tile * TPB) >> twos), 1, cur.r - 1, S, fi.n3a, fi.n3b);
            else { fi.n3a = cur.h2a; fi.n3b = cur.h2b; }
            bmask |= 4;
          }
        }
        const double* bb = sB + ((tile - dlo) & (WIN_NB - 1)) * 3 * TPB + tid * 3;
        const Folded& F = *reinterpret_cast<const Folded*>(sPC + PC_FOLD);
        double o1, o2, o3;
        elem_apply_folded<MODE_GS>(F, sPC + PC_DPEN, bmask, T1, T2, T3, fi, bb[0], bb[1], bb[2], a.rsign, o1, o2, o3);
        t[0] = o1; t[1] = o2; t[2] = o3;
      }
    }
    fence_async_smem();
    __syncthreads();
    if (tid == 0 && doU) {
      tma_store_1d(a.Tout + tile * 3 * TPB, sT + (tile & (WIN_NT - 1)) * 3 * TPB, TILE_BYTES);
      tma_store_commit();
    }
    cur = nxt;
  }
  if (tid == 0) tma_store_wait_all();
}

__device__ __forceinline__ void mbar_arrive_cta(uint64_t* bar) {
  asm volatile("mbarrier.arrive.release.cta.shared::cta.b64 _, [%0];" ::"r"(smem_u32(bar)) : "memory");
}

template <bool XCHG>
__global__ void __launch_bounds__(WIN2_THREADS, 3) k_gs_win2(ElemArgs a) {
  extern __shared__ __align__(128) unsigned char dsm[];
  double* sT = reinterpret_cast<double*>(dsm);
  double* sB = sT + 3 * WIN_CH;
  uint64_t* barT = reinterpret_cast<uint64_t*>(sB + 3 * TPB * WIN_NB);
  uint64_t* barB = barT + WIN_NT;
  __shared__ __align__(16) double sPC2[2][NPC];
  __shared__ int sIdx2[2][12];
  __shared__ __align__(8) uint64_t doneD[4];
  const int s = a.s, twos = 2 * s, b = 2 << s, S = 1 << s;
  const long long Cmask = (1ll << twos) - 1;
  const int tid = threadIdx.x;
  constexpr uint32_t TILE_BYTES = 3 * TPB * sizeof(double);
  if (tid == 0) {
    for (int i = 0; i < WIN_NT + WIN_NB; ++i) mbar_init(&barT[i], 1);
    for (int i = 0; i < 4; ++i) mbar_init(&doneD[i], TPB / 64);
    asm volatile("fence.mbarrier_init.release.cluster;" ::: "memory");
  }
  __syncthreads();
  const long long ntiles = a.nelem / TPB;
  const long long per = (ntiles + gridDim.x - 1) / gridDim.x;
  const long long tbeg = (long long)blockIdx.x * per, tend = min(ntiles, tbeg + per);
  if (tbeg >= tend) {
    if (XCHG && tid == TPB) p2p_advance(a.xsync, *(volatile unsigned long long*)(a.xsync + P2P_EPOCH));
    return;
  }
  const long long dlo = max(0ll, tbeg - 2), dhi = min(ntiles - 1, tend);
  const long long tlo = max(0ll, dlo - 1), thi = min(ntiles, dhi + 3);
  const long long t0 = dlo - 1;

  if (tid >= TPB) {
    const int lane = tid - TPB;
    int u_loaded = -1;
    unsigned long long e64 = 0;
    if (XCHG) e64 = *(volatile unsigned long long*)(a.xsync + P2P_EPOCH);
    auto issueT = [&](long long tile) {
      const int sl = (int)(tile & (WIN_NT - 1));
      mbar_expect_tx(&barT[sl], TILE_BYTES);
      tma_load_1d(sT + sl * 3 * TPB, a.Tin + tile * 3 * TPB, TILE_BYTES, &barT[sl]);
    };
    auto issueB = [&](long long tile) {
      const int u = (int)((tile * TPB) >> twos);
      if (u != u_loaded) {
        for (int i = lane; i < NPC; i += 32) sPC2[u & 1][i] = __ldg(a.pc + (size_t)u * NPC + i);
        if (lane < 3) {
          sIdx2[u & 1][lane] = __ldg(a.strip_of + u * 3 + lane); sIdx2[u & 1][4 + lane] = __ldg(a.hmap + u * 3 + lane);
          sIdx2[u & 1][8 + lane] = a.nsrc ? __ldg(a.nsrc + u * 3 + lane) : -1;
        }
        u_loaded = u;
        __syncwarp();
      }
      if (lane == 0) {
        const int sl = (int)((tile - dlo) & (WIN_NB - 1));
        mbar_expect_tx(&barB[sl], TILE_BYTES);
        tma_load_1d(sB + sl * 3 * TPB, a.rhs + tile * 3 * TPB, TILE_BYTES, &barB[sl]);
      }
    };
    if (lane == 0) for (long long t = tlo; t < min(thi, t0 + 6); ++t) issueT(t);
    for (long long t = dlo; t <= min(dhi, dlo + 3); ++t) issueB(t);
    int m0 = 0, u_m0 = -1;
    StripDst sd = {-1, -1, -1, 0, nullptr, nullptr, nullptr};
    for (long long tile = t0; tile < tend; ++tile) {
      const int it = (int)(tile - t0);
      named_sync(1 + (it & 3), WIN2_THREADS);
      if (lane == 0) {
        if (tile >= tbeg) {
          tma_store_1d(a.Tout + tile * 3 * TPB, sT + (tile & (WIN_NT - 1)) * 3 * TPB, TILE_BYTES);
          tma_store_commit();
        }
        if (tile + 6 < thi) { asm volatile("cp.async.bulk.wait_group.read 2;" ::: "memory"); issueT(tile + 6); }
      }
      __syncwarp();
      if (tile + 4 >= dlo + 4 && tile + 4 <= dhi) issueB(tile + 4);
      if (a.ovl_next && tile >= tbeg) {
        const int u = (int)((tile * TPB) >> twos);
        if (u != u_m0) { m0 = 0; u_m0 = u; sd = strip_dst_load(a, u, lane, XCHG ? e64 + 1 : 0); }
        strips_from_tile(a, sT + (tile & (WIN_NT - 1)) * 3 * TPB, sd, (int)((tile * TPB) & Cmask), s, m0, lane, XCHG ? e64 + 1 : 0);
      }
    }
    if (XCHG && lane == 0) p2p_advance(a.xsync, e64);
    if (lane == 0) tma_store_wait_all();
  } else {
    const int t0i = (int)t0, tbegi = (int)tbeg, tendi = (int)tend, dloi = (int)dlo, dhii = (int)dhi, tloi = (int)tlo, thii = (int)thi;
    const int pshift = twos - 8;
    const unsigned kmask = (unsigned)Cmask;
    auto waitT = [&](int tile) { mbar_wait(&barT[tile & (WIN_NT - 1)], (uint32_t)(((tile - tloi) >> 3) & 1)); };
    auto waitB = [&](int tile) { mbar_wait(&barB[(tile - dloi) & (WIN_NB - 1)], (uint32_t)(((tile - dloi) >> 2) & 1)); };
    const int j2 = (tid & (TPB / 2 - 1)) * 2;
    int r = 2, ipos = 2;
    auto relax_up = [&](int tile, int cw, int rr, int ip, int ln, double h1a, double h1b, double h2a, double h2b) {
      const int u_tile = tile >> pshift;
      double* t = sT + cw * 3;
      const double T1 = t[0], T2 = t[1], T3 = t[2];
      FaceIn fi;
      int bmask = 0;
      const double* tv = sT + ((cw + 2 * rr - b - 2) & (WIN_CH - 1)) * 3;
      fi.n1a = tv[2]; fi.n1b = tv[0];
      const double* tl = sT + ((cw - 1) & (WIN_CH - 1)) * 3;
      const double* tr = sT + ((cw + 1) & (WIN_CH - 1)) * 3;
      fi.n2a = tl[1]; fi.n2b = tl[2];
      fi.n3a = tr[0]; fi.n3b = tr[1];
      if (rr == 1 || ip == 1 || ip == ln) {
        if (rr == 1) { fi.n1a = h1a; fi.n1b = h1b; bmask |= 1; }
        if (ip == 1) { fi.n2a = h2a; fi.n2b = h2b; bmask |= 2; }
        if (ip == ln) {
          if (ln == 1) halo_pair(a, u_tile, 1, rr - 1, S, fi.n3a, fi.n3b);
          else { fi.n3a = h2a; fi.n3b = h2b; }
          bmask |= 4;
        }
      }
      const double* bb = sB + ((tile - dloi) & (WIN_NB - 1)) * (3 * TPB) + (cw & (TPB - 1)) * 3;
      const double* pu = sPC2[u_tile & 1];
      const Folded& F = *reinterpret_cast<const Folded*>(pu + PC_FOLD);
      double o1, o2, o3;
      elem_apply_folded<MODE_GS>(F, pu + PC_DPEN, bmask, T1, T2, T3, fi, bb[0], bb[1], bb[2], a.rsign, o1, o2, o3);
      t[0] = o1; t[1] = o2; t[2] = o3;
    };
    if (tid < TPB / 2) {
      bool sec = false;
      int sec_r = 0;
      double sec_a = 0.0, sec_b = 0.0;
      for (int tile = t0i; tile < tendi; ++tile) {
        const int it = tile - t0i;
        const int td = tile + 1;
        bool nsec = false;
        double nsec_a = 0.0, nsec_b = 0.0;
        if (tile == t0i) {
          for (int tw = tloi; tw < min(thii, tile + 4); ++tw) waitT(tw);
        } else if (tile + 3 < thii) {
          waitT(tile + 3);
        }
        if (td >= dloi && td <= dhii) {
          waitB(td);
          const int k = (int)((((unsigned)td << 8) + (unsigned)j2) & kmask);
          if (td == dloi) { int len; child_from_ele0(k, s, r, ipos, len); }
          else child_advance(s, b, k, r, ipos);
          const int off = ipos & 1;
          if (!off || ipos < b + 1 - 2 * r) {
            const int cw = ((td & (WIN_NT - 1)) << 8) + j2 + off;
            double* t = sT + cw * 3;
            const double T1 = t[0], T2 = t[1], T3 = t[2];
            FaceIn fi;
            const double* tv = sT + ((cw + b - 2 * r) & (WIN_CH - 1)) * 3;
            fi.n1a = tv[2]; fi.n1b = tv[0];
            const double* tr = sT + ((cw + 1) & (WIN_CH - 1)) * 3;
            const double* tl = sT + ((cw - 1) & (WIN_CH - 1)) * 3;
            fi.n2a = tr[1]; fi.n2b = tr[2];
            fi.n3a = tl[0]; fi.n3b = tl[1];
            const double* bb = sB + ((td - dloi) & (WIN_NB - 1)) * (3 * TPB) + (j2 + off) * 3;
            const double* pd = sPC2[(td >> pshift) & 1] + PC_FOLD + 16;
            const Folded& F = *reinterpret_cast<const Folded*>(pd);
// ... 565 lines not shown
```

Measured before the change: 252.7 billion.

## Fuse two Jacobi sweeps per kernel via shared-memory temporal blocking

Adds a k_jacobi_pair kernel that performs two Jacobi sweeps in one pass: one warp group relaxes tiles into a shared-memory intermediate buffer and a second group relaxes again from it, with a producer warp streaming tiles via TMA and writing the next halo strips. A separate boundary-sweep kernel precomputes the intermediate halo values into a new ovl_mid buffer. The aim is to halve global memory traffic per sweep for fine levels. Because the batching step advances the loop by four sweeps while only two pair launches run, the final sweep is deferred and completed lazily through tnew_resolve with an extra launch and copy. This adds complexity, shared-memory pressure at one block per SM, and correctness risk around the deferred state.

```diff
diff --git a/p-a_multigrids_b200/csrc/pamg_api.cu b/p-a_multigrids_b200/csrc/pamg_api.cu
--- a/p-a_multigrids_b200/csrc/pamg_api.cu
+++ b/p-a_multigrids_b200/csrc/pamg_api.cu
@@ -70,6 +70,10 @@
   double* pc_old = nullptr;
   bool rhs_valid = false;
   double* spare = nullptr;
+  double* ovl_mid = nullptr;
+  double* tmid = nullptr;
+  bool tnew_pending = false;
+  const double* tnew_ovl = nullptr;
 };
 
 struct pamg_handle {
@@ -95,7 +99,7 @@
   int kernel_mode = 4;
   int halo_mode = 2;
   long long debug_gap_ns = 0;
-  struct KernelCfg { int win2[2] = {0, 0}, win2x = 0, win[2] = {0, 0}, tma[2] = {0, 0}, gs2 = 0, gs2x = 0, gs = 0, halo = 0; bool done = false; } kc;
+  struct KernelCfg { int win2[2] = {0, 0}, win2x = 0, win[2] = {0, 0}, tma[2] = {0, 0}, gs2 = 0, gs2x = 0, gs = 0, halo = 0, pair = 0; bool done = false; } kc;
   bool capturing = false;
   bool use_graph = true;
   struct VcGraph { long long key; std::vector<cudaGraphExec_t> exec; std::vector<long long> launches; };
@@ -168,10 +172,13 @@
 
 double* tnew_ptr(LevelDev& L) { return L.tnew_alias ? L.T[L.cur] : L.T[L.cur ^ 1]; }
 
+int tnew_resolve(pamg_handle* h, LevelDev& L);
+
 int materialise_tnew(pamg_handle* h, LevelDev& L) {
-  if (!L.tnew_alias) return PAMG_OK;
+  if (!L.tnew_alias) return tnew_resolve(h, L);
   CK(cudaMemcpyAsync(L.T[L.cur ^ 1], L.T[L.cur], L.ndof * sizeof(double), cudaMemcpyDeviceToDevice, h->stream));
   L.tnew_alias = false;
+  L.tnew_ovl = nullptr;
   return PAMG_OK;
 }
 
@@ -180,7 +187,11 @@
   LevelDev& L = h->lev[level - 1];
   switch (field) {
     case PAMG_TNEW:
-      if (for_write) { *rc = materialise_tnew(h, L); L.strips_valid = false; L.cut_valid = false; L.stage_valid = false; return L.T[L.cur ^ 1]; }
+      if (for_write) {
+        *rc = materialise_tnew(h, L); L.strips_valid = false; L.cut_valid = false; L.stage_valid = false; L.tnew_ovl = nullptr;
+        return L.T[L.cur ^ 1];
+      }
+      *rc = tnew_resolve(h, L);
       return tnew_ptr(L);
     case PAMG_TNONLIN:
       if (for_write) { *rc = materialise_tnew(h, L); L.strips_valid = false; L.cut_valid = false; L.stage_valid = false; }
@@ -442,6 +453,7 @@
 
 int launch_halo(pamg_handle* h, int level, int what) {
   LevelDev& L = h->lev[level - 1];
+  if (int rc = tnew_resolve(h, L)) return rc;
   HaloArgs a;
   a.tnew = tnew_ptr(L); a.told = L.told; a.ovl = L.ovlb[L.ovl_cur]; a.ovl_old = L.ovl_old; a.xg = h->xg;
   a.dst_strip = h->dst_strip; a.rev = h->rev; a.strip_of = h->strip_of;
@@ -552,6 +564,7 @@
   if ((rc = configure_one(h, k_gs_win2<false>, WIN2_THREADS, GSW_SMEM_BYTES, h->kc.gs2))) return rc;
   if ((rc = configure_one(h, k_gs_win2<true>, WIN2_THREADS, GSW_SMEM_BYTES, h->kc.gs2x))) return rc;
   if ((rc = configure_one(h, k_gs_win, TPB, GSW_SMEM_BYTES, h->kc.gs))) return rc;
+  if ((rc = configure_one(h, k_jacobi_pair, PAIR_THREADS, PAIR_SMEM_BYTES, h->kc.pair))) return rc;
   CK(cudaOccupancyMaxActiveBlocksPerMultiprocessor(&h->kc.halo, k_halo, TPB, 0));
   if (h->kc.halo < 1) h->kc.halo = 1;
   cudaFuncAttributes fa;
@@ -710,13 +723,73 @@
   return h->p.face_terms && h->kernel_mode == 4 && h->win_producer && L.s >= 6 && L.s <= 8;
 }
 
+bool pair_level(const pamg_handle* h, int s) {
+  return h->p.face_terms && h->halo_mode == 2 && h->kernel_mode == 4 && h->win_producer && s >= 6 && s <= 8 &&
+         h->plan.peers.empty() && !h->in_group;
+}
+
+int launch_pair(pamg_handle* h, LevelDev& L) {
+  ElemArgs a{};
+  a.Tin = L.T[L.cur]; a.Tout = L.T[L.cur ^ 1]; a.rhs = L.rhs; a.ovl = L.ovlb[L.ovl_cur]; a.pc = L.pc; a.strip_of = h->strip_of;
+  a.hmap = h->hmap; a.nsrc = nullptr; a.ovl_next = L.ovlb[L.ovl_cur ^ 1]; a.ovl_mid = L.ovl_mid; a.dst_strip = h->dst_strip;
+  a.rev = h->rev; a.nstrips = h->plan.nstrips; a.omega = h->p.omega; a.rsign = (double)h->p.residual_sign; a.nelem = L.nelem;
+  a.s = L.s;
+  const long long nb = (long long)h->U * 3 * L.S;
+  k_boundary_sweep<<<(unsigned)((nb + TPB - 1) / TPB), TPB, 0, h->stream>>>(a, h->U);
+  h->launches++;
+  CK(cudaGetLastError());
+  const bool prof = h->profiling && h->pev_used + 2 <= (int)h->pev.size();
+  if (prof) CK(cudaEventRecord(h->pev[h->pev_used], h->stream));
+  const int tgrid = (int)std::max(1ll, std::min(L.nelem / TPB, (long long)h->nsm * h->kc.pair));
+  k_jacobi_pair<<<tgrid, PAIR_THREADS, PAIR_SMEM_BYTES, h->stream>>>(a);
+  if (prof) { CK(cudaEventRecord(h->pev[h->pev_used + 1], h->stream)); h->pev_used += 2; }
+  h->launches++;
+  CK(cudaGetLastError());
+  return PAMG_OK;
+}
+
+int tnew_resolve(pamg_handle* h, LevelDev& L) {
+  if (!L.tnew_pending || L.tnew_alias) { L.tnew_pending = false; return PAMG_OK; }
+  L.tnew_pending = false;
+  const ElemOverride ov = {L.ovlb[L.ovl_cur ^ 1], L.pc, (double)h->p.residual_sign};
+  int rc = launch_element<MODE_JACOBI>(h, L, L.T[L.cur ^ 1], L.tmid, 0, grid_for(h, L.nelem), true, false, false, false, &ov);
+  if (rc) return rc;
+  CK(cudaMemcpyAsync(L.T[L.cur ^ 1], L.tmid, L.ndof * sizeof(double), cudaMemcpyDeviceToDevice, h->stream));
+  return PAMG_OK;
+}
+
+int smooth_pair(pamg_handle* h, int level) {
+  LevelDev& L = h->lev[level - 1];
+  if (!L.tmid) CK(cudaMalloc(&L.tmid, L.ndof * sizeof(double)));
+  L.tnew_alias = true;
+  L.tnew_pending = false;
+  if (h->debug_gap_ns > 0) { k_spin<<<1, 32, 0, h->stream>>>(h->debug_gap_ns); }
+  int rc = ensure_strips(h, level, true);
+  if (rc) return rc;
+  if ((rc = launch_pair(h, L))) return rc;
+  L.cur ^= 1;
+  L.tnew_alias = false; L.tnew_pending = true; L.tnew_ovl = L.ovl_mid;
+  L.ovl_cur ^= 1;
+  L.strips_valid = true; L.cut_valid = true; L.stage_valid = false;
+  return PAMG_OK;
+}
+
 int do_smooth(pamg_handle* h, int level, int solver, int nsweeps, bool norm_first = false) {
   LevelDev& L = h->lev[level - 1];
   if (level == 1 && !L.rhs_valid) { int rc = launch_build_rhs(h); if (rc) return rc; }
   const int grid = grid_for(h, L.nelem);
   if (solver < 1 || solver > 4) return fail(h, PAMG_ERR_ARG, "solver must be 1 (Jacobi), 2 (Richardson) or 3 (Gauss-Seidel)");
   for (int sw = 0; sw < nsweeps; ++sw) {
+    if (solver == 1 && L.ovl_mid && sw + 3 < nsweeps && !(norm_first && sw == 0) && (L.tmid || !h->capturing)) {
+      for (int k = 0; k < 2; ++k) {
+        int rc = smooth_pair(h, level);
+        if (rc) return rc;
+      }
+      sw += 3;
+      continue;
+    }
     L.tnew_alias = true;
+    L.tnew_pending = false;
     if (h->debug_gap_ns > 0) { k_spin<<<1, 32, 0, h->stream>>>(h->debug_gap_ns); }
     const bool gs = solver == 3 || solver == 4;
     const bool in_place = gs && !gs_fused_ok(h, L);
@@ -745,10 +818,12 @@
       if (rc) return rc;
     }
     if (fusedk) {
+      L.tnew_ovl = L.ovlb[L.ovl_cur];
       L.ovl_cur ^= 1;
       L.strips_valid = true; L.cut_valid = h->plan.peers.empty();
       L.stage_valid = xs;
     } else {
+      L.tnew_ovl = nullptr;
       L.strips_valid = false; L.cut_valid = false; L.stage_valid = false;
     }
   }
@@ -774,10 +849,17 @@
   if (level == 1 && !L.rhs_valid) { int rc = launch_build_rhs(h); if (rc) return rc; }
   const int grid = grid_for(h, L.nelem);
   if (2 * grid > h->npartial) return fail(h, PAMG_ERR_STATE, "partial buffer too small");
-  const bool use_strips = L.strips_valid || h->halo_mode == 0;
-  int rc = ensure_strips(h, level, use_strips);
+  int rc = tnew_resolve(h, L);
   if (rc) return rc;
-  rc = launch_element<MODE_RESID>(h, L, tnew_ptr(L), L.res, 0, grid, use_strips);
+  if (!L.tnew_alias && L.tnew_ovl) {
+    const ElemOverride ov = {L.tnew_ovl, L.pc, (double)h->p.residual_sign};
+    rc = launch_element<MODE_RESID>(h, L, tnew_ptr(L), L.res, 0, grid, true, false, false, false, &ov);
+  } else {
+    const bool use_strips = L.strips_valid || h->halo_mode == 0;
+    rc = ensure_strips(h, level, use_strips);
+    if (rc) return rc;
+    rc = launch_element<MODE_RESID>(h, L, tnew_ptr(L), L.res, 0, grid, use_strips);
+  }
   if (rc) return rc;
   if (l2 || linf || smax) {
     if ((rc = queue_norms(h))) return rc;
@@ -813,6 +895,8 @@
   if (h->p.transfer == 0) {
     int rc = materialise_tnew(h, F);
     if (rc) return rc;
+    if ((rc = tnew_resolve(h, Cc))) return rc;
+    F.tnew_ovl = nullptr;
     a.src = tnew_ptr(Cc); a.dst = F.T[F.cur ^ 1];
     k_prolong_literal<<<grid_for(h, Cc.nelem), TPB, 0, h->stream>>>(a);
   } else {
@@ -1055,7 +1139,7 @@
   for (auto& g : h->vc_graphs) for (auto e : g.exec) cudaGraphExecDestroy(e);
   h->vc_graphs.clear();
   for (auto& L : h->lev) {
-    cudaFree(L.T[0]); cudaFree(L.T[1]); cudaFree(L.spare); cudaFree(L.told); cudaFree(L.rhs); cudaFree(L.res);
+    cudaFree(L.T[0]); cudaFree(L.T[1]); cudaFree(L.spare); cudaFree(L.tmid); cudaFree(L.told); cudaFree(L.rhs); cudaFree(L.res);
     cudaFree(L.ovl_old); cudaFree(L.pc); cudaFree(L.pc_old); cudaFree(L.xsend);
   }
   h->lev.clear();
@@ -1308,7 +1392,7 @@
     size_t tot = 0;
     for (int il = 0; il < h->p.multi_levels; ++il) {
       const size_t S = (size_t)1 << (h->p.n_split - il);
-      tot += 2 * (((size_t)(h->plan.nstrips + h->plan.nsend) * 3 * S * sizeof(double) + 255) / 256 * 256);
+      tot += (pair_level(h, h->p.n_split - il) ? 3 : 2) * (((size_t)(h->plan.nstrips + h->plan.nsend) * 3 * S * sizeof(double) + 255) / 256 * 256);
     }
     CK(cudaMalloc(&h->strip_arena, tot));
     CK(cudaMemsetAsync(h->strip_arena, 0, tot, h->stream));
@@ -1347,6 +1431,8 @@
     L.ovlb[0] = reinterpret_cast<double*>(reinterpret_cast<char*>(h->strip_arena) + arena_off);
     L.ovlb[1] = reinterpret_cast<double*>(reinterpret_cast<char*>(h->strip_arena) + arena_off + obp);
     arena_off += 2 * obp;
+    L.ovl_mid = nullptr;
+    if (pair_level(h, L.s)) { L.ovl_mid = reinterpret_cast<double*>(reinterpret_cast<char*>(h->strip_arena) + arena_off); arena_off += obp; }
     CK(cudaMalloc(&L.ovl_old, ob));
     CK(cudaMemsetAsync(L.ovl_old, 0, ob, h->stream));
     L.ovl_cur = 0; L.strips_valid = false; L.cut_valid = false; L.stage_valid = false;
@@ -1371,6 +1457,15 @@
       if (rc2) return rc2;
     }
   for (auto& Lv : h->lev) Lv.ovl_cur = 0;
+  for (int il = 1; il <= h->p.multi_levels; ++il) {
+    LevelDev& Lp = h->lev[il - 1];
+    if (!Lp.ovl_mid) continue;
+    double* keep = Lp.ovlb[0];
+    Lp.ovlb[0] = Lp.ovl_mid;
+    int rc2 = launch_halo(h, il, 1);
+    Lp.ovlb[0] = keep;
+    if (rc2) return rc2;
+  }
   if (h->lev[0].pc_old) {
     LevelDev& L1 = h->lev[0];
     double* keep = L1.ovlb[0];
@@ -1561,6 +1656,7 @@
   if (dst_field == src_field) return PAMG_OK;
   if (dst_field == PAMG_TNEW && src_field == PAMG_TNONLIN) { L.tnew_alias = true; return PAMG_OK; }
   if (dst_field == PAMG_TNONLIN && src_field == PAMG_TNEW) {
+    if (int rc = tnew_resolve(h, L)) return rc;
     if (!L.tnew_alias) { L.cur ^= 1; L.tnew_alias = true; L.strips_valid = false; L.cut_valid = false; L.stage_valid = false; }
     return PAMG_OK;
   }
@@ -2158,6 +2254,7 @@
   const size_t n = (size_t)L.nelem;
   double* d = nullptr;
   CK(cudaMalloc(&d, n * 12 * sizeof(double)));
+  if (int rc = tnew_resolve(h, L)) return rc;
   OutArgs a;
   a.xg = h->xg; a.T = tnew_ptr(L); a.x_all = x_all ? d : nullptr; a.analytical = analytical ? d + n * 6 : nullptr;
   a.error = error ? d + n * 9 : nullptr; a.nelem = L.nelem; a.s = L.s;
diff --git a/p-a_multigrids_b200/csrc/pamg_kernels.cuh b/p-a_multigrids_b200/csrc/pamg_kernels.cuh
--- a/p-a_multigrids_b200/csrc/pamg_kernels.cuh
+++ b/p-a_multigrids_b200/csrc/pamg_kernels.cuh
@@ -56,6 +56,7 @@
   const int32_t* hmap;
   const int32_t* nsrc;
   double* ovl_next;
+  double* ovl_mid;
   const int32_t* dst_strip;
   const int32_t* rev;
   int nstrips;
@@ -161,10 +162,13 @@
   va = __ldg(T + o + (d & 3)); vb = __ldg(T + o + ((d >> 2) & 3));
 }
 
+__device__ __forceinline__ void strip_pair(const double* __restrict__ ovl, int strip, int hm, int p, int S, double& va, double& vb) {
+  const double* e = ovl + ((size_t)strip * S + p) * 3;
+  va = __ldg(e + (hm & 3)); vb = __ldg(e + (hm >> 2));
+}
 __device__ __forceinline__ void ext_pair(const ElemArgs& a, int d, int strip, int hm, int p, int S, double& va, double& vb) {
   if (d >= 0) { nbr_pair(a.Tin, d, p, a.s, va, vb); return; }
-  const double* e = a.ovl + ((size_t)strip * S + p) * 3;
-  va = __ldg(e + (hm & 3)); vb = __ldg(e + (hm >> 2));
+  strip_pair(a.ovl, strip, hm, p, S, va, vb);
 }
 
 __device__ __forceinline__ void halo_pair(const ElemArgs& a, int u, int mf, int slot0, int S, double& va, double& vb) {
@@ -710,6 +714,28 @@
 constexpr int WIN2_THREADS = TPB + 32;
 __device__ __forceinline__ void named_arrive(int id, int count) { asm volatile("bar.arrive %0, %1;" ::"r"(id), "r"(count) : "memory"); }
 __device__ __forceinline__ void named_sync(int id, int count) { asm volatile("bar.sync %0, %1;" ::"r"(id), "r"(count) : "memory"); }
+__device__ __forceinline__ void mbar_arrive_cta(uint64_t* bar) {
+  asm volatile("mbarrier.arrive.release.cta.shared::cta.b64 _, [%0];" ::"r"(smem_u32(bar)) : "memory");
+}
+
+__device__ __forceinline__ int face_child_fi(const ElemArgs& a, const double* __restrict__ ovl, const ParentRegs& P, int u,
+                                             int r, int ipos, int len, int S, double h1a, double h1b, double h2a, double h2b,
+                                             FaceIn& fi) {
+  int bmask = 0;
+  if (r == 1) { fi.n1a = h1a; fi.n1b = h1b; fi.pen1 = P.px1; bmask |= 1; }
+  if (ipos == 1) { fi.n2a = h2a; fi.n2b = h2b; fi.pen2 = P.px2; bmask |= 2; }
+  if (ipos == len) {
+    if (len == 1) {
+      const int d = a.nsrc ? __ldg(a.nsrc + u * 3 + 1) : -1;
+      if (d >= 0) nbr_pair(a.Tin, d, r - 1, a.s, fi.n3a, fi.n3b);
+      else strip_pair(ovl, __ldg(a.strip_of + u * 3 + 1), __ldg(a.hmap + u * 3 + 1), r - 1, S, fi.n3a, fi.n3b);
+    } else {
+      fi.n3a = h2a; fi.n3b = h2b;
+    }
+    fi.pen3 = P.px3; bmask |= 4;
+  }
+  return bmask;
+}
 
 template <int MODE, bool FACE, bool XCHG = false, bool NORM = false>
 __global__ void __launch_bounds__(WIN2_THREADS, 3) k_element_win2(ElemArgs a) {
@@ -858,13 +884,7 @@
           fi.n3a = t3[0]; fi.n3b = t3[1];
           if (up && (cur.r == 1 || cur.ipos == 1 || cur.ipos == cur.len)) {
             interior = false;
-            if (cur.r == 1) { fi.n1a = cur.h1a; fi.n1b = cur.h1b; fi.pen1 = P.px1; bmask |= 1; }
-            if (cur.ipos == 1) { fi.n2a = cur.h2a; fi.n2b = cur.h2b; fi.pen2 = P.px2; bmask |= 2; }
-            if (cur.ipos == cur.len) {
-              if (cur.len == 1) halo_pair(a, u_tile, 1, cur.r - 1, S, fi.n3a, fi.n3b);
-              else { fi.n3a = cur.h2a; fi.n3b = cur.h2b; }
-              fi.pen3 = P.px3; bmask |= 4;
-            }
+            bmask = face_child_fi(a, a.ovl, P, u_tile, cur.r, cur.ipos, cur.len, S, cur.h1a, cur.h1b, cur.h2a, cur.h2b, fi);
           }
         }
         if (FACE && MODE != MODE_RICH) {
@@ -908,6 +928,220 @@
       for (int i = 0; i < TPB / 32; ++i) { s0 += shp[0][i]; s1 = fmax(s1, shp[1][i]); s2 = fmax(s2, shp[2][i]); }
       double* partial = a.partial + (size_t)3 * a.partial_off;
       partial[(size_t)blockIdx.x * 3 + 0] = s0; partial[(size_t)blockIdx.x * 3 + 1] = s1; partial[(size_t)blockIdx.x * 3 + 2] = s2;
+    }
+  }
+}
+
+__global__ void __launch_bounds__(TPB) k_boundary_sweep(ElemArgs a, int U) {
+  const int s = a.s, S = 1 << s, b = 2 << s;
+  const long long gid = (long long)blockIdx.x * TPB + threadIdx.x;
+  if (gid >= (long long)U * 3 * S) return;
+  const int p = (int)(gid & (S - 1));
+  const int mf = (int)((gid >> s) % 3);
+  const int u = (int)((gid >> s) / 3);
+  const int dst = __ldg(a.dst_strip + u * 3 + mf);
+  if (dst < 0) return;
+  int r, ipos, len, k;
+  if (mf == 0) { r = 1; len = b - 1; ipos = 2 * p + 1; k = 2 * p; }
+  else { r = p + 1; len = b - 1 - 2 * p; ipos = (mf == 2) ? 1 : len; k = p * (b - p) + ipos - 1; }
+  const double* __restrict__ pc = a.pc + (size_t)u * NPC;
+  const ParentRegs& P = *reinterpret_cast<const ParentRegs*>(pc);
+  const size_t base = (((size_t)u) << (2 * s)) * 3;
+  const double* T = a.Tin + base + (size_t)k * 3;
+  FaceIn fi;
+  fi.pen1 = P.pi1; fi.pen2 = P.pi2; fi.pen3 = P.pi3;
+  fi.n1a = 0.0; fi.n1b = 0.0; fi.n2a = 0.0; fi.n2b = 0.0; fi.n3a = 0.0; fi.n3b = 0.0;
+  if (r > 1) { const double* tv = T + (2 * r - b - 2) * 3; fi.n1a = __ldg(tv + 2); fi.n1b = __ldg(tv); }
+  if (ipos > 1) { fi.n2a = __ldg(T - 2); fi.n2b = __ldg(T - 1); }
+  if (ipos < len) { fi.n3a = __ldg(T + 3); fi.n3b = __ldg(T + 4); }
+  double h1a = 0.0, h1b = 0.0, h2a = 0.0, h2b = 0.0;
+  if (r == 1) strip_pair(a.ovl, __ldg(a.strip_of + u * 3), __ldg(a.hmap + u * 3), ipos >> 1, S, h1a, h1b);
+  if (ipos == 1 || ipos == len) {
+    const int ms = (ipos == 1) ? 2 : 1;
+    strip_pair(a.ovl, __ldg(a.strip_of + u * 3 + ms), __ldg(a.hmap + u * 3 + ms), r - 1, S, h2a, h2b);
+  }
+  const int bmask = face_child_fi(a, a.ovl, P, u, r, ipos, len, S, h1a, h1b, h2a, h2b, fi);
+  const Folded& F = *reinterpret_cast<const Folded*>(pc + PC_FOLD);
+  const double* bb = a.rhs + base + (size_t)k * 3;
+  double o1, o2, o3;
+  elem_apply_folded<MODE_JACOBI>(F, pc + PC_DPEN, bmask, __ldg(T), __ldg(T + 1), __ldg(T + 2), fi, __ldg(bb), __ldg(bb + 1),
+                                 __ldg(bb + 2), a.rsign, o1, o2, o3);
+  const int slot = __ldg(a.rev + u * 3 + mf) ? (S - 1 - p) : p;
+  double* e = a.ovl_mid + ((size_t)dst * S + slot) * 3;
+  e[0] = o1; e[1] = o2; e[2] = o3;
+}
+
+constexpr int PAIR_NT = 16;
+constexpr int PAIR_NR = 8;
+constexpr int PAIR_CH = PAIR_NR * TPB;
+constexpr int PAIR_THREADS = 2 * TPB + 32;
+constexpr size_t PAIR_SMEM_BYTES = sizeof(double) * 3 * TPB * (PAIR_NT + 2 * PAIR_NR) + 8 * (PAIR_NT + 3 * PAIR_NR);
+
+__global__ void __launch_bounds__(PAIR_THREADS, 1) k_jacobi_pair(ElemArgs a) {
+  extern __shared__ __align__(128) unsigned char dsm[];
+  double* sT = reinterpret_cast<double*>(dsm);
+  double* s1 = sT + 3 * TPB * PAIR_NT;
+  double* sB = s1 + 3 * PAIR_CH;
+  uint64_t* barT = reinterpret_cast<uint64_t*>(sB + 3 * PAIR_CH);
+  uint64_t* barB = barT + PAIR_NT;
+  uint64_t* doneA = barB + PAIR_NR;
+  uint64_t* freeS1 = doneA + PAIR_NR;
+  __shared__ __align__(16) double sPC2[2][NPC];
+  __shared__ int sIdx2[2][8];
+  const int s = a.s, twos = 2 * s, b = 2 << s, S = 1 << s;
+  const int tid = threadIdx.x;
+  constexpr uint32_t TILE_BYTES = 3 * TPB * sizeof(double);
+  if (tid == 0) {
+    for (int i = 0; i < PAIR_NT + PAIR_NR; ++i) mbar_init(&barT[i], 1);
+    for (int i = 0; i < 2 * PAIR_NR; ++i) mbar_init(&doneA[i], TPB / 32);
+    asm volatile("fence.mbarrier_init.release.cluster;" ::: "memory");
+  }
+  __syncthreads();
+  const int ntiles = (int)(a.nelem / TPB);
+  const int per = (ntiles + gridDim.x - 1) / gridDim.x;
+  const int tbeg = blockIdx.x * per, tend = min(ntiles, tbeg + per);
+  if (tbeg >= tend) return;
+  const int pshift = twos - 8;
+  const int pfirst = (tbeg >> pshift) << pshift, pend = (((tend - 1) >> pshift) + 1) << pshift;
+  const int s1lo = max(pfirst, tbeg - 2), s1hi = min(pend, tend + 2);
+  const int tlo = max(pfirst, s1lo - 2), thi = min(pend, s1hi + 2);
+  auto slotB = [&](int t) { return (t - s1lo) & (PAIR_NR - 1); };
+  auto parB = [&](int t) { return (uint32_t)(((t - s1lo) >> 3) & 1); };
+
+  if (tid >= 2 * TPB) {
+    const int lane = tid - 2 * TPB;
+    int u_loaded = -1;
+    auto issueT = [&](int tile) {
+      const int sl = tile & (PAIR_NT - 1);
+      mbar_expect_tx(&barT[sl], TILE_BYTES);
+      tma_load_1d(sT + sl * 3 * TPB, a.Tin + (size_t)tile * 3 * TPB, TILE_BYTES, &barT[sl]);
+    };
+    auto issueB = [&](int tile) {
+      const int u = tile >> pshift;
+      if (u != u_loaded) {
+        for (int i = lane; i < NPC; i += 32) sPC2[u & 1][i] = __ldg(a.pc + (size_t)u * NPC + i);
+        if (lane < 3) { sIdx2[u & 1][lane] = __ldg(a.strip_of + u * 3 + lane); sIdx2[u & 1][4 + lane] = __ldg(a.hmap + u * 3 + lane); }
+        u_loaded = u;
+        __syncwarp();
+      }
+      if (lane == 0) {
+        mbar_expect_tx(&barB[slotB(tile)], TILE_BYTES);
+        tma_load_1d(sB + slotB(tile) * 3 * TPB, a.rhs + (size_t)tile * 3 * TPB, TILE_BYTES, &barB[slotB(tile)]);
+      }
+    };
+    int nT = tlo, nB = s1lo;
+    if (lane == 0) for (; nT < min(thi, tlo + PAIR_NT); ++nT) issueT(nT);
+    for (; nB < min(s1hi, s1lo + PAIR_NR); ++nB) issueB(nB);
+    int m0 = 0, u_m0 = -1;
+    StripDst sd = {-1, -1, -1, 0, nullptr, nullptr, nullptr};
+    for (int j = tbeg; j < tend; ++j) {
+      const int it = j - tbeg;
+      named_sync(1 + (it & 7), TPB + 32);
+      if (lane == 0) {
+        tma_store_1d(a.Tout + (size_t)j * 3 * TPB, sB + slotB(j) * 3 * TPB, TILE_BYTES);
+        tma_store_commit();
+        for (; nT < thi && nT <= j + PAIR_NT; ++nT) issueT(nT);
+        tma_store_wait_read1();
+      }
+      __syncwarp();
+      for (; nB < s1hi && nB <= j + 7; ++nB) issueB(nB);
+      const int u = j >> pshift;
+      if (u != u_m0) { m0 = 0; u_m0 = u; sd = strip_dst_load(a, u, lane); }
+      strips_from_tile(a, sB + slotB(j) * 3 * TPB, sd, (j << 8) & ((1 << twos) - 1), s, m0, lane);
+    }
+    if (lane == 0) tma_store_wait_all();
+    return;
+  }
+  const bool groupA = tid < TPB;
+  const int ct = tid & (TPB - 1);
+  const unsigned kmask = (1u << twos) - 1;
+  const double* ovl = groupA ? a.ovl : a.ovl_mid;
+  struct Prep { int r, ipos, len; double h1a, h1b, h2a, h2b; };
+  auto prepare = [&](int tile, int tile_end, int u_cur, bool first, Prep& p) {
+    p.h1a = 0.0; p.h1b = 0.0; p.h2a = 0.0; p.h2b = 0.0;
+    if (tile >= tile_end) return;
+    const int kk = (int)((((unsigned)tile << 8) + (unsigned)ct) & kmask);
+    if (first) child_from_ele0(kk, s, p.r, p.ipos, p.len);
+    else child_advance(s, b, kk, p.r, p.ipos);
+    p.len = b + 1 - 2 * p.r;
+    if (!(p.ipos & 1)) return;
+    const bool f1 = p.r == 1, side = p.ipos == 1 || p.ipos == p.len;
+    if (f1 | side) {
+      const int u = tile >> pshift;
+      const bool same = u == u_cur;
+      const int* ix = sIdx2[u & 1];
+      if (f1) strip_pair(ovl, same ? ix[0] : __ldg(a.strip_of + u * 3), same ? ix[4] : __ldg(a.hmap + u * 3), p.ipos >> 1, S, p.h1a, p.h1b);
+      if (side) {
+        const int mf = (p.ipos == 1) ? 2 : 1;
+        strip_pair(ovl, same ? ix[mf] : __ldg(a.strip_of + u * 3 + mf), same ? ix[4 + mf] : __ldg(a.hmap + u * 3 + mf), p.r - 1, S,
+                   p.h2a, p.h2b);
+      }
+    }
+  };
+  auto waitB = [&](int t) { mbar_wait(&barB[slotB(t)], parB(t)); };
+  auto relax = [&](const Prep& c, int u, auto ld, int rmask, double b1, double b2, double b3, double& o1, double& o2, double& o3,
+                   int cw) {
+    const double* sPC = sPC2[u & 1];
+    const ParentRegs& P = *reinterpret_cast<const ParentRegs*>(sPC);
+    const bool up = c.ipos & 1;
+    FaceIn fi;
+    fi.pen1 = P.pi1; fi.pen2 = P.pi2; fi.pen3 = P.pi3;
+    const int dv = up ? (2 * c.r - b - 2) : (b - 2 * c.r);
+    const int iv = (cw + dv) & rmask, il = (cw - 1) & rmask, ir = (cw + 1) & rmask;
+    fi.n1a = ld(iv, 2); fi.n1b = ld(iv, 0);
+    const int i2 = up ? il : ir, i3 = up ? ir : il;
+    fi.n2a = ld(i2, 1); fi.n2b = ld(i2, 2);
+    fi.n3a = ld(i3, 0); fi.n3b = ld(i3, 1);
+    int bmask = 0;
+    if (up && (c.r == 1 || c.ipos == 1 || c.ipos == c.len))
+      bmask = face_child_fi(a, ovl, P, u, c.r, c.ipos, c.len, S, c.h1a, c.h1b, c.h2a, c.h2b, fi);
+    const Folded& F = *reinterpret_cast<const Folded*>(sPC + PC_FOLD + (up ? 0 : 16));
+    elem_apply_folded<MODE_JACOBI>(F, sPC + PC_DPEN, bmask, ld(cw, 0), ld(cw, 1), ld(cw, 2), fi, b1, b2, b3, a.rsign, o1, o2, o3);
+  };
+  Prep cur, nxt;
+  cur.r = 2; cur.ipos = 2; cur.len = 3;
+  if (groupA) {
+    auto ldT = [&](int i, int c) { return sT[i * 3 + c]; };
+    auto waitT = [&](int t) { mbar_wait(&barT[t & (PAIR_NT - 1)], (uint32_t)(((t - tlo) >> 4) & 1)); };
+    prepare(s1lo, s1hi, -1, true, cur);
+    for (int t = s1lo; t < s1hi; ++t) {
+      const int u = t >> pshift;
+      if (t == s1lo) { for (int tw = tlo; tw <= min(t + 2, thi - 1); ++tw) waitT(tw); }
+      else if (t + 2 < thi) waitT(t + 2);
+      waitB(t);
+      if (t - PAIR_NR >= s1lo) mbar_wait(&freeS1[(t - 6) & (PAIR_NR - 1)], (uint32_t)(((t - 6 - tbeg) >> 3) & 1));
+      nxt.r = cur.r; nxt.ipos = cur.ipos;
+      prepare(t + 1, s1hi, u, false, nxt);
+      const double* bb = sB + slotB(t) * 3 * TPB + ct * 3;
+      double o1, o2, o3;
+      relax(cur, u, ldT, PAIR_NT * TPB - 1, bb[0], bb[1], bb[2], o1, o2, o3, ((t & (PAIR_NT - 1)) << 8) + ct);
+      const int cw = ((t & (PAIR_NR - 1)) << 8) + ct;
+      s1[cw] = o1; s1[PAIR_CH + cw] = o2; s1[2 * PAIR_CH + cw] = o3;
+      __syncwarp();
+      if ((tid & 31) == 0) mbar_arrive_cta(&doneA[t & (PAIR_NR - 1)]);
+      cur = nxt;
+    }
+  } else {
+    auto ldS = [&](int i, int c) { return s1[c * PAIR_CH + i]; };
+    auto waitA = [&](int t) { mbar_wait(&doneA[t & (PAIR_NR - 1)], (uint32_t)(((t - s1lo) >> 3) & 1)); };
+    prepare(tbeg, tend, -1, true, cur);
+    for (int j = tbeg; j < tend; ++j) {
+      const int it = j - tbeg;
+      const int u = j >> pshift;
+      if (j == tbeg) { for (int tw = s1lo; tw <= min(j + 2, s1hi - 1); ++tw) waitA(tw); }
+      else if (j + 2 < s1hi) waitA(j + 2);
+      waitB(j);
+      nxt.r = cur.r; nxt.ipos = cur.ipos;
+      prepare(j + 1, tend, u, false, nxt);
+      double* bb = sB + slotB(j) * 3 * TPB + ct * 3;
+      double o1, o2, o3;
+      relax(cur, u, ldS, PAIR_CH - 1, bb[0], bb[1], bb[2], o1, o2, o3, ((j & (PAIR_NR - 1)) << 8) + ct);
+      bb[0] = o1; bb[1] = o2; bb[2] = o3;
+      fence_async_smem();
+      named_arrive(1 + (it & 7), TPB + 32);
+      __syncwarp();
+      if ((tid & 31) == 0) mbar_arrive_cta(&freeS1[j & (PAIR_NR - 1)]);
+      cur = nxt;
     }
   }
 }
@@ -1077,9 +1311,6 @@
   if (tid == 0) tma_store_wait_all();
 }
 
-__device__ __forceinline__ void mbar_arrive_cta(uint64_t* bar) {
-  asm volatile("mbarrier.arrive.release.cta.shared::cta.b64 _, [%0];" ::"r"(smem_u32(bar)) : "memory");
-}
 
 template <bool XCHG>
 __global__ void __launch_bounds__(WIN2_THREADS, 3) k_gs_win2(ElemArgs a) {
```

Measured after the change: 226.1 billion, median of 6. 0.894x the previous value.
